# MingyuKim87/Safe_Denoiser

Hardware: AMD Instinct MI355X
Metric: images/sec (512x512, 50 steps, SD-v1.4 + repellency) (higher is better)
Workload: dtype bf16; 1 GPU; README-default end to end (safree = svf = lra = true, safree_neg_prompt_config.json:26-28): token ids -> CLIP -> SAFREE projection -> DDPM 50 steps x UNet on 3 guidance branches with per-prompt text switching + safe_denoiser.yaml repellency (kernel_fast, M=515, sigma 3.15, scale .33, margin 1.6, window 780<=t<=1000) -> VAE decode -> uint8 512x512 images; SD-v1.4 UNet / CLIP / VAE with random weigh; guidance_branches=3, text_encoder_precision=bf16x3, prompts_per_batch=64, latent_repeat=3, renoise_draws_rank0=3520, parallelism=prompt-shard x1

## Files before the change

### include/sdn.h

```cpp
#ifndef SDN_H_
#define SDN_H_

#include <stddef.h>
#include <stdint.h>

#ifdef __cplusplus
extern "C" {
#endif

#define SDN_OK            0
#define SDN_E_INVALID    -1
#define SDN_E_LAUNCH     -2
#define SDN_E_WORKSPACE  -3
#define SDN_E_ARCH       -4

int sdn_abi_version(void);
const char* sdn_device_arch_host(void);


#define SDN_REPEL_RBF     0
#define SDN_REPEL_SPARSE  1
#define SDN_QNORM_NONE    0
#define SDN_QNORM_CHANNEL 1
#define SDN_OUT_REPELLED  0
// ... 129 lines not shown
                        void* stream);

int sdn_layernorm_mod_bf16(const void* x, int64_t rows, int32_t c, float eps, const float* scale, const float* shift,
                           int32_t ld_mod, int32_t rows_per_batch, void* out, void* stream);
int sdn_layernorm_mod_f16(const void* x, int64_t rows, int32_t c, float eps, const float* scale, const float* shift,
                          int32_t ld_mod, int32_t rows_per_batch, void* out, void* stream);

int sdn_patchify_bf16(const float* latents, int32_t batch, int32_t c, int32_t h, int32_t w, int32_t p, void* out, void* stream);
int sdn_patchify_f16(const float* latents, int32_t batch, int32_t c, int32_t h, int32_t w, int32_t p, void* out, void* stream);
int sdn_unpatchify_f32(const float* tokens, int32_t batch, int32_t c, int32_t h, int32_t w, int32_t p, float* out, void* stream);

int sdn_conv_in_bf16(const float* latents_nchw, const void* w, const float* bias, int32_t batch, int32_t cin,
                     int32_t h, int32_t wd, int32_t cout, void* out_nhwc, void* stream);
int sdn_conv_in_f16(const float* latents_nchw, const void* w, const float* bias, int32_t batch, int32_t cin,
                    int32_t h, int32_t wd, int32_t cout, void* out_nhwc, void* stream);

int sdn_timestep_embed_bf16(float timestep, int32_t batch, int32_t dim, void* out, void* stream);
int sdn_timestep_embed_f16(float timestep, int32_t batch, int32_t dim, void* out, void* stream);

int sdn_gemm_f32(const sdn_gemm_desc* d_host, const void* a, const void* a2, const void* w,
                 const float* bias, const float* rowbias, const float* rowgate, const void* residual, void* out,
                 void* stream);
int sdn_groupnorm_f32(const void* x, const void* x2, int32_t batch, int32_t hw, int32_t c1, int32_t c2,
                      int32_t groups, float eps, int32_t silu, const float* gamma, const float* beta,
                      void* out, float* stats_ws, void* stream);
int sdn_layernorm_f32(const void* x, int64_t rows, int32_t c, float eps, const float* gamma,
                      const float* beta, void* out, void* stream);
int sdn_attention_f32(const void* q, const void* k, const void* v, void* out, int32_t batch, int32_t heads,
                      int32_t nq, int32_t nk, int32_t head_dim, int32_t ldq, int32_t ldk, int32_t ldv,
                      int32_t ldo, float scale, void* stream);
int sdn_conv_in_f32(const float* latents_nchw, const void* w, const float* bias, int32_t batch, int32_t cin,
                    int32_t h, int32_t wd, int32_t cout, void* out_nhwc, void* stream);
int sdn_timestep_embed_f32(float timestep, int32_t batch, int32_t dim, void* out, void* stream);

int sdn_gemm_x3(const sdn_gemm_desc* d_host, const void* a, const void* a2, const void* w,
                const float* bias, const float* rowbias, const float* rowgate, const void* residual, void* out,
                void* stream);
int sdn_attention_x3(const void* q, const void* k, const void* v, void* out, int32_t batch, int32_t heads,
                     int32_t nq, int32_t nk, int32_t head_dim, int32_t ldq, int32_t ldk, int32_t ldv,
                     int32_t ldo, float scale, void* stream);

int sdn_layernorm_mod_f32(const void* x, int64_t rows, int32_t c, float eps, const float* scale, const float* shift,
                          int32_t ld_mod, int32_t rows_per_batch, void* out, void* stream);
int sdn_patchify_f32(const float* latents, int32_t batch, int32_t c, int32_t h, int32_t w, int32_t p, void* out, void* stream);
int sdn_joint_attention_f32(int32_t mode, const void* q, const void* k, const void* v, void* out,
                            const sdn_attn_segment2* seg2_host, int32_t batch, int32_t heads, int32_t n_total,
                            int32_t head_dim, int32_t ldq, int32_t ldk, int32_t ldv, int32_t ldo, float scale,
                            void* stream);

int sdn_split3(const float* x, const float* x2, int64_t rows, int32_t c1, int32_t c2, void* out_triple, void* stream);
int sdn_expand3_weights(const float* w, int64_t rows, int32_t cols, int32_t group, void* out_bf16, void* stream);
int sdn_groupnorm_f32_triple(const void* x, const void* x2, int32_t batch, int32_t hw, int32_t c1, int32_t c2, int32_t groups,
                             float eps, int32_t silu, const float* gamma, const float* beta, void* out_triple, float* stats_ws,
                             void* stream);
int sdn_layernorm_f32_triple(const void* x, int64_t rows, int32_t c, float eps, const float* gamma, const float* beta,
                             void* out_triple, void* stream);
int sdn_attention_x3_triple(const void* q, const void* k, const void* v, void* out_triple, int32_t batch, int32_t heads, int32_t nq,
                            int32_t nk, int32_t head_dim, int32_t ldq, int32_t ldk, int32_t ldv, int32_t ldo, float scale,
                            void* stream);
int sdn_attention_x3_pairs(const void* q, const void* k, const void* v, int32_t lo_offset_q, int32_t lo_offset_kv, void* out,
                           int32_t batch, int32_t heads, int32_t nq, int32_t nk, int32_t head_dim, int32_t ldq, int32_t ldk,
                           int32_t ldv, int32_t ldo, float scale, int32_t triple_out, void* stream);

int sdn_randn_philox_plan(int64_t numel, int32_t* grid_out, int64_t* offset_increment_out);
int sdn_randn_philox(const uint64_t* seeds, const uint64_t* offsets, const int32_t* rows, int32_t n_gen, int64_t numel,
                     float* out, void* stream);
int sdn_randn_philox_state(const uint64_t* seeds, uint64_t* offsets, const int32_t* flags, int32_t n_gen, int64_t numel,
                           float* out, void* stream);

typedef struct sdn_unet_config {
  int32_t in_channels, out_channels, sample_size;
  int32_t n_levels;
  int32_t block_out_channels[4];
  int32_t level_has_attn[4];
  int32_t layers_per_block;
  int32_t n_heads;
  int32_t cross_dim, text_len;
  int32_t norm_groups;
  int32_t dtype;
  int32_t latent_repeat;
} sdn_unet_config;

typedef struct sdn_unet sdn_unet;

#define SDN_P_VEC_F32     0
#define SDN_P_MAT         1
#define SDN_P_CONV3X3     2
#define SDN_P_GEGLU_MAT   3
#define SDN_P_GEGLU_VEC   4
#define SDN_P_POS_CROP    5
#define SDN_P_GLU_VALUE   7
#define SDN_P_GLU_GATE    8
#define SDN_P_DERIVED     6

typedef struct sdn_param_info {
  char     name[128];
  int32_t  kind;
  int32_t  rows, cols;
  int32_t  rows_padded;
  int64_t  offset;
} sdn_param_info;

int    sdn_unet_create(const sdn_unet_config* cfg_host, sdn_unet** out_host);
void   sdn_unet_destroy(sdn_unet* u);
int    sdn_unet_param_count(const sdn_unet* u);
int    sdn_unet_param_info(const sdn_unet* u, int32_t index, sdn_param_info* info_host);
size_t sdn_unet_weight_bytes(const sdn_unet* u);
size_t sdn_unet_workspace_bytes(sdn_unet* u, int32_t batch);
double sdn_unet_flops(sdn_unet* u, int32_t batch, double* attention_core_flops_host);

int sdn_unet_forward(sdn_unet* u, const void* weights, const float* latents, float timestep, const void* text,
                     float* out, int32_t batch, void* workspace, size_t workspace_bytes, void* stream);

typedef struct sdn_mmdit_config {
  int32_t in_channels, out_channels;
  int32_t sample_size, patch_size;
  int32_t num_layers;
  int32_t num_heads, head_dim;
  int32_t joint_dim, pooled_dim;
  int32_t text_len;
  int32_t time_dim;
  int32_t dtype;
} sdn_mmdit_config;
int sdn_mmdit_create(const sdn_mmdit_config* cfg_host, sdn_unet** out_host);
int sdn_mmdit_forward(sdn_unet* m, const void* weights, const float* latents, float timestep, const void* text,
                      const void* pooled, float* out, int32_t batch, void* workspace, size_t workspace_bytes,
                      void* stream);

typedef struct sdn_mmdit_ext {
  int32_t qk_norm;
  float qk_norm_eps;
  uint64_t dual_attention_mask;
} sdn_mmdit_ext;
int sdn_mmdit_create_ex(const sdn_mmdit_config* cfg_host, const sdn_mmdit_ext* ext_host, sdn_unet** out_host);
int sdn_qk_rmsnorm(int32_t dtype, void* qkv, int64_t rows, int32_t heads, int32_t ld, const float* wq, const float* wk, float eps,
                   void* stream);

int sdn_ln_fold(int32_t dtype, const void* w, const float* gamma, const float* beta, const float* bias, int32_t rows,
                int32_t cols, void* w_folded, float* c, float* d, void* stream);
int sdn_gemm_ln_bf16(const sdn_gemm_desc* desc, const void* a, const void* w_folded, const float* c, const float* d, float eps,
                     const float* row_stats, void* out, void* stream);
int sdn_gemm_ln_f16(const sdn_gemm_desc* desc, const void* a, const void* w_folded, const float* c, const float* d, float eps,
                    const float* row_stats, void* out, void* stream);
int sdn_row_stats_bf16(const void* x, int64_t rows, int32_t c, float eps, float* out, void* stream);
int sdn_row_stats_f16(const void* x, int64_t rows, int32_t c, float eps, float* out, void* stream);

int sdn_ffn_geglu_fused(int32_t dtype, int64_t M, int32_t C, const void* x, const float* row_stats, const void* w1_folded,
                        const float* c1, const float* d1, const void* w_cat, const float* b_cat, const void* residual, void* out,
                        float* col_stats, void* stream);

int sdn_gemm_k320(int32_t dtype, const sdn_gemm_desc* desc, const void* a, const void* w, const float* bias, const float* ln_c,
                  const float* ln_d, float ln_eps, const void* residual, void* out, void* stream);
int32_t sdn_gemm_k320_map(int32_t grid, int32_t col_groups, int32_t wg, int32_t* stream_out, int32_t* group_out);

int sdn_gemm_stats_bf16(const sdn_gemm_desc* desc, const void* a, const void* a2, const void* w, const float* bias,
                        const float* rowbias, const void* residual, void* out, float* col_stats, void* stream);
int sdn_gemm_stats_f16(const sdn_gemm_desc* desc, const void* a, const void* a2, const void* w, const float* bias,
                       const float* rowbias, const void* residual, void* out, float* col_stats, void* stream);
int sdn_groupnorm_cols_bf16(const void* x, const void* x2, int32_t batch, int32_t hw, int32_t c1, int32_t c2, int32_t groups,
                            float eps, int32_t silu, const float* gamma, const float* beta, void* out, float* stats_ws,
                            const float* cols1, const float* cols2, void* stream);
int sdn_groupnorm_cols_f16(const void* x, const void* x2, int32_t batch, int32_t hw, int32_t c1, int32_t c2, int32_t groups,
                           float eps, int32_t silu, const float* gamma, const float* beta, void* out, float* stats_ws,
                           const float* cols1, const float* cols2, void* stream);

int sdn_gemm_splitk_bf16(const sdn_gemm_desc* d, const void* a, const void* a2, const void* w, const float* bias,
                         const float* rowbias, const float* rowgate, const void* residual, void* out, void* partials,
                         size_t partial_bytes, void* stream);
int sdn_gemm_splitk_f16(const sdn_gemm_desc* d, const void* a, const void* a2, const void* w, const float* bias,
                        const float* rowbias, const float* rowgate, const void* residual, void* out, void* partials,
                        size_t partial_bytes, void* stream);

int sdn_conv_up4_weights(int32_t dtype, const void* w9, int32_t N, int32_t Cin, void* out, void* stream);

int sdn_repeat(const void* in, size_t bytes, int32_t rep, void* out, void* stream);

int sdn_unet_prepare(sdn_unet* u, void* weights, void* stream);

typedef struct sdn_vae_config {
  int32_t latent_channels, out_channels;
  int32_t sample_size;
  int32_t n_levels;
  int32_t block_out_channels[4];
  int32_t layers_per_block;
  int32_t norm_groups;
  int32_t dtype;
} sdn_vae_config;
int sdn_vae_decoder_create(const sdn_vae_config* cfg_host, sdn_unet** out_host);
int sdn_vae_decode(sdn_unet* vae, const void* weights, const float* latents, float latent_scale, float* image,
                   int32_t batch, void* workspace, size_t workspace_bytes, void* stream);
int sdn_vae_encoder_create(const sdn_vae_config* cfg_host, sdn_unet** out_host);
int sdn_vae_encode(sdn_unet* vae_encoder, const void* weights, const float* image, float* moments, int32_t batch,
                   void* workspace, size_t workspace_bytes, void* stream);
int sdn_gaussian_sample(const float* moments, const float* noise, int32_t batch, int32_t latent_channels, int32_t hw,
                        float scale, float* out, void* stream);
int sdn_image_postprocess(const float* image_nchw, int32_t batch, int32_t channels, int32_t height, int32_t width,
                          float* out_nhwc01, uint8_t* out_nhwc_u8, void* stream);
int sdn_latent_mix(const float* z, const float* w, const float* bias, int32_t batch, int32_t channels, int32_t hw,
                   float in_scale, float* out, void* stream);
int sdn_softmax_rows(int32_t dtype, const float* scores, int64_t ld_scores, int64_t rows, int32_t n, float scale,
                     void* out, int64_t ld_out, void* stream);
int sdn_transpose16(const void* in, int32_t rows, int32_t cols, int64_t ld_in, void* out, int64_t ld_out, void* stream);
int sdn_transpose32(const void* in, int32_t rows, int32_t cols, int64_t ld_in, void* out, int64_t ld_out, void* stream);

typedef struct sdn_clip_config {
  int32_t vocab_size;
  int32_t hidden_size, intermediate_size;
  int32_t num_layers, num_heads;
  int32_t max_position_embeddings;
  int32_t dtype;
} sdn_clip_config;
int sdn_clip_create(const sdn_clip_config* cfg_host, sdn_unet** out_host);
int sdn_clip_forward(sdn_unet* clip, const void* weights, const int32_t* input_ids, const int32_t* attention_mask,
                     void* last_hidden_state, int32_t batch, void* workspace, size_t workspace_bytes, void* stream);
int sdn_clip_embed(int32_t dtype, const int32_t* input_ids, const void* token_embedding, const void* position_embedding,
                   int64_t rows, int32_t seq_len, int32_t hidden, int32_t vocab, void* out, void* stream);
int sdn_masked_attention(int32_t dtype, const void* q, const void* k, const void* v, void* out, const int32_t* key_mask,
                         int32_t causal, int32_t batch, int32_t heads, int32_t n, int32_t head_dim, int32_t ldq,
                         int32_t ldk, int32_t ldv, int32_t ldo, float scale, void* stream);
int sdn_clip_embed_f32(const int32_t* input_ids, const void* token_embedding, const void* position_embedding, int64_t rows,
                       int32_t seq_len, int32_t hidden, int32_t vocab, void* out, void* stream);
int sdn_masked_attention_f32(const void* q, const void* k, const void* v, void* out, const int32_t* key_mask, int32_t causal,
                             int32_t batch, int32_t heads, int32_t n, int32_t head_dim, int32_t ldq, int32_t ldk, int32_t ldv,
                             int32_t ldo, float scale, void* stream);

typedef struct sdn_clip_proj_config {
  int32_t vocab_size;
  int32_t hidden_size, intermediate_size;
  int32_t num_layers, num_heads;
  int32_t max_position_embeddings;
  int32_t dtype;
  int32_t projection_dim;
  int32_t act;
  int32_t eos_token_id;
  int32_t hidden_tap;
} sdn_clip_proj_config;
int sdn_clip_proj_create(const sdn_clip_proj_config* cfg_host, sdn_unet** out_host);
int sdn_clip_proj_forward(sdn_unet* clip, const void* weights, const int32_t* input_ids, void* hidden, int64_t hidden_batch_stride,
                          int64_t hidden_row_stride, void* text_embeds, int64_t embeds_row_stride, int32_t batch, void* workspace,
                          size_t workspace_bytes, void* stream);
int sdn_clip_eos_rows(int32_t dtype, const int32_t* input_ids, const void* x, const float* gamma, const float* beta, int32_t batch,
                      int32_t seq_len, int32_t hidden, int32_t vocab, int32_t eos_token_id, float eps, void* out,
                      int32_t* positions, void* stream);
int sdn_copy_rows_strided(const void* src, int32_t batch, int32_t rows_per_batch, int32_t cols, int32_t elem_bytes, void* dst,
                          int64_t dst_batch_stride, int64_t dst_row_stride, void* stream);

typedef struct sdn_clip_vision_config {
  int32_t image_size, patch_size;
  int32_t hidden_size, intermediate_size;
  int32_t num_layers, num_heads;
  int32_t projection_dim;
  int32_t act;
  int32_t dtype;
} sdn_clip_vision_config;
int sdn_clip_vision_create(const sdn_clip_vision_config* cfg_host, sdn_unet** out_host);
int sdn_clip_vision_forward(sdn_unet* vision, const void* weights, const float* pixel_values, void* last_hidden_state,
                            void* image_embeds, int32_t batch, void* workspace, size_t workspace_bytes, void* stream);
int sdn_clip_patch_rows(int32_t dtype, const float* pixels, int32_t batch, int32_t image_size, int32_t patch_size, int32_t kpad,
                        void* out, void* stream);
int sdn_clip_vision_embed(int32_t dtype, const void* patch_proj, const float* class_embedding, const void* position_embedding,
                          const float* gamma, const float* beta, int32_t batch, int32_t tokens, int32_t hidden, float eps, void* out,
                          void* stream);
int sdn_clip_class_rows(int32_t dtype, const void* x, const float* gamma, const float* beta, int32_t batch, int32_t seq_len,
                        int32_t hidden, float eps, void* out, void* stream);
int sdn_image_resize_u8(const uint8_t* in, int32_t batch, int32_t in_size, int32_t out_size, const int32_t* coeffs,
                        const int32_t* bounds, int32_t ksize, uint8_t* tmp, uint8_t* out, void* stream);
int sdn_clip_normalize_u8(const uint8_t* in, int32_t batch, int32_t size, float mean_r, float mean_g, float mean_b, float std_r,
                          float std_g, float std_b, float* out, void* stream);
int sdn_embed_row_scores(const void* x, int32_t dtype_x, int64_t ldx, const void* y, int32_t dtype_y, int64_t ldy,
                         int32_t y_rows, int32_t rows, int32_t dim, int32_t normalize_y, float scale, float bias,
                         float* out, void* stream);
int sdn_embed_cross_mean(const void* x, int32_t dtype_x, int64_t ldx, int32_t rx, const void* y, int32_t dtype_y, int64_t ldy,
                         int32_t ry, int32_t dim, float* scratch, float* out, void* stream);
int sdn_image_resize_rect_u8(const uint8_t* in, int32_t batch, int32_t in_h, int32_t in_w, int32_t out_h, int32_t out_w,
                             const int32_t* coeffs_x, const int32_t* bounds_x, int32_t ksize_x, const int32_t* coeffs_y,
                             const int32_t* bounds_y, int32_t ksize_y, uint8_t* tmp, uint8_t* out_u8, float* out_f32, float mean_r,
                             float mean_g, float mean_b, float std_r, float std_g, float std_b, void* stream);

typedef struct sdn_t5_config {
  int32_t vocab_size;
  int32_t d_model, d_kv, d_ff;
  int32_t num_layers, num_heads;
  int32_t num_buckets, max_distance;
  float   eps;
  int32_t dtype;
} sdn_t5_config;
int sdn_t5_create(const sdn_t5_config* cfg_host, sdn_unet** out_host);
size_t sdn_t5_workspace_bytes(sdn_unet* t5, int32_t batch, int32_t n);
double sdn_t5_flops(sdn_unet* t5, int32_t batch, int32_t n, double* attention_core_flops_host);
int sdn_t5_forward(sdn_unet* t5, const void* weights, const int32_t* input_ids, const int32_t* attention_mask, int32_t n,
                   void* out, int32_t batch, void* workspace, size_t workspace_bytes, void* stream);
int sdn_rmsnorm(int32_t dtype, const void* x, int32_t x_is_f32, int64_t rows, int32_t c, float eps, const float* weight, void* out,
                void* stream);
int sdn_embed_tokens(int32_t dtype, const int32_t* input_ids, const void* token_embedding, int64_t rows, int32_t hidden,
                     int32_t vocab, float* out, void* stream);
int sdn_t5_bucket(int32_t relative_position, int32_t num_buckets, int32_t max_distance);
int sdn_t5_relative_bias(int32_t dtype, const void* table, int32_t num_buckets, int32_t max_distance, int32_t heads, int32_t n,
                         float* out, void* stream);
int sdn_bias_attention(int32_t dtype, const void* q, const void* k, const void* v, void* out, const float* bias,
                       const int32_t* key_mask, int32_t batch, int32_t heads, int32_t n, int32_t head_dim, int32_t ldq,
                       int32_t ldk, int32_t ldv, int32_t ldo, float scale, void* stream);

void sdn_unet_set_text_version(sdn_unet* u, uint64_t version);

void sdn_unet_set_graph_mode(sdn_unet* u, int32_t on);
void sdn_unet_set_split_k(sdn_unet* u, int32_t on);
// ... 42 lines not shown
```

### safe_denoiser_amd/_lib.py

```python
from __future__ import annotations

import ctypes as C
import os

import torch

_HERE = os.path.dirname(os.path.abspath(__file__))
_LIB = None


class SdnUnavailable(RuntimeError):
    """libsdn.so is missing/unloadable, or there is no gfx950 device for a compute call."""


class SdnError(RuntimeError):
    """A libsdn entry point returned a negative status."""


_ERR = {-1: "SDN_E_INVALID (bad shape / null or misaligned pointer)", -2: "SDN_E_LAUNCH", -3: "SDN_E_WORKSPACE",
        -4: "SDN_E_ARCH"}


def lib_path() -> str:
    return os.environ.get("SDN_LIB", os.path.join(_HERE, "libsdn.so"))


class RepelParams(C.Structure):
    _fields_ = [("n_query", C.c_int32), ("n_ref", C.c_int32), ("channels", C.c_int32), ("hw", C.c_int32),
                ("weight_fn", C.c_int32), ("qnorm", C.c_int32), ("sigma", C.c_float), ("radius", C.c_float),
                ("scale", C.c_float), ("epsilon", C.c_float), ("gate", C.c_float)]


class GemmDesc(C.Structure):
    _fields_ = [(n, C.c_int32) for n in ("M", "N", "K", "a_mode", "K1", "Hs", "Ws", "Cin", "Ho", "Wo", "stride",
                                         "upsample", "act", "out_kind", "rows_per_batch", "ld_rowbias", "ld_rowgate",
                                         "residual_bcast", "n_valid", "ldc", "asym_pad", "split_k", "res_pre", "x3_out",
                                         "f32_stream")]


class UnetConfig(C.Structure):
    _fields_ = [("in_channels", C.c_int32), ("out_channels", C.c_int32), ("sample_size", C.c_int32),
                ("n_levels", C.c_int32), ("block_out_channels", C.c_int32 * 4), ("level_has_attn", C.c_int32 * 4),
                ("layers_per_block", C.c_int32), ("n_heads", C.c_int32), ("cross_dim", C.c_int32),
                ("text_len", C.c_int32), ("norm_groups", C.c_int32), ("dtype", C.c_int32), ("latent_repeat", C.c_int32)]


class ProfileRow(C.Structure):
    _fields_ = [("kernel", C.c_char * 24), ("launches", C.c_int32), ("ms", C.c_double), ("flops", C.c_double),
                ("bytes", C.c_double)]


class MmditConfig(C.Structure):
    _fields_ = [(n, C.c_int32) for n in ("in_channels", "out_channels", "sample_size", "patch_size", "num_layers",
                                         "num_heads", "head_dim", "joint_dim", "pooled_dim", "text_len", "time_dim",
                                         "dtype")]


class MmditExt(C.Structure):
    _fields_ = [("qk_norm", C.c_int32), ("qk_norm_eps", C.c_float), ("dual_attention_mask", C.c_uint64)]


class VaeConfig(C.Structure):
    _fields_ = [("latent_channels", C.c_int32), ("out_channels", C.c_int32), ("sample_size", C.c_int32),
                ("n_levels", C.c_int32), ("block_out_channels", C.c_int32 * 4), ("layers_per_block", C.c_int32),
                ("norm_groups", C.c_int32), ("dtype", C.c_int32)]


class ClipConfig(C.Structure):
    _fields_ = [(n, C.c_int32) for n in ("vocab_size", "hidden_size", "intermediate_size", "num_layers", "num_heads",
                                         "max_position_embeddings", "dtype")]


class ClipProjConfig(C.Structure):
    _fields_ = [(n, C.c_int32) for n in ("vocab_size", "hidden_size", "intermediate_size", "num_layers", "num_heads",
                                         "max_position_embeddings", "dtype", "projection_dim", "act", "eos_token_id", "hidden_tap")]


class ClipVisionConfig(C.Structure):
    _fields_ = [(n, C.c_int32) for n in ("image_size", "patch_size", "hidden_size", "intermediate_size", "num_layers", "num_heads",
                                         "projection_dim", "act", "dtype")]


class InceptionConfig(C.Structure):
    _fields_ = [(n, C.c_int32) for n in ("image_size", "normalize_input", "dtype")]


class InceptionConv(C.Structure):
    _fields_ = [("name", C.c_char * 64)] + [(n, C.c_int32) for n in ("cin", "cout", "kh", "kw", "stride", "pad_h", "pad_w", "kpad",
                                                                     "n_padded")]


class T5Config(C.Structure):
    _fields_ = [(n, C.c_int32) for n in ("vocab_size", "d_model", "d_kv", "d_ff", "num_layers", "num_heads", "num_buckets",
                                         "max_distance")] + [("eps", C.c_float), ("dtype", C.c_int32)]


class AttnSegment2(C.Structure):
    _fields_ = [("q2", C.c_void_p), ("k2", C.c_void_p), ("v2", C.c_void_p), ("out2", C.c_void_p), ("n1", C.c_int32),
                ("ldq2", C.c_int32), ("ldk2", C.c_int32), ("ldv2", C.c_int32), ("ldo2", C.c_int32)]


class ParamInfo(C.Structure):
    _fields_ = [("name", C.c_char * 128), ("kind", C.c_int32), ("rows", C.c_int32), ("cols", C.c_int32),
                ("rows_padded", C.c_int32), ("offset", C.c_int64)]


_vp, _i32, _i64, _f32, _sz = C.c_void_p, C.c_int32, C.c_int64, C.c_float, C.c_size_t

SIGNATURES = {
    "sdn_abi_version": (C.c_int, []),
    "sdn_device_arch_host": (C.c_char_p, []),
    "sdn_repel_workspace_bytes": (_sz, [_i32, _i32, _i32, _i32]),
    "sdn_repel_apply": (C.c_int, [C.POINTER(RepelParams), _vp, _vp, _vp, _vp, _vp, _vp, _sz, _vp]),
    "sdn_repel_calibrate": (C.c_int, [C.POINTER(RepelParams), _vp, _vp, _vp, _vp, _sz, _vp]),
    "sdn_cfg_combine": (C.c_int, [_vp, _i32, _i32, _i64, _f32, _vp, _vp]),
    "sdn_sld_guidance": (C.c_int, [_vp, _i32, _i64, _f32, _f32, _f32, _f32, _f32, _i32, _vp, _vp, _vp]),
    "sdn_cfg_combine_rows": (C.c_int, [_vp, _i32, _i32, _i64, _vp, _vp, _vp]),
    "sdn_sld_guidance_rows": (C.c_int, [_vp, _i32, _i64, _vp, _f32, _f32, _f32, _f32, _i32, _vp, _vp, _vp]),
    "sdn_pred_x0": (C.c_int, [_vp, _vp, _i64, _f32, _f32, _f32, _vp, _vp]),
    "sdn_sched_step": (C.c_int, [_vp, _vp, _vp, _i64, _f32, _f32, _f32, _f32, _f32, _f32, _f32, _vp, _vp]),
    "sdn_add_noise": (C.c_int, [_vp, _vp, _i64, _f32, _f32, _vp, _vp]),
    "sdn_renoise_select": (C.c_int, [_vp, _vp, _vp, _vp, _i32, _i64, _f32, _f32, _vp]),
    "sdn_flow_euler_step": (C.c_int, [_vp, _vp, _i64, _f32, _f32, _vp, _vp]),
    "sdn_flow_endpoints": (C.c_int, [_vp, _vp, _i64, _f32, _vp, _vp, _vp]),
    "sdn_flow_renoise": (C.c_int, [_vp, _vp, _vp, _i64, _f32, _vp, _vp]),
    "sdn_gemm_bf16": (C.c_int, [C.POINTER(GemmDesc), _vp, _vp, _vp, _vp, _vp, _vp, _vp, _vp, _vp]),
    "sdn_gemm_f16": (C.c_int, [C.POINTER(GemmDesc), _vp, _vp, _vp, _vp, _vp, _vp, _vp, _vp, _vp]),
    "sdn_ln_fold": (C.c_int, [_i32, _vp, _vp, _vp, _vp, _i32, _i32, _vp, _vp, _vp, _vp]),
    "sdn_gemm_ln_bf16": (C.c_int, [C.POINTER(GemmDesc), _vp, _vp, _vp, _vp, _f32, _vp, _vp, _vp]),
    "sdn_gemm_ln_f16": (C.c_int, [C.POINTER(GemmDesc), _vp, _vp, _vp, _vp, _f32, _vp, _vp, _vp]),
    "sdn_row_stats_bf16": (C.c_int, [_vp, _i64, _i32, _f32, _vp, _vp]),
    "sdn_row_stats_f16": (C.c_int, [_vp, _i64, _i32, _f32, _vp, _vp]),
    "sdn_ffn_geglu_fused": (C.c_int, [_i32, _i64, _i32, _vp, _vp, _vp, _vp, _vp, _vp, _vp, _vp, _vp, _vp, _vp]),
    "sdn_gemm_k320": (C.c_int, [_i32, C.POINTER(GemmDesc), _vp, _vp, _vp, _vp, _vp, _f32, _vp, _vp, _vp]),
    "sdn_gemm_k320_map": (_i32, [_i32, _i32, _i32, C.POINTER(_i32), C.POINTER(_i32)]),
    "sdn_gemm_stats_bf16": (C.c_int, [C.POINTER(GemmDesc), _vp, _vp, _vp, _vp, _vp, _vp, _vp, _vp, _vp]),
    "sdn_gemm_stats_f16": (C.c_int, [C.POINTER(GemmDesc), _vp, _vp, _vp, _vp, _vp, _vp, _vp, _vp, _vp]),
    "sdn_groupnorm_cols_bf16": (C.c_int, [_vp, _vp, _i32, _i32, _i32, _i32, _i32, _f32, _i32, _vp, _vp, _vp, _vp, _vp, _vp, _vp]),
    "sdn_groupnorm_cols_f16": (C.c_int, [_vp, _vp, _i32, _i32, _i32, _i32, _i32, _f32, _i32, _vp, _vp, _vp, _vp, _vp, _vp, _vp]),
    "sdn_gemm_splitk_bf16": (C.c_int, [C.POINTER(GemmDesc), _vp, _vp, _vp, _vp, _vp, _vp, _vp, _vp, _vp, _sz, _vp]),
    "sdn_gemm_splitk_f16": (C.c_int, [C.POINTER(GemmDesc), _vp, _vp, _vp, _vp, _vp, _vp, _vp, _vp, _vp, _sz, _vp]),
    "sdn_groupnorm_bf16": (C.c_int, [_vp, _vp, _i32, _i32, _i32, _i32, _i32, _f32, _i32, _vp, _vp, _vp, _vp, _vp]),
    "sdn_groupnorm_f16": (C.c_int, [_vp, _vp, _i32, _i32, _i32, _i32, _i32, _f32, _i32, _vp, _vp, _vp, _vp, _vp]),
    "sdn_layernorm_f16": (C.c_int, [_vp, _i64, _i32, _f32, _vp, _vp, _vp, _vp]),
    "sdn_conv_in_f16": (C.c_int, [_vp, _vp, _vp, _i32, _i32, _i32, _i32, _i32, _vp, _vp]),
    "sdn_timestep_embed_f16": (C.c_int, [_f32, _i32, _i32, _vp, _vp]),
    "sdn_layernorm_bf16": (C.c_int, [_vp, _i64, _i32, _f32, _vp, _vp, _vp, _vp]),
    "sdn_attention_bf16": (C.c_int, [_vp, _vp, _vp, _vp, _i32, _i32, _i32, _i32, _i32, _i32, _i32, _i32, _i32, _f32,
                                     _vp]),
    "sdn_attention_f16": (C.c_int, [_vp, _vp, _vp, _vp, _i32, _i32, _i32, _i32, _i32, _i32, _i32, _i32, _i32, _f32,
                                    _vp]),
    "sdn_conv_in_bf16": (C.c_int, [_vp, _vp, _vp, _i32, _i32, _i32, _i32, _i32, _vp, _vp]),
    "sdn_timestep_embed_bf16": (C.c_int, [_f32, _i32, _i32, _vp, _vp]),
    "sdn_gemm_f32": (C.c_int, [C.POINTER(GemmDesc), _vp, _vp, _vp, _vp, _vp, _vp, _vp, _vp, _vp]),
    "sdn_groupnorm_f32": (C.c_int, [_vp, _vp, _i32, _i32, _i32, _i32, _i32, _f32, _i32, _vp, _vp, _vp, _vp, _vp]),
    "sdn_layernorm_f32": (C.c_int, [_vp, _i64, _i32, _f32, _vp, _vp, _vp, _vp]),
    "sdn_attention_f32": (C.c_int, [_vp, _vp, _vp, _vp, _i32, _i32, _i32, _i32, _i32, _i32, _i32, _i32, _i32, _f32, _vp]),
    "sdn_randn_philox_plan": (C.c_int, [C.c_int64, C.POINTER(C.c_int32), C.POINTER(C.c_int64)]),
    "sdn_randn_philox": (C.c_int, [_vp, _vp, _vp, _i32, C.c_int64, _vp, _vp]),
    "sdn_randn_philox_state": (C.c_int, [_vp, _vp, _vp, _i32, C.c_int64, _vp, _vp]),
    "sdn_gemm_x3": (C.c_int, [C.POINTER(GemmDesc), _vp, _vp, _vp, _vp, _vp, _vp, _vp, _vp, _vp]),
    "sdn_attention_x3": (C.c_int, [_vp, _vp, _vp, _vp, _i32, _i32, _i32, _i32, _i32, _i32, _i32, _i32, _i32, _f32, _vp]),
    "sdn_conv_in_f32": (C.c_int, [_vp, _vp, _vp, _i32, _i32, _i32, _i32, _i32, _vp, _vp]),
    "sdn_timestep_embed_f32": (C.c_int, [_f32, _i32, _i32, _vp, _vp]),
    "sdn_unet_create": (C.c_int, [C.POINTER(UnetConfig), C.POINTER(_vp)]),
    "sdn_unet_destroy": (None, [_vp]),
    "sdn_unet_param_count": (C.c_int, [_vp]),
    "sdn_unet_param_info": (C.c_int, [_vp, _i32, C.POINTER(ParamInfo)]),
    "sdn_unet_weight_bytes": (_sz, [_vp]),
    "sdn_unet_workspace_bytes": (_sz, [_vp, _i32]),
    "sdn_unet_flops": (C.c_double, [_vp, _i32, C.POINTER(C.c_double)]),
    "sdn_unet_forward": (C.c_int, [_vp, _vp, _vp, _f32, _vp, _vp, _i32, _vp, _sz, _vp]),
    "sdn_mmdit_create": (C.c_int, [C.POINTER(MmditConfig), C.POINTER(_vp)]),
    "sdn_mmdit_forward": (C.c_int, [_vp, _vp, _vp, _f32, _vp, _vp, _vp, _i32, _vp, _sz, _vp]),
    "sdn_mmdit_create_ex": (C.c_int, [C.POINTER(MmditConfig), C.POINTER(MmditExt), C.POINTER(_vp)]),
    "sdn_qk_rmsnorm": (C.c_int, [_i32, _vp, _i64, _i32, _i32, _vp, _vp, _f32, _vp]),
    "sdn_joint_attention": (C.c_int, [_i32, _vp, _vp, _vp, _vp, C.POINTER(AttnSegment2), _i32, _i32, _i32, _i32, _i32,
                                      _i32, _i32, _i32, _f32, _vp]),
    "sdn_layernorm_mod_bf16": (C.c_int, [_vp, _i64, _i32, _f32, _vp, _vp, _i32, _i32, _vp, _vp]),
    "sdn_layernorm_mod_f16": (C.c_int, [_vp, _i64, _i32, _f32, _vp, _vp, _i32, _i32, _vp, _vp]),
    "sdn_patchify_bf16": (C.c_int, [_vp, _i32, _i32, _i32, _i32, _i32, _vp, _vp]),
    "sdn_patchify_f16": (C.c_int, [_vp, _i32, _i32, _i32, _i32, _i32, _vp, _vp]),
    "sdn_unpatchify_f32": (C.c_int, [_vp, _i32, _i32, _i32, _i32, _i32, _vp, _vp]),
    "sdn_layernorm_mod_f32": (C.c_int, [_vp, _i64, _i32, _f32, _vp, _vp, _i32, _i32, _vp, _vp]),
    "sdn_patchify_f32": (C.c_int, [_vp, _i32, _i32, _i32, _i32, _i32, _vp, _vp]),
    "sdn_joint_attention_f32": (C.c_int, [_i32, _vp, _vp, _vp, _vp, C.POINTER(AttnSegment2), _i32, _i32, _i32, _i32, _i32,
                                          _i32, _i32, _i32, _f32, _vp]),
    "sdn_repeat": (C.c_int, [_vp, _sz, _i32, _vp, _vp]),
    "sdn_vae_decoder_create": (C.c_int, [C.POINTER(VaeConfig), C.POINTER(_vp)]),
    "sdn_vae_decode": (C.c_int, [_vp, _vp, _vp, _f32, _vp, _i32, _vp, _sz, _vp]),
    "sdn_vae_encoder_create": (C.c_int, [C.POINTER(VaeConfig), C.POINTER(_vp)]),
    "sdn_vae_encode": (C.c_int, [_vp, _vp, _vp, _vp, _i32, _vp, _sz, _vp]),
    "sdn_gaussian_sample": (C.c_int, [_vp, _vp, _i32, _i32, _i32, _f32, _vp, _vp]),
    "sdn_image_postprocess": (C.c_int, [_vp, _i32, _i32, _i32, _i32, _vp, _vp, _vp]),
    "sdn_latent_mix": (C.c_int, [_vp, _vp, _vp, _i32, _i32, _i32, _f32, _vp, _vp]),
    "sdn_softmax_rows": (C.c_int, [_i32, _vp, _i64, _i64, _i32, _f32, _vp, _i64, _vp]),
    "sdn_transpose16": (C.c_int, [_vp, _i32, _i32, _i64, _vp, _i64, _vp]),
    "sdn_transpose32": (C.c_int, [_vp, _i32, _i32, _i64, _vp, _i64, _vp]),
    "sdn_clip_create": (C.c_int, [C.POINTER(ClipConfig), C.POINTER(_vp)]),
    "sdn_clip_forward": (C.c_int, [_vp, _vp, _vp, _vp, _vp, _i32, _vp, _sz, _vp]),
    "sdn_clip_embed": (C.c_int, [_i32, _vp, _vp, _vp, _i64, _i32, _i32, _i32, _vp, _vp]),
    "sdn_masked_attention": (C.c_int, [_i32, _vp, _vp, _vp, _vp, _vp, _i32, _i32, _i32, _i32, _i32, _i32, _i32, _i32, _i32,
                                       _f32, _vp]),
    "sdn_clip_proj_create": (C.c_int, [C.POINTER(ClipProjConfig), C.POINTER(_vp)]),
    "sdn_clip_proj_forward": (C.c_int, [_vp, _vp, _vp, _vp, _i64, _i64, _vp, _i64, _i32, _vp, _sz, _vp]),
    "sdn_clip_eos_rows": (C.c_int, [_i32, _vp, _vp, _vp, _vp, _i32, _i32, _i32, _i32, _i32, _f32, _vp, _vp, _vp]),
    "sdn_copy_rows_strided": (C.c_int, [_vp, _i32, _i32, _i32, _i32, _vp, _i64, _i64, _vp]),
    "sdn_clip_vision_create": (C.c_int, [C.POINTER(ClipVisionConfig), C.POINTER(_vp)]),
    "sdn_clip_vision_forward": (C.c_int, [_vp, _vp, _vp, _vp, _vp, _i32, _vp, _sz, _vp]),
    "sdn_clip_patch_rows": (C.c_int, [_i32, _vp, _i32, _i32, _i32, _i32, _vp, _vp]),
    "sdn_clip_vision_embed": (C.c_int, [_i32, _vp, _vp, _vp, _vp, _vp, _i32, _i32, _i32, _f32, _vp, _vp]),
    "sdn_clip_class_rows": (C.c_int, [_i32, _vp, _vp, _vp, _i32, _i32, _i32, _f32, _vp, _vp]),
    "sdn_image_resize_u8": (C.c_int, [_vp, _i32, _i32, _i32, _vp, _vp, _i32, _vp, _vp, _vp]),
    "sdn_clip_normalize_u8": (C.c_int, [_vp, _i32, _i32, _f32, _f32, _f32, _f32, _f32, _f32, _vp, _vp]),
    "sdn_image_resize_rect_u8": (C.c_int, [_vp, _i32, _i32, _i32, _i32, _i32, _vp, _vp, _i32, _vp, _vp, _i32, _vp, _vp, _vp, _f32, _f32,
                                           _f32, _f32, _f32, _f32, _vp]),
    "sdn_inception_create": (C.c_int, [C.POINTER(InceptionConfig), C.POINTER(_vp)]),
    "sdn_inception_conv_count": (C.c_int, [_vp]),
    "sdn_inception_conv_info": (C.c_int, [_vp, _i32, C.POINTER(InceptionConv)]),
    "sdn_inception_forward": (C.c_int, [_vp, _vp, _vp, _vp, _i32, _i32, _i32, _i32, _vp, _sz, _vp]),
    "sdn_patch_rows_f32": (C.c_int, [_vp, _i32, _i32, _i32, _i32, _i32, _i32, _i32, _i32, _i32, _i32, _i32, _vp, _vp]),
    "sdn_pool3_f32": (C.c_int, [_i32, _vp, _i32, _i32, _i32, _i32, _i32, _i32, _vp, _i32, _i32, _vp]),
    "sdn_resize_bilinear_f32": (C.c_int, [_vp, _i32, _i32, _i32, _i32, _i32, _f32, _f32, _vp, _vp]),
    "sdn_spatial_mean_f32": (C.c_int, [_vp, _i32, _i32, _i32, _vp, _vp]),
    "sdn_embed_row_scores": (C.c_int, [_vp, _i32, _i64, _vp, _i32, _i64, _i32, _i32, _i32, _i32, _f32, _f32, _vp, _vp]),
    "sdn_embed_cross_mean": (C.c_int, [_vp, _i32, _i64, _i32, _vp, _i32, _i64, _i32, _i32, _vp, _vp, _vp]),
    "sdn_t5_create": (C.c_int, [C.POINTER(T5Config), C.POINTER(_vp)]),
    "sdn_t5_workspace_bytes": (_sz, [_vp, _i32, _i32]),
    "sdn_t5_flops": (C.c_double, [_vp, _i32, _i32, C.POINTER(C.c_double)]),
    "sdn_t5_forward": (C.c_int, [_vp, _vp, _vp, _vp, _i32, _vp, _i32, _vp, _sz, _vp]),
    "sdn_rmsnorm": (C.c_int, [_i32, _vp, _i32, _i64, _i32, _f32, _vp, _vp, _vp]),
    "sdn_embed_tokens": (C.c_int, [_i32, _vp, _vp, _i64, _i32, _i32, _vp, _vp]),
    "sdn_t5_bucket": (C.c_int, [_i32, _i32, _i32]),
    "sdn_t5_relative_bias": (C.c_int, [_i32, _vp, _i32, _i32, _i32, _i32, _vp, _vp]),
    "sdn_bias_attention": (C.c_int, [_i32, _vp, _vp, _vp, _vp, _vp, _vp, _i32, _i32, _i32, _i32, _i32, _i32, _i32, _i32, _f32,
                                     _vp]),
    "sdn_split3": (C.c_int, [_vp, _vp, _i64, _i32, _i32, _vp, _vp]),
    "sdn_expand3_weights": (C.c_int, [_vp, _i64, _i32, _i32, _vp, _vp]),
    "sdn_groupnorm_f32_triple": (C.c_int, [_vp, _vp, _i32, _i32, _i32, _i32, _i32, _f32, _i32, _vp, _vp, _vp, _vp, _vp]),
    "sdn_layernorm_f32_triple": (C.c_int, [_vp, _i64, _i32, _f32, _vp, _vp, _vp, _vp]),
    "sdn_attention_x3_triple": (C.c_int, [_vp, _vp, _vp, _vp, _i32, _i32, _i32, _i32, _i32, _i32, _i32, _i32, _i32, _f32, _vp]),
    "sdn_attention_x3_pairs": (C.c_int, [_vp, _vp, _vp, _i32, _i32, _vp, _i32, _i32, _i32, _i32, _i32, _i32, _i32, _i32, _i32, _f32, _i32, _vp]),
    "sdn_clip_embed_f32": (C.c_int, [_vp, _vp, _vp, _i64, _i32, _i32, _i32, _vp, _vp]),
    "sdn_masked_attention_f32": (C.c_int, [_vp, _vp, _vp, _vp, _vp, _i32, _i32, _i32, _i32, _i32, _i32, _i32, _i32, _i32, _f32, _vp]),
    "sdn_unet_prepare": (C.c_int, [_vp, _vp, _vp]),
    "sdn_unet_set_graph_mode": (None, [_vp, _i32]),
    "sdn_unet_set_text_version": (None, [_vp, C.c_uint64]),
    "sdn_unet_set_split_k": (None, [_vp, _i32]),
    "sdn_unet_set_conv_up4": (None, [_vp, _i32]),
    "sdn_conv_up4_weights": (C.c_int, [_i32, _vp, _i32, _i32, _vp, _vp]),
    "sdn_unet_profile_next": (None, [_vp]),
    "sdn_unet_profile_read": (C.c_int, [_vp, C.POINTER(ProfileRow), _i32]),
}


def lib():
    global _LIB
    if _LIB is None:
        path = lib_path()
        if not os.path.exists(path):
            raise SdnUnavailable(f"{path} not found: build it with `python -c 'import __graft_entry__ as g; g.build()'` "
                                 f"(or `make -C safe_denoiser_amd/csrc`).  There is no CPU fallback.")
        try:
            handle = C.CDLL(path)
        except OSError as e:
            raise SdnUnavailable(f"cannot load {path}: {e}") from e
        for name, (res, args) in SIGNATURES.items():
            fn = getattr(handle, name)
            fn.restype, fn.argtypes = res, args
        _LIB = handle
    return _LIB


def check(rc: int, what: str):
    if rc != 0:
        raise SdnError(f"{what} failed: {_ERR.get(rc, rc)}")


def require_gpu():
    if not torch.cuda.is_available():
        raise SdnUnavailable("no GPU visible: the safe-denoiser hot path only runs on an MI355X (gfx950); "
                             "there is no CPU fallback")


def dptr(t: torch.Tensor | None, dtype=None) -> int | None:
    if t is None:
        return None
# ... 12 lines not shown
```

### safe_denoiser_amd/csrc/sdn_gemm_k320.hip

```cpp
#include "sdn_common.h"
#include "sdn_ops.h"
#include "sdn_gemm_common.h"
#include "sdn_gemm_k320.h"

static int g_k320_max_wgs = 0;
static int g_k320_last[8] = {0};

namespace sdn_gemm_detail {

struct K320Args {
  const unsigned short* a; const unsigned short* w; const float* bias; const float* ln_c; const float* ln_d;
  const unsigned short* res; unsigned short* out;
  int M, ldc, ncg;
  float ln_eps;
};

template <typename T, int LNF, bool RES>
__global__ void __launch_bounds__(512)
k_gemm_k320(const K320Args g) {
#if defined(__HIP_DEVICE_COMPILE__)
  constexpr int ROWS = RES ? 32 : 64;
  constexpr int G = ROWS / 32;
  constexpr int RB = ROWS / 8;
  constexpr int IMG = ROWS * 128;
  constexpr int A_PIECES = 5 * RB / 4;
  constexpr int SLOT = 40960, RING = 3 * SLOT;
  constexpr int STG = RING;
  constexpr int PRM = STG + 32 * 640;
  constexpr int SMEM = PRM + 3 * 1280;
  static_assert(5 * IMG * (RES ? 2 : 1) == SLOT, "a panel fills its slot");
  static_assert(A_PIECES + (RES ? 5 : 0) == 10, "vmcnt(10) below counts ten pieces per DMA wave and panel");
  __shared__ __attribute__((aligned(1024))) unsigned char smem[SMEM];

  const int tid = threadIdx.x, lane = tid & 63;
  const int wid = __builtin_amdgcn_readfirstlane(tid >> 6);
  const int wm = wid >> 2, wn = wid & 3;
  const int fr = lane & 15, fq = lane >> 4;
  int stream, cg;
  const int S = sdn_k320_map((int)gridDim.x, g.ncg, (int)blockIdx.x, &stream, &cg);
  if (stream < 0) return;
  const int n0 = cg * 320;

  typename T::v8 wf[5][10];
  {
    const unsigned short* wrow = g.w + (long)(n0 + wn * 80 + fr) * 320 + fq * 8;
#pragma unroll
    for (int t = 0; t < 5; ++t)
#pragma unroll
      for (int s = 0; s < 10; ++s) wf[t][s] = *reinterpret_cast<const typename T::v8*>(wrow + t * 16 * 320 + s * 32);
  }
  if (tid < 320) {
    float* prm = reinterpret_cast<float*>(smem + PRM);
    prm[tid] = g.bias ? g.bias[n0 + tid] : 0.f;
    if constexpr (LNF) { prm[320 + tid] = g.ln_c[n0 + tid]; prm[640 + tid] = g.ln_d[n0 + tid]; }
  }
#pragma unroll
  for (int t = 0; t < 5; ++t)
#pragma unroll
    for (int s = 0; s < 10; ++s) asm volatile("" : "+v"(wf[t][s]));
  asm volatile("s_waitcnt vmcnt(0)" ::: "memory");
  __syncthreads();

  const __amdgpu_buffer_rsrc_t rs_a = make_rsrc(g.a, (unsigned)((long)g.M * 640));
  [[maybe_unused]] const __amdgpu_buffer_rsrc_t rs_r = make_rsrc(RES ? g.res : g.a, RES ? (unsigned)((long)g.M * g.ldc * 2) : 0u);
  auto issue = [&](int p, int slot, int ln) {
    const int lrow = (ln >> 3) & 7;
    const unsigned a_lane = (unsigned)(lrow * 640 + (((ln & 7) ^ lrow) << 4));
    [[maybe_unused]] const unsigned r_lane = (unsigned)(lrow * g.ldc * 2 + (((ln & 7) ^ lrow) << 4));
    const unsigned m0 = (unsigned)p * ROWS;
    unsigned char* dst = smem + slot * SLOT;
#pragma unroll
    for (int q = 0; q < A_PIECES; ++q) {
      const int piece = wid * A_PIECES + q;
      const int kt = piece / RB, rb = piece - kt * RB;
      const unsigned off = (m0 + rb * 8) * 640u + kt * 128 + a_lane;
      __builtin_amdgcn_raw_ptr_buffer_load_lds(rs_a, (lds_ptr_t)(dst + piece * 1024), 16, off, 0, 0, 0);
    }
    if constexpr (RES) {
#pragma unroll
      for (int q = 0; q < 5; ++q) {
        const unsigned off = (m0 + wid * 8) * (unsigned)(g.ldc * 2) + (unsigned)(n0 * 2 + q * 128) + r_lane;
        __builtin_amdgcn_raw_ptr_buffer_load_lds(rs_r, (lds_ptr_t)(dst + 5 * IMG + (wid * 5 + q) * 1024), 16, off, 0, 0, 0);
      }
    }
  };

  const int NP = (g.M + ROWS - 1) / ROWS;
  const int n_my = stream < NP ? (NP - stream + S - 1) / S : 0;
  if (wid < 4) { issue(stream, 0, tid); issue(stream + S, 1, tid); }

  const float* prm = reinterpret_cast<const float*>(smem + PRM);
  int slot = 0;
  for (int i = 0; i < n_my; ++i) {
    int tl = tid;
    asm volatile("" : "+v"(tl));
    const int fr = tl & 15, fq = (tl >> 4) & 3;
    const int orow = wm * 16 + fr;
    const int o_rowpart = (orow >> 3) * 5120 + (orow & 7) * 128;
    auto out_off = [&](int t) {
      const int cb = wn * 160 + t * 32 + fq * 8;
      return o_rowpart + (cb >> 7) * 1024 + ((((cb >> 4) & 7) ^ (orow & 7)) << 4) + (cb & 8);
    };
    const int st_r = (tl >> 3) & 31;
    const int st_lds = (st_r >> 3) * 5120 + (st_r & 7) * 128 + (((tl & 7) ^ (st_r & 7)) << 4);
    const int p = stream + i * S;
    const int m0 = p * ROWS;
    if (wid < 4) asm volatile("s_waitcnt vmcnt(10)" ::: "memory");
    asm volatile("s_waitcnt lgkmcnt(0)" ::: "memory");
    __builtin_amdgcn_s_barrier();
    asm volatile("" ::: "memory");
    if (wid < 4) issue(p + 2 * S, slot == 0 ? 2 : slot - 1, tl);
    const unsigned char* sa = smem + slot * SLOT;
#pragma unroll
    for (int gi = 0; gi < G; ++gi) {
      const int row_l = wm * (ROWS / 2) + gi * 16 + fr;
      f32x4 acc[5];
#pragma unroll
      for (int t = 0; t < 5; ++t) acc[t] = *reinterpret_cast<const f32x4*>(prm + wn * 80 + t * 16 + fq * 4);
      if constexpr (RES) {
        const unsigned r_addr = (unsigned)(unsigned long)(lds_ptr_t)const_cast<unsigned char*>(sa + 5 * IMG);
        unsigned long long rr[5];
#pragma unroll
        for (int t = 0; t < 5; ++t) asm volatile("ds_read_b64 %0, %1" : "=v"(rr[t]) : "v"(r_addr + (unsigned)out_off(t)) : "memory");
        asm volatile("s_waitcnt lgkmcnt(0)" : "+v"(rr[0]), "+v"(rr[1]), "+v"(rr[2]), "+v"(rr[3]), "+v"(rr[4])::"memory");
#pragma unroll
        for (int t = 0; t < 5; ++t) {
          const unsigned lo = (unsigned)rr[t], hi = (unsigned)(rr[t] >> 32);
          acc[t][0] += T::to_f(lo & 0xffff); acc[t][1] += T::to_f(lo >> 16);
          acc[t][2] += T::to_f(hi & 0xffff); acc[t][3] += T::to_f(hi >> 16);
        }
      }
      [[maybe_unused]] float s1 = 0.f, s2 = 0.f;
      typename T::v8 fa[2];
      fa[0] = *reinterpret_cast<const typename T::v8*>(sa + lds_off(row_l, fq));
#pragma unroll
      for (int s = 0; s < 10; ++s) {
        if (s + 1 < 10)
          fa[(s + 1) & 1] = *reinterpret_cast<const typename T::v8*>(sa + ((s + 1) >> 1) * IMG + lds_off(row_l, ((s + 1) & 1) * 4 + fq));
        __builtin_amdgcn_sched_barrier(0);
        if constexpr (LNF) { s1 = T::dot_ones(fa[s & 1], s1); s2 = T::dot_self(fa[s & 1], s2); }
#pragma unroll
        for (int t = 0; t < 5; ++t) acc[t] = T::mfma16(wf[t][s], fa[s & 1], acc[t]);
        __builtin_amdgcn_sched_barrier(0);
      }
      [[maybe_unused]] float mu = 0.f, rs = 0.f;
      if constexpr (LNF) {
        const float invk = 1.0f / 320.0f;
        float a1 = s1, a2 = s2;
        a1 += __shfl_xor(a1, 16, 64); a2 += __shfl_xor(a2, 16, 64);
        a1 += __shfl_xor(a1, 32, 64); a2 += __shfl_xor(a2, 32, 64);
        mu = a1 * invk;
        const float var = fmaxf(a2 * invk - mu * mu, 0.f);
        rs = __builtin_amdgcn_rsqf(var + g.ln_eps);
      }
      if (!RES && gi > 0) {
        asm volatile("s_waitcnt lgkmcnt(0)" ::: "memory");
        __builtin_amdgcn_s_barrier();
        asm volatile("" ::: "memory");
      }
      const unsigned char* oimg = RES ? sa + 5 * IMG : smem + STG;
      const unsigned o_addr = (unsigned)(unsigned long)(lds_ptr_t)const_cast<unsigned char*>(oimg);
#pragma unroll
      for (int t = 0; t < 5; ++t) {
        f32x4 v = acc[t];
        if constexpr (LNF) {
          const f32x4 cv = *reinterpret_cast<const f32x4*>(prm + 320 + wn * 80 + t * 16 + fq * 4);
          const f32x4 dv = *reinterpret_cast<const f32x4*>(prm + 640 + wn * 80 + t * 16 + fq * 4);
          v = (acc[t] - mu * cv) * rs + dv;
        }
        uint2 pk; pk.x = T::pack2(v[0], v[1]); pk.y = T::pack2(v[2], v[3]);
        asm volatile("ds_write_b64 %0, %1" ::"v"(o_addr + (unsigned)out_off(t)), "v"((unsigned long long)pk.y << 32 | pk.x) : "memory");
        if constexpr (LNF) __builtin_amdgcn_sched_barrier(0);
      }
      asm volatile("s_waitcnt lgkmcnt(0)" ::: "memory");
      __builtin_amdgcn_s_barrier();
      asm volatile("" ::: "memory");
      if (wid >= 4) {
        const int m = m0 + (RES ? st_r : (st_r >> 4) * 32 + gi * 16 + (st_r & 15));
        if (m < g.M) {
          unsigned short* op = g.out + (long)m * g.ldc + n0 + (tl & 7) * 8;
#pragma unroll
          for (int k = 0; k < 5; ++k) *reinterpret_cast<u32x4*>(op + k * 64) = *reinterpret_cast<const u32x4*>(oimg + st_lds + k * 1024);
        }
      }
    }
    slot = slot == 2 ? 0 : slot + 1;
  }
  asm volatile("s_waitcnt vmcnt(0)" ::: "memory");
#endif
}

template <typename T>
int launch_k320(const K320Args& g, int grid, bool ln, bool res, hipStream_t st) {
  if (ln) hipLaunchKernelGGL((k_gemm_k320<T, 1, false>), dim3(grid), dim3(512), 0, st, g);
  else if (res) hipLaunchKernelGGL((k_gemm_k320<T, 0, true>), dim3(grid), dim3(512), 0, st, g);
  else hipLaunchKernelGGL((k_gemm_k320<T, 0, false>), dim3(grid), dim3(512), 0, st, g);
  return sdn_launch_status();
}

static inline bool al16(const void* p) { return (reinterpret_cast<uintptr_t>(p) & 15) == 0; }

}
using namespace sdn_gemm_detail;

extern "C" int32_t sdn_gemm_k320_map(int32_t grid, int32_t col_groups, int32_t wg, int32_t* stream_out, int32_t* group_out) {
  if (grid <= 0 || col_groups <= 0 || wg < 0 || wg >= grid) return SDN_E_INVALID;
  int s = -1, c = 0;
  const int S = sdn_k320_map(grid, col_groups, wg, &s, &c);
  if (stream_out) *stream_out = s;
  if (group_out) *group_out = c;
  return S;
}

extern "C" void sdn_debug_set_k320_max_wgs(int n) { g_k320_max_wgs = n > 0 ? n : 0; }
extern "C" void sdn_debug_k320_last_launch(int* out, int n) {
  for (int i = 0; out && i < n; ++i) out[i] = i < 8 ? g_k320_last[i] : 0;
}
extern "C" void sdn_debug_k320_reset_launch(void) { for (int& v : g_k320_last) v = 0; }

extern "C" int sdn_gemm_k320(int32_t dtype, const sdn_gemm_desc* d, const void* a, const void* w, const float* bias, const float* ln_c,
                             const float* ln_d, float ln_eps, const void* residual, void* out, void* stream) {
  if (!d || !a || !w || !out || dtype < 0 || dtype > 1) return SDN_E_INVALID;
  if (d->K != 320 || d->N <= 0 || d->N % 320 != 0 || d->M < 0) return SDN_E_INVALID;
  if (d->a_mode != SDN_A_PLAIN || (d->K1 != 0 && d->K1 != d->K) || d->act != SDN_ACT_NONE || d->out_kind != SDN_OUT_BF16 ||
      (d->n_valid != 0 && d->n_valid != d->N) || d->residual_bcast || d->split_k > 1 || d->x3_out || d->f32_stream || d->upsample)
    return SDN_E_INVALID;
  const bool ln = ln_c || ln_d;
  if (ln && (!ln_c || !ln_d || bias || residual)) return SDN_E_INVALID;
  const int ldc = d->ldc > 0 ? d->ldc : d->N;
  if (ldc < d->N || (ldc & 7)) return SDN_E_INVALID;
  if (!al16(a) || !al16(w) || !al16(out) || (residual && !al16(residual)) || (bias && !al16(bias)) || (ln && (!al16(ln_c) || !al16(ln_d))))
    return SDN_E_INVALID;
  if ((long)d->M * 640 >= (1L << 31) || (long)d->M * ldc * 2 >= (1L << 31) || ((long)d->M + 40000) * ldc * 2 >= (1L << 32)) return SDN_E_INVALID;
  if (d->M == 0) return SDN_OK;
  static int cus = 0;
  if (cus == 0) {
    int dev = 0;
    hipDeviceProp_t prop;
    if (hipGetDevice(&dev) != hipSuccess || hipGetDeviceProperties(&prop, dev) != hipSuccess) return SDN_E_LAUNCH;
    cus = prop.multiProcessorCount;
  }
  const int ncg = d->N / 320;
  int grid = cus > ncg ? cus : ncg;
  if (g_k320_max_wgs > 0 && g_k320_max_wgs < cus) {
    const int want = g_k320_max_wgs / ncg > 0 ? g_k320_max_wgs / ncg : 1;
    int s0, c0;
    for (grid = ncg; grid < cus && sdn_k320_map(grid, ncg, 0, &s0, &c0) < want; ++grid) {}
  }
  {
    int s0, c0;
    if (sdn_k320_map(grid, ncg, 0, &s0, &c0) < 1) return SDN_E_INVALID;
  }
  K320Args g{};
  g.a = (const unsigned short*)a; g.w = (const unsigned short*)w; g.bias = bias; g.ln_c = ln_c; g.ln_d = ln_d;
  g.res = (const unsigned short*)residual; g.out = (unsigned short*)out;
  g.M = d->M; g.ldc = ldc; g.ncg = ncg; g.ln_eps = ln_eps;
  {
    int s0, c0;
    const int S = sdn_k320_map(grid, ncg, 0, &s0, &c0);
    const int rows = residual ? 32 : 64;
    const int v[8] = {6, dtype, ln ? 1 : 0, residual ? 1 : 0, grid, ncg, S, (d->M + rows - 1) / rows};
    for (int i = 0; i < 8; ++i) g_k320_last[i] = v[i];
  }
  hipStream_t st = (hipStream_t)stream;
  return dtype == 0 ? launch_k320<SdnBF16>(g, grid, ln, residual != nullptr, st) : launch_k320<SdnF16>(g, grid, ln, residual != nullptr, st);
}
```

### safe_denoiser_amd/csrc/sdn_norm.hip

```cpp
#include "sdn_common.h"
#include "sdn_ops.h"

namespace sdn_norm_detail {

typedef __attribute__((ext_vector_type(4))) unsigned int u32x4;
constexpr int THREADS = 256;
constexpr int GN_MAX_TILES = 128;

template <typename T>
__device__ __forceinline__ void unpack8(const u32x4 v, float* f) {
  f[0] = T::to_f(v.x & 0xffff); f[1] = T::to_f(v.x >> 16); f[2] = T::to_f(v.y & 0xffff); f[3] = T::to_f(v.y >> 16);
  f[4] = T::to_f(v.z & 0xffff); f[5] = T::to_f(v.z >> 16); f[6] = T::to_f(v.w & 0xffff); f[7] = T::to_f(v.w >> 16);
}
template <typename T>
__device__ __forceinline__ u32x4 pack8(const float* f) {
  return (u32x4){T::pack2(f[0], f[1]), T::pack2(f[2], f[3]), T::pack2(f[4], f[5]), T::pack2(f[6], f[7])};
}
__device__ __forceinline__ float silu_f(float v) { return v / (1.f + __expf(-v)); }

template <typename T>
__global__ void __launch_bounds__(THREADS)
k_gn_stats(const unsigned short* __restrict__ x, const unsigned short* __restrict__ x2, int hw, int c1, int c2,
           int groups, int rows_per_tile, int ct, int nch, float* __restrict__ partials) {
  extern __shared__ float lds[];
  const int C = c1 + c2, cpg = C / groups;
  const int b = blockIdx.x, tile = blockIdx.y, ntiles = gridDim.y;
  const int rt = THREADS / ct;
  const int cl = threadIdx.x % ct, rl = threadIdx.x / ct;
  const int r_lo = tile * rows_per_tile, r_hi = min(hw, r_lo + rows_per_tile);
  if (rl < rt) {
    for (int q = 0; q < nch; ++q) {
      const int ch0 = (cl + q * ct) * 8;
      const unsigned short* src; int ld, cc;
      if (ch0 < c1) { src = x; ld = c1; cc = ch0; } else { src = x2; ld = c2; cc = ch0 - c1; }
      float s[8], ss[8];
#pragma unroll
      for (int e = 0; e < 8; ++e) { s[e] = 0.f; ss[e] = 0.f; }
      for (int r = r_lo + rl; r < r_hi; r += 4 * rt) {
        u32x4 v[4];
#pragma unroll
        for (int j = 0; j < 4; ++j) {
          const int rr = min(r + j * rt, r_hi - 1);
          v[j] = *reinterpret_cast<const u32x4*>(src + ((long)b * hw + rr) * ld + cc);
        }
#pragma unroll
        for (int j = 0; j < 4; ++j) {
          if (r + j * rt < r_hi) {
            float f[8];
            unpack8<T>(v[j], f);
#pragma unroll
            for (int e = 0; e < 8; ++e) { s[e] += f[e]; ss[e] = fmaf(f[e], f[e], ss[e]); }
          }
        }
      }
#pragma unroll
      for (int e = 0; e < 8; ++e) {
        lds[((long)rl * C + ch0 + e) * 2 + 0] = s[e];
        lds[((long)rl * C + ch0 + e) * 2 + 1] = ss[e];
      }
    }
  }
  __syncthreads();
  if (threadIdx.x < groups) {
    const int gidx = threadIdx.x;
    float s = 0.f, ss = 0.f;
    for (int r = 0; r < rt; ++r)
      for (int c = gidx * cpg; c < (gidx + 1) * cpg; ++c) {
        s += lds[((long)r * C + c) * 2 + 0];
        ss += lds[((long)r * C + c) * 2 + 1];
      }
    float* o = partials + (((long)b * ntiles + tile) * groups + gidx) * 2;
    o[0] = s; o[1] = ss;
  }
}

__global__ void __launch_bounds__(512)
k_gn_finalize(const float* __restrict__ partials, int ntiles, int groups, float n, float eps,
              float* __restrict__ stats) {
  __shared__ float sh[64][8][2];
  const int b = blockIdx.x, gi = threadIdx.x >> 3, part = threadIdx.x & 7;
  if (gi < groups) {
    float s = 0.f, ss = 0.f;
    for (int t = part; t < ntiles; t += 8) {
      const float* p = partials + (((long)b * ntiles + t) * groups + gi) * 2;
      s += p[0]; ss += p[1];
    }
    sh[gi][part][0] = s; sh[gi][part][1] = ss;
  }
  __syncthreads();
  if (gi < groups && part == 0) {
    float s = 0.f, ss = 0.f;
#pragma unroll
    for (int k = 0; k < 8; ++k) { s += sh[gi][k][0]; ss += sh[gi][k][1]; }
    const float mean = s / n;
    const float var = fmaxf(ss / n - mean * mean, 0.f);
    stats[((long)b * groups + gi) * 2 + 0] = mean;
    stats[((long)b * groups + gi) * 2 + 1] = rsqrtf(var + eps);
  }
}

__global__ void __launch_bounds__(256)
k_gn_finalize_cols(const float* __restrict__ cols1, const float* __restrict__ cols2, int blocks_per_sample, int c1, int c2,
                   int groups, float n, float eps, float* __restrict__ stats) {
  __shared__ float red[8];
  const int C = c1 + c2, cpg = C / groups, b = blockIdx.x, gi = blockIdx.y;
  const int total = blocks_per_sample * cpg;
  float s = 0.f, q = 0.f;
  for (int e = threadIdx.x; e < total; e += 256) {
    const int t = e / cpg, c = gi * cpg + (e - t * cpg);
    const bool second = c >= c1;
    const float* src = second ? cols2 : cols1;
    const int cw = second ? c2 : c1, cc = second ? c - c1 : c;
    const float2 v = *reinterpret_cast<const float2*>(src + 2 * (((long)b * blocks_per_sample + t) * cw + cc));
    s += v.x; q += v.y;
  }
  s = block_sum<4>(s, red);
  q = block_sum<4>(q, red + 4);
  if (threadIdx.x == 0) {
    const float mean = s / n;
    const float var = fmaxf(q / n - mean * mean, 0.f);
    stats[((long)b * groups + gi) * 2 + 0] = mean;
    stats[((long)b * groups + gi) * 2 + 1] = rsqrtf(var + eps);
  }
}

template <typename T>
__global__ void __launch_bounds__(THREADS)
k_gn_apply(const unsigned short* __restrict__ x, const unsigned short* __restrict__ x2, int hw, int c1, int c2,
           int groups, int rows_per_block, int silu, const float* __restrict__ gamma,
           const float* __restrict__ beta, const float* __restrict__ stats, unsigned short* __restrict__ out) {
  extern __shared__ float aff[];
  const int C = c1 + c2, cpg = C / groups, cchunks = C / 8;
  const int b = blockIdx.x;
  float* ca = aff; float* cb = aff + C;
  for (int c = threadIdx.x; c < C; c += THREADS) {
    const int gi = c / cpg;
    const float mean = stats[((long)b * groups + gi) * 2 + 0], rstd = stats[((long)b * groups + gi) * 2 + 1];
    const float a = rstd * gamma[c];
    ca[c] = a; cb[c] = beta[c] - mean * a;
  }
  __syncthreads();
  const int r_lo = blockIdx.y * rows_per_block, r_hi = min(hw, r_lo + rows_per_block);
  const long total = (long)(r_hi - r_lo) * cchunks;
  for (long e = threadIdx.x; e < total; e += THREADS) {
    const int r = r_lo + (int)(e / cchunks), ch0 = (int)(e % cchunks) * 8;
    const unsigned short* src; int ld, cc;
    if (ch0 < c1) { src = x; ld = c1; cc = ch0; } else { src = x2; ld = c2; cc = ch0 - c1; }
    const u32x4 v = *reinterpret_cast<const u32x4*>(src + ((long)b * hw + r) * ld + cc);
    float f[8];
    unpack8<T>(v, f);
    const float4 a0 = *reinterpret_cast<const float4*>(ca + ch0), a1 = *reinterpret_cast<const float4*>(ca + ch0 + 4);
    const float4 b0 = *reinterpret_cast<const float4*>(cb + ch0), b1 = *reinterpret_cast<const float4*>(cb + ch0 + 4);
    const float am[8] = {a0.x, a0.y, a0.z, a0.w, a1.x, a1.y, a1.z, a1.w};
    const float bm[8] = {b0.x, b0.y, b0.z, b0.w, b1.x, b1.y, b1.z, b1.w};
#pragma unroll
    for (int k = 0; k < 8; ++k) {
      const float y = fmaf(f[k], am[k], bm[k]);
      f[k] = silu ? silu_f(y) : y;
    }
    *reinterpret_cast<u32x4*>(out + ((long)b * hw + r) * C + ch0) = pack8<T>(f);
  }
}

template <typename T, int NQ, int R>
__global__ void __launch_bounds__(THREADS)
k_layernorm(const unsigned short* __restrict__ x, long rows, int C, float eps, const float* __restrict__ gamma,
            const float* __restrict__ beta, unsigned short* __restrict__ out, int mod, int rows_per_batch, int ld_mod) {
  const int lane = threadIdx.x & 63;
  const long row0 = ((long)blockIdx.x * 4 + (threadIdx.x >> 6)) * R;
  if (row0 >= rows) return;
  const int cchunks = C / 8;
  float f[R][NQ][8];
  float s[R];
#pragma unroll
  for (int r = 0; r < R; ++r) {
    s[r] = 0.f;
    const long row = row0 + r < rows ? row0 + r : rows - 1;
#pragma unroll
    for (int q = 0; q < NQ; ++q) {
      const int cc = lane + q * 64;
      if (cc < cchunks) {
        unpack8<T>(*reinterpret_cast<const u32x4*>(x + row * C + cc * 8), f[r][q]);
#pragma unroll
        for (int k = 0; k < 8; ++k) s[r] += f[r][q][k];
      }
    }
  }
  float mean[R], rstd[R];
#pragma unroll
  for (int r = 0; r < R; ++r) mean[r] = wave_sum(s[r]) / (float)C;
#pragma unroll
  for (int r = 0; r < R; ++r) {
    float ss = 0.f;
#pragma unroll
    for (int q = 0; q < NQ; ++q) {
      const int cc = lane + q * 64;
      if (cc < cchunks) {
#pragma unroll
        for (int k = 0; k < 8; ++k) { const float d = f[r][q][k] - mean[r]; ss = fmaf(d, d, ss); }
      }
    }
    s[r] = ss;
  }
#pragma unroll
  for (int r = 0; r < R; ++r) rstd[r] = rsqrtf(wave_sum(s[r]) / (float)C + eps);
#pragma unroll
  for (int q = 0; q < NQ; ++q) {
    const int cc = lane + q * 64;
    if (cc < cchunks) {
      float gm[8], bt[8];
      auto load_affine = [&](const float* gp, const float* bp) {
        const float4 g0 = *reinterpret_cast<const float4*>(gp + cc * 8), g1 = *reinterpret_cast<const float4*>(gp + cc * 8 + 4);
        const float4 b0 = *reinterpret_cast<const float4*>(bp + cc * 8), b1 = *reinterpret_cast<const float4*>(bp + cc * 8 + 4);
        gm[0] = g0.x; gm[1] = g0.y; gm[2] = g0.z; gm[3] = g0.w; gm[4] = g1.x; gm[5] = g1.y; gm[6] = g1.z; gm[7] = g1.w;
        bt[0] = b0.x; bt[1] = b0.y; bt[2] = b0.z; bt[3] = b0.w; bt[4] = b1.x; bt[5] = b1.y; bt[6] = b1.z; bt[7] = b1.w;
      };
      if (!mod) load_affine(gamma, beta);
#pragma unroll
      for (int r = 0; r < R; ++r) {
        const long row = row0 + r;
        if (row < rows) {
          if (mod) {
            const long b = row / rows_per_batch;
            load_affine(gamma + b * ld_mod, beta + b * ld_mod);
          }
          float y[8];
#pragma unroll
          for (int k = 0; k < 8; ++k) y[k] = (f[r][q][k] - mean[r]) * rstd[r] * (mod ? 1.f + gm[k] : gm[k]) + bt[k];
          *reinterpret_cast<u32x4*>(out + row * C + cc * 8) = pack8<T>(y);
        }
      }
    }
  }
}

template <typename T, int NQ, int R>
__global__ void __launch_bounds__(THREADS)
k_row_stats(const unsigned short* __restrict__ x, long rows, int C, float eps, float* __restrict__ out) {
  const int lane = threadIdx.x & 63;
  const long row0 = ((long)blockIdx.x * 4 + (threadIdx.x >> 6)) * R;
  if (row0 >= rows) return;
  const int cchunks = C / 8;
  float f[R][NQ][8];
  float s[R];
#pragma unroll
  for (int r = 0; r < R; ++r) {
    s[r] = 0.f;
    const long row = row0 + r < rows ? row0 + r : rows - 1;
#pragma unroll
    for (int q = 0; q < NQ; ++q) {
      const int cc = lane + q * 64;
      if (cc < cchunks) {
        unpack8<T>(*reinterpret_cast<const u32x4*>(x + row * C + cc * 8), f[r][q]);
#pragma unroll
        for (int k = 0; k < 8; ++k) s[r] += f[r][q][k];
      }
    }
  }
  float mean[R];
#pragma unroll
  for (int r = 0; r < R; ++r) mean[r] = wave_sum(s[r]) / (float)C;
#pragma unroll
  for (int r = 0; r < R; ++r) {
    float ss = 0.f;
#pragma unroll
    for (int q = 0; q < NQ; ++q) {
      const int cc = lane + q * 64;
      if (cc < cchunks) {
#pragma unroll
        for (int k = 0; k < 8; ++k) { const float d = f[r][q][k] - mean[r]; ss = fmaf(d, d, ss); }
      }
    }
    s[r] = ss;
  }
#pragma unroll
  for (int r = 0; r < R; ++r) {
    const float rstd = rsqrtf(wave_sum(s[r]) / (float)C + eps);
    if (lane == 0 && row0 + r < rows) *reinterpret_cast<float2*>(out + 2 * (row0 + r)) = make_float2(mean[r], rstd);
  }
}

template <typename T>
__global__ void __launch_bounds__(THREADS)
k_conv_in(const float* __restrict__ lat, const unsigned short* __restrict__ w, const float* __restrict__ bias,
          int B, int cin, int H, int W, int cout, int ldo, unsigned short* __restrict__ out) {
  extern __shared__ float wl[];
  const int kk = 9 * cin;
  for (int i = threadIdx.x; i < cout * kk; i += THREADS) {
    const int co = i / kk, k = i - co * kk;
    wl[((k * 2 + ((co >> 2) & 1)) * (cout / 8) + (co >> 3)) * 4 + (co & 3)] = T::to_f(w[i]);
  }
  __syncthreads();
  constexpr int PX = 4;
  const int cchunks = cout / 8;
  const int WQ = (W + PX - 1) / PX;
  const int total = B * H * WQ * cchunks;
  const int HWQ = H * WQ;
  for (int e = blockIdx.x * THREADS + threadIdx.x; e < total; e += gridDim.x * THREADS) {
    const int pq = e / cchunks, cc = e - pq * cchunks;
    const int b = pq / HWQ, rem = pq - b * HWQ;
    const int yh = rem / WQ, x0 = (rem - yh * WQ) * PX;
    float acc[PX][8];
    {
      const float4 b0 = *reinterpret_cast<const float4*>(bias + cc * 8), b1 = *reinterpret_cast<const float4*>(bias + cc * 8 + 4);
#pragma unroll
      for (int p = 0; p < PX; ++p) {
        acc[p][0] = b0.x; acc[p][1] = b0.y; acc[p][2] = b0.z; acc[p][3] = b0.w;
        acc[p][4] = b1.x; acc[p][5] = b1.y; acc[p][6] = b1.z; acc[p][7] = b1.w;
      }
    }
    const float* lb = lat + (long)b * cin * H * W;
    for (int c = 0; c < cin; ++c) {
      float v[3][PX + 2];
#pragma unroll
      for (int ty = 0; ty < 3; ++ty)
#pragma unroll
        for (int tx = 0; tx < PX + 2; ++tx) {
          const int iy = yh + ty - 1, ix = x0 + tx - 1;
          const bool ok = iy >= 0 && iy < H && ix >= 0 && ix < W;
          const float t = lb[((long)c * H + min(max(iy, 0), H - 1)) * W + min(max(ix, 0), W - 1)];
          v[ty][tx] = ok ? t : 0.f;
        }
#pragma unroll
      for (int tap = 0; tap < 9; ++tap) {
        const float4 w0 = *reinterpret_cast<const float4*>(&wl[(((tap * cin + c) * 2 + 0) * cchunks + cc) * 4]);
        const float4 w1 = *reinterpret_cast<const float4*>(&wl[(((tap * cin + c) * 2 + 1) * cchunks + cc) * 4]);
#pragma unroll
        for (int p = 0; p < PX; ++p) {
          const float x = v[tap / 3][tap % 3 + p];
          acc[p][0] = fmaf(x, w0.x, acc[p][0]); acc[p][1] = fmaf(x, w0.y, acc[p][1]);
          acc[p][2] = fmaf(x, w0.z, acc[p][2]); acc[p][3] = fmaf(x, w0.w, acc[p][3]);
          acc[p][4] = fmaf(x, w1.x, acc[p][4]); acc[p][5] = fmaf(x, w1.y, acc[p][5]);
          acc[p][6] = fmaf(x, w1.z, acc[p][6]); acc[p][7] = fmaf(x, w1.w, acc[p][7]);
        }
      }
    }
    const long pix0 = ((long)b * H + yh) * W + x0;
#pragma unroll
    for (int p = 0; p < PX; ++p)
      if (x0 + p < W) *reinterpret_cast<u32x4*>(out + (pix0 + p) * ldo + cc * 8) = pack8<T>(acc[p]);
  }
}

template <typename T>
__global__ void k_temb(float t_val, const float* __restrict__ t_dev, int B, int dim, unsigned short* __restrict__ out) {
  const float t = t_dev ? *t_dev : t_val;
  const int half = dim / 2;
  for (int i = blockIdx.x * blockDim.x + threadIdx.x; i < B * dim; i += gridDim.x * blockDim.x) {
    const int k = i % dim;
    const int kk = k < half ? k : k - half;
    const float f = expf(-9.210340371976184f * (float)kk / (float)half);
    const float a = t * f;
    const float v = k < half ? cosf(a) : sinf(a);
    out[i] = (unsigned short)(T::pack2(v, 0.f) & 0xffff);
  }
}

inline bool al16(const void* p) { return (reinterpret_cast<uintptr_t>(p) & 15) == 0; }


template <typename T>
int groupnorm_impl(const void* x, const void* x2, int32_t batch, int32_t hw, int32_t c1, int32_t c2, int32_t groups,
                   float eps, int32_t silu, const float* gamma, const float* beta, void* out, float* stats_ws,
                   void* stream, const float* cols1 = nullptr, const float* cols2 = nullptr) {
  if (!x || !gamma || !beta || !out || !stats_ws || batch < 0 || hw <= 0 || c1 <= 0 || c2 < 0 || groups <= 0 ||
      groups > 64)
    return SDN_E_INVALID;
  if (c2 > 0 && !x2) return SDN_E_INVALID;
  const int C = c1 + c2;
  if ((c1 & 7) || (c2 & 7) || C % groups != 0 || C > 4096) return SDN_E_INVALID;
  if (!al16(x) || (x2 && !al16(x2)) || !al16(out) || !al16(gamma) || !al16(beta)) return SDN_E_INVALID;
  if (batch == 0) return SDN_OK;
  const int cch = C / 8;
  int nch = (cch + THREADS - 1) / THREADS;
  while (cch % nch != 0) ++nch;
  const int ct = cch / nch;
  if (ct > THREADS) return SDN_E_INVALID;
  const int rt = THREADS / ct;
  int ntiles = (hw + 31) / 32;
  if (ntiles > GN_MAX_TILES) ntiles = GN_MAX_TILES;
  const int rows_per_tile = (hw + ntiles - 1) / ntiles;
  ntiles = (hw + rows_per_tile - 1) / rows_per_tile;
  hipStream_t st = (hipStream_t)stream;
  const size_t lds = (size_t)rt * C * 2 * sizeof(float);
  if (lds > 64 * 1024) return SDN_E_INVALID;
  if (cols1) {
    if ((hw & 127) || (c2 > 0 && !cols2)) return SDN_E_INVALID;
    record_norm_launch({2, T::kDtype, 0, 0, 0, 0, 0, 0, 0, 0, 1, 0});
    hipLaunchKernelGGL(k_gn_finalize_cols, dim3(batch, groups), dim3(256), 0, st, cols1, cols2, hw / 128, c1, c2, groups,
                       (float)hw * (float)(C / groups), eps, stats_ws);
  } else {
    float* partials = stats_ws + (size_t)batch * groups * 2;
    record_norm_launch({1, T::kDtype, 0, 0, nch, ct, ntiles, rows_per_tile, 0, 0, 0, 0});
    hipLaunchKernelGGL((k_gn_stats<T>), dim3(batch, ntiles), dim3(THREADS), lds, st, (const unsigned short*)x,
                       (const unsigned short*)x2, hw, c1, c2, groups, rows_per_tile, ct, nch, partials);
    hipLaunchKernelGGL(k_gn_finalize, dim3(batch), dim3(512), 0, st, partials, ntiles, groups,
                       (float)hw * (float)(C / groups), eps, stats_ws);
  }
  int rows_per_block = (256 * 8 * 16) / C;
  if (rows_per_block < 1) rows_per_block = 1;
  const int nblk = (hw + rows_per_block - 1) / rows_per_block;
  hipLaunchKernelGGL((k_gn_apply<T>), dim3(batch, nblk), dim3(THREADS), (size_t)2 * C * sizeof(float), st, (const unsigned short*)x,
                     (const unsigned short*)x2, hw, c1, c2, groups, rows_per_block, silu, gamma, beta, stats_ws,
                     (unsigned short*)out);
  return sdn_launch_status();
}

inline bool ln_width_ok(int c) { return c > 0 && !(c & 7) && (c <= 2048 || (c <= 2560 && c % 128 == 0)); }

template <typename T>
int layernorm_wide(const void* x, int64_t rows, int32_t c, float eps, const float* gamma, const float* beta, void* out, void* stream,
                   int mod, int rows_per_batch, int ld_mod) {
  hipLaunchKernelGGL((k_layernorm<T, 5, 1>), dim3((unsigned)((rows + 3) / 4)), dim3(THREADS), 0, (hipStream_t)stream,
                     (const unsigned short*)x, (long)rows, c, eps, gamma, beta, (unsigned short*)out, mod, rows_per_batch, ld_mod);
  record_norm_launch({mod ? 4 : 3, T::kDtype, 5, 1, 0, 0, 0, 0, 0, 0, 0, 0});
  return sdn_launch_status();
}
template <typename T>
int row_stats_wide(const void* x, int64_t rows, int32_t c, float eps, float* out, void* stream) {
  hipLaunchKernelGGL((k_row_stats<T, 5, 1>), dim3((unsigned)((rows + 3) / 4)), dim3(THREADS), 0, (hipStream_t)stream,
                     (const unsigned short*)x, (long)rows, c, eps, out);
  record_norm_launch({5, T::kDtype, 5, 1, 0, 0, 0, 0, 0, 0, 0, 0});
  return sdn_launch_status();
}

template <typename T>
int layernorm_impl(const void* x, int64_t rows, int32_t c, float eps, const float* gamma, const float* beta, void* out,
                   void* stream, int mod = 0, int rows_per_batch = 0, int ld_mod = 0) {
  if (!x || !gamma || !beta || !out || rows < 0 || !ln_width_ok(c)) return SDN_E_INVALID;
  if (!al16(x) || !al16(out) || !al16(gamma) || !al16(beta)) return SDN_E_INVALID;
  if (mod && (rows_per_batch <= 0 || ld_mod < c || (ld_mod & 3))) return SDN_E_INVALID;
  if (rows == 0) return SDN_OK;
  if (c > 2048) return layernorm_wide<T>(x, rows, c, eps, gamma, beta, out, stream, mod, rows_per_batch, ld_mod);
#define SDN_LN_LAUNCH(NQ, R)                                                                                          \
  do { hipLaunchKernelGGL((k_layernorm<T, NQ, R>), dim3((unsigned)((rows + 4 * (R) - 1) / (4 * (R)))), dim3(THREADS), 0,      \
                     (hipStream_t)stream, (const unsigned short*)x, (long)rows, c, eps, gamma, beta, (unsigned short*)out, \
                     mod, rows_per_batch, ld_mod);                                                                     \
  record_norm_launch({mod ? 4 : 3, T::kDtype, NQ, R, 0, 0, 0, 0, 0, 0, 0, 0}); } while (0)
  if (c <= 512) SDN_LN_LAUNCH(1, 4);
  else if (c <= 1024) SDN_LN_LAUNCH(2, 2);
  else SDN_LN_LAUNCH(4, 1);
#undef SDN_LN_LAUNCH
  return sdn_launch_status();
}

template <typename T>
__global__ void __launch_bounds__(THREADS)
k_patchify(const float* __restrict__ lat, int B, int C, int H, int W, int p, unsigned short* __restrict__ out) {
  const int hp = H / p, wp = W / p, K = C * p * p;
  const long total = (long)B * hp * wp * K;
  for (long e = (long)blockIdx.x * THREADS + threadIdx.x; e < total; e += (long)gridDim.x * THREADS) {
    const int k = (int)(e % K);
    const long tok = e / K;
    const int px = k % p, py = (k / p) % p, c = k / (p * p);
    const int tx = (int)(tok % wp), ty = (int)((tok / wp) % hp), b = (int)(tok / ((long)wp * hp));
    const float v = lat[(((long)b * C + c) * H + ty * p + py) * W + tx * p + px];
    out[e] = (unsigned short)(T::pack2(v, 0.f) & 0xffff);
  }
}
__global__ void __launch_bounds__(THREADS)
k_unpatchify(const float* __restrict__ tok, int B, int C, int H, int W, int p, float* __restrict__ out) {
  const int hp = H / p, wp = W / p;
  const long total = (long)B * C * H * W;
  for (long e = (long)blockIdx.x * THREADS + threadIdx.x; e < total; e += (long)gridDim.x * THREADS) {
    const int x = (int)(e % W), y = (int)((e / W) % H), c = (int)((e / ((long)W * H)) % C), b = (int)(e / ((long)W * H * C));
    const long t = ((long)b * hp + y / p) * wp + x / p;
    out[e] = tok[t * (p * p * C) + ((y % p) * p + (x % p)) * C + c];
  }
}
template <typename T>
int patchify_impl(const float* lat, int32_t B, int32_t C, int32_t H, int32_t W, int32_t p, void* out, void* stream) {
  if (!lat || !out || B < 0 || C <= 0 || H <= 0 || W <= 0 || p <= 0 || H % p || W % p) return SDN_E_INVALID;
  if (B == 0) return SDN_OK;
  const long total = (long)B * C * H * W;
  long grid = (total + THREADS - 1) / THREADS;
  if (grid > 2048) grid = 2048;
  hipLaunchKernelGGL((k_patchify<T>), dim3((unsigned)grid), dim3(THREADS), 0, (hipStream_t)stream, lat, B, C, H, W, p,
                     (unsigned short*)out);
  return sdn_launch_status();
}

template <typename T>
int conv_in_impl(const float* lat, const void* w, const float* bias, int32_t batch, int32_t cin, int32_t h, int32_t wd,
                 int32_t cout, void* out, void* stream) {
  if (!lat || !w || !bias || !out || batch < 0 || cin <= 0 || cin > 16 || h <= 0 || wd <= 0 || cout <= 0 ||
      (cout & 7) || !al16(out))
    return SDN_E_INVALID;
  if (batch == 0) return SDN_OK;
  int chunk = (int)((64 * 1024) / ((size_t)9 * cin * sizeof(float))) & ~7;
  if (chunk < 8) return SDN_E_INVALID;
  if (chunk > cout) chunk = cout;
  if ((long)batch * h * wd * (chunk / 8) >= (1L << 31)) return SDN_E_INVALID;
  for (int co0 = 0; co0 < cout; co0 += chunk) {
    const int cc = cout - co0 < chunk ? cout - co0 : chunk;
    const size_t lds = (size_t)cc * 9 * cin * sizeof(float);
    const long total = (long)batch * h * ((wd + 3) / 4) * (cc / 8);
    long grid = (total + THREADS - 1) / THREADS;
    if (grid > 4096) grid = 4096;
    hipLaunchKernelGGL((k_conv_in<T>), dim3((unsigned)grid), dim3(THREADS), lds, (hipStream_t)stream, lat,
                       (const unsigned short*)w + (size_t)co0 * 9 * cin, bias + co0, batch, cin, h, wd, cc, cout,
                       (unsigned short*)out + co0);
  }
  return sdn_launch_status();
}

template <typename T>
int temb_impl(float timestep, int32_t batch, int32_t dim, void* out, void* stream, const float* t_dev = nullptr) {
  if (!out || batch < 0 || dim <= 0 || (dim & 1)) return SDN_E_INVALID;
  if (batch == 0) return SDN_OK;
  const int n = batch * dim;
  hipLaunchKernelGGL((k_temb<T>), dim3((n + 255) / 256), dim3(256), 0, (hipStream_t)stream, timestep, t_dev, batch, dim,
                     (unsigned short*)out);
  return sdn_launch_status();
}

template <typename T>
int row_stats_impl(const void* x, int64_t rows, int32_t c, float eps, float* out, void* stream) {
  if (!x || !out || rows < 0 || !ln_width_ok(c) || !al16(x) || (reinterpret_cast<uintptr_t>(out) & 7)) return SDN_E_INVALID;
  if (rows == 0) return SDN_OK;
  if (c > 2048) return row_stats_wide<T>(x, rows, c, eps, out, stream);
#define SDN_RS_LAUNCH(NQ, R)                                                                                          \
  do { hipLaunchKernelGGL((k_row_stats<T, NQ, R>), dim3((unsigned)((rows + 4 * (R) - 1) / (4 * (R)))), dim3(THREADS), 0,      \
                     (hipStream_t)stream, (const unsigned short*)x, (long)rows, c, eps, out);                            \
  record_norm_launch({5, T::kDtype, NQ, R, 0, 0, 0, 0, 0, 0, 0, 0}); } while (0)
  if (c <= 512) SDN_RS_LAUNCH(1, 4);
  else if (c <= 1024) SDN_RS_LAUNCH(2, 2);
  else SDN_RS_LAUNCH(4, 1);
#undef SDN_RS_LAUNCH
  return sdn_launch_status();
}

}

int sdn_temb_from_device(int dtype, const float* t_dev, int batch, int dim, void* out, void* stream) {
  if (!t_dev) return SDN_E_INVALID;
  return dtype == 1 ? sdn_norm_detail::temb_impl<SdnF16>(0.f, batch, dim, out, stream, t_dev)
                    : sdn_norm_detail::temb_impl<SdnBF16>(0.f, batch, dim, out, stream, t_dev);
}
namespace { __global__ void k_set_scalar(float* dst, float v) { *dst = v; } }
int sdn_set_scalar(float* dst, float v, void* stream) {
  if (!dst) return SDN_E_INVALID;
  hipLaunchKernelGGL(k_set_scalar, dim3(1), dim3(1), 0, (hipStream_t)stream, dst, v);
  return sdn_launch_status();
}
using namespace sdn_norm_detail;

static int g_last_norm_launch[SDN_NL_COUNT] = {0};
void record_norm_launch(const sdn_norm_launch& l) {
  const int v[SDN_NL_COUNT] = {l.kernel, l.dtype, l.nq, l.r, l.nch, l.ct, l.ntiles, l.rows_per_tile, l.rpc, l.nchunk, l.stats_src, l.triple};
  for (int i = 0; i < SDN_NL_COUNT; ++i) g_last_norm_launch[i] = v[i];
}
extern "C" void sdn_debug_norm_last_launch(int* out, int n) {
  for (int i = 0; out && i < n; ++i) out[i] = i < SDN_NL_COUNT ? g_last_norm_launch[i] : 0;
}

#define SDN_NORM_ENTRY(SUF, T)                                                                                          \
  extern "C" int sdn_groupnorm_##SUF(const void* x, const void* x2, int32_t batch, int32_t hw, int32_t c1, int32_t c2, \
                                     int32_t groups, float eps, int32_t silu, const float* gamma, const float* beta,   \
                                     void* out, float* stats_ws, void* stream) {                                        \
    return groupnorm_impl<T>(x, x2, batch, hw, c1, c2, groups, eps, silu, gamma, beta, out, stats_ws, stream);         \
  }                                                                                                                     \
  extern "C" int sdn_groupnorm_cols_##SUF(const void* x, const void* x2, int32_t batch, int32_t hw, int32_t c1,         \
                                          int32_t c2, int32_t groups, float eps, int32_t silu, const float* gamma,      \
                                          const float* beta, void* out, float* stats_ws, const float* cols1,            \
                                          const float* cols2, void* stream) {                                           \
    if (!cols1) return SDN_E_INVALID;                                                                                   \
    return groupnorm_impl<T>(x, x2, batch, hw, c1, c2, groups, eps, silu, gamma, beta, out, stats_ws, stream, cols1,    \
                             cols2);                                                                                    \
  }                                                                                                                     \
  extern "C" int sdn_layernorm_##SUF(const void* x, int64_t rows, int32_t c, float eps, const float* gamma,            \
                                     const float* beta, void* out, void* stream) {                                      \
    return layernorm_impl<T>(x, rows, c, eps, gamma, beta, out, stream);                                                \
  }                                                                                                                     \
  extern "C" int sdn_layernorm_mod_##SUF(const void* x, int64_t rows, int32_t c, float eps, const float* scale,        \
                                         const float* shift, int32_t ld_mod, int32_t rows_per_batch, void* out,        \
                                         void* stream) {                                                                \
    return layernorm_impl<T>(x, rows, c, eps, scale, shift, out, stream, 1, rows_per_batch, ld_mod);                    \
  }                                                                                                                     \
  extern "C" int sdn_patchify_##SUF(const float* lat, int32_t B, int32_t C, int32_t H, int32_t W, int32_t p, void* out, \
                                    void* stream) {                                                                     \
    return patchify_impl<T>(lat, B, C, H, W, p, out, stream);                                                           \
  }                                                                                                                     \
  extern "C" int sdn_conv_in_##SUF(const float* lat, const void* w, const float* bias, int32_t batch, int32_t cin,     \
                                   int32_t h, int32_t wd, int32_t cout, void* out, void* stream) {                      \
    return conv_in_impl<T>(lat, w, bias, batch, cin, h, wd, cout, out, stream);                                         \
  }                                                                                                                     \
  extern "C" int sdn_timestep_embed_##SUF(float timestep, int32_t batch, int32_t dim, void* out, void* stream) {       \
    return temb_impl<T>(timestep, batch, dim, out, stream);                                                             \
  }
SDN_NORM_ENTRY(bf16, SdnBF16)
SDN_NORM_ENTRY(f16, SdnF16)

extern "C" int sdn_row_stats_bf16(const void* x, int64_t rows, int32_t c, float eps, float* out, void* stream) {
  return sdn_norm_detail::row_stats_impl<SdnBF16>(x, rows, c, eps, out, stream);
}
extern "C" int sdn_row_stats_f16(const void* x, int64_t rows, int32_t c, float eps, float* out, void* stream) {
  return sdn_norm_detail::row_stats_impl<SdnF16>(x, rows, c, eps, out, stream);
}

extern "C" int sdn_unpatchify_f32(const float* tok, int32_t B, int32_t C, int32_t H, int32_t W, int32_t p, float* out,
                                  void* stream) {
  if (!tok || !out || B < 0 || C <= 0 || H <= 0 || W <= 0 || p <= 0 || H % p || W % p) return SDN_E_INVALID;
  if (B == 0) return SDN_OK;
  const long total = (long)B * C * H * W;
  long grid = (total + THREADS - 1) / THREADS;
  if (grid > 2048) grid = 2048;
  hipLaunchKernelGGL(k_unpatchify, dim3((unsigned)grid), dim3(THREADS), 0, (hipStream_t)stream, tok, B, C, H, W, p, out);
  return sdn_launch_status();
}
```

### safe_denoiser_amd/csrc/sdn_plan.h

```cpp
#pragma once
#include <stdio.h>
#include <string.h>

#include <map>
#include <set>
#include <string>
#include <tuple>
#include <vector>

#include "sdn_common.h"
#include "sdn_ops.h"

namespace sdn_plan {

enum ModelKind { UNET, MMDIT, VAE_DECODER, VAE_ENCODER, CLIP, CLIP_PROJ, T5, CLIP_VISION, INCEPTION };

enum Space { SP_NONE = 0, SP_W = 1, SP_WS = 2, SP_IN = 3, SP_TEXT = 4, SP_OUT = 5, SP_POOLED = 6, SP_KV = 7, SP_OUT2 = 8 };
struct Ref { int space = SP_NONE; int64_t off = 0; };

struct Call {
  const void* weights; void* workspace; size_t workspace_bytes; int32_t batch; void* stream;
  const void *in = nullptr, *text = nullptr, *pooled = nullptr;
  void *out = nullptr, *out2 = nullptr;
  float scalar = 0.f; int n = 0;
  const int32_t* mask = nullptr;
  int64_t out_bs = 0, out_rs = 0, out2_rs = 0;
  int64_t kv_base = 0;
  int in_h = 0, in_w = 0;
  Call(const void* w, void* ws, size_t ws_bytes, int32_t b, void* s) : weights(w), workspace(ws), workspace_bytes(ws_bytes), batch(b), stream(s) {}
  const char* operator()(const Ref& r) const {
    switch (r.space) {
      case SP_W: return (const char*)weights + r.off;
      case SP_WS: return (const char*)workspace + r.off;
      case SP_KV: return (const char*)workspace + kv_base + r.off;
      case SP_IN: return (const char*)in + r.off;
      case SP_TEXT: return (const char*)text + r.off;
      case SP_OUT: return (const char*)out + r.off;
      case SP_OUT2: return (const char*)out2 + r.off;
      case SP_POOLED: return (const char*)pooled + r.off;
      default: return nullptr;
    }
  }
};

enum OpKind { OP_TEMB, OP_CONV_IN, OP_GEMM, OP_GN, OP_LN, OP_ATTN, OP_PATCHIFY, OP_UNPATCHIFY, OP_LATENT_MIX, OP_SOFTMAX,
              OP_TRANSPOSE, OP_REPEAT = 12 , OP_CLIP_EMBED, OP_MATTN,
              OP_ROWSTATS, OP_FFN, OP_SPLIT3,
              OP_RMSNORM, OP_EMBED, OP_T5_BIAS, OP_BATTN, OP_EOS_ROWS, OP_COPY_ROWS, OP_PATCH_ROWS, OP_VISION_EMBED, OP_CLASS_ROWS,
              OP_CONV_ROWS, OP_POOL3, OP_RESIZE, OP_SPATIAL_MEAN,
              OP_QK_RMSNORM  };

struct Op {
  int kind;
  sdn_gemm_desc gd;
  Ref a, a2, w, bias, rowbias, rowgate, residual, out, aux;
  Ref q2, k2, v2, out2;
  Ref col, cols1, cols2;
  Ref ln_c, ln_d, ln_stats;
  int ln = 0;
  int text_kv = 0;
  int x3t = 0;
  int pair_in = 0;
  int tri_out = 0;
  int dyn_ldc = 0;
  int k320 = 0;
  int n1 = 0, mod = 0, ld_mod = 0, patch = 0;
  int batch = 0, hw = 0, c1 = 0, c2 = 0, groups = 0, silu = 0;
  float eps = 0.f;
  int64_t rows = 0;
  int heads = 0, nq = 0, nk = 0, hd = 0, ldq = 0, ldk = 0, ldv = 0, ldo = 0;
  float scale = 0.f;
  Ref k, v;
  int kh = 0, kw = 0, sh = 0, sw = 0, ph = 0, pw = 0;
  char label[24] = {0};
  double flops = 0.0;
  double bytes = 0.0;
};

struct Arena {
  std::map<int64_t, int64_t> free_;
  int64_t top = 0, peak = 0;
  static int64_t up(int64_t v) { return (v + 255) & ~(int64_t)255; }
  int64_t alloc(int64_t bytes) {
    bytes = up(bytes);
    for (auto it = free_.begin(); it != free_.end(); ++it) {
      if (it->second >= bytes) {
        const int64_t off = it->first, rest = it->second - bytes;
        free_.erase(it);
        if (rest > 0) free_[off + bytes] = rest;
        return off;
      }
    }
    if (!free_.empty()) {
      auto last = std::prev(free_.end());
      if (last->first + last->second == top) {
        const int64_t off = last->first;
        free_.erase(last);
        top = off + bytes;
        if (top > peak) peak = top;
        return off;
      }
    }
    const int64_t off = top;
    top += bytes;
    if (top > peak) peak = top;
    return off;
  }
  void release(int64_t off, int64_t bytes) {
    bytes = up(bytes);
    auto it = free_.emplace(off, bytes).first;
    auto nx = std::next(it);
    if (nx != free_.end() && it->first + it->second == nx->first) { it->second += nx->second; free_.erase(nx); }
    if (it != free_.begin()) {
      auto pv = std::prev(it);
      if (pv->first + pv->second == it->first) { pv->second += it->second; free_.erase(it); }
    }
  }
};

struct Act {
  int64_t off = -1, bytes = 0; int C = 0, hw = 0, side = 0;
  int64_t content = 0;
  int64_t st_off = -1, st_bytes = 0;
};

struct Plan {
  int batch = 0;
  int64_t tscalar_off = -1;
  std::vector<Op> ops;
  int64_t ws_bytes = 0;
  int64_t kv_base = 0;
  double flops = 0.0, attn_flops = 0.0;
};

}

struct sdn_unet {
  sdn_plan::ModelKind kind = sdn_plan::UNET;
  sdn_unet_config cfg;
  sdn_mmdit_config mcfg;
  sdn_mmdit_ext mext = {0, 0.f, 0};
  sdn_vae_config vcfg;
  sdn_clip_config ccfg;
  sdn_clip_proj_config pcfg;
  sdn_t5_config tcfg;
  sdn_clip_vision_config vis;
  sdn_inception_config icfg;
  std::vector<sdn_inception_conv> convs;
  std::vector<sdn_param_info> params;
  std::map<std::string, int> param_index;
  int64_t weight_bytes = 0;
  std::map<int, sdn_plan::Plan> plans;
  int tproj_total = 0;
  int64_t subbatch_bytes = 0;
  bool profile_next = false;
  bool use_graph = false;
  bool gn_fuse = true;
  bool ln_fold = true;
  int ln_prepass_all = 0;
  bool ff_fuse = true;
  bool ffn_own_stats = true;
  bool ffn_fuse = true;
  struct FoldJob { int64_t w, gamma, beta, bias, wf, c, d; int rows, cols; int kind = 0; int group = 0; };
  std::vector<FoldJob> fold_jobs;
  uint64_t text_version = 0, kv_version = 0;
  int kv_batch = 0;
  const void *kv_w = nullptr, *kv_text = nullptr, *kv_ws = nullptr;
  bool x3_pairs = true;
  bool res_pre = true;
  bool gemm_k320 = true;
  bool x3_expand = true;
  bool split_k = false;
  bool conv_up4 = true;
  struct GraphKey {
    int batch; const void *w, *lat, *text, *pooled, *out, *ws;
    bool operator<(const GraphKey& o) const {
      return std::tie(batch, w, lat, text, pooled, out, ws) < std::tie(o.batch, o.w, o.lat, o.text, o.pooled, o.out, o.ws);
    }
  };
  std::map<GraphKey, hipGraphExec_t> graphs;
  hipStream_t cap_stream = nullptr;
  ~sdn_unet() {
    for (auto& kv : graphs) (void)hipGraphExecDestroy(kv.second);
    for (auto e : ev) (void)hipEventDestroy(e);
    if (cap_stream) (void)hipStreamDestroy(cap_stream);
  }
  std::vector<hipEvent_t> ev;
  int profiled_batch = 0;
  int profiled_n = 0;
  int dtype() const {
    switch (kind) {
      case sdn_plan::MMDIT: return mcfg.dtype;
      case sdn_plan::VAE_DECODER: case sdn_plan::VAE_ENCODER: return vcfg.dtype;
      case sdn_plan::CLIP: return ccfg.dtype;
      case sdn_plan::CLIP_PROJ: return pcfg.dtype;
      case sdn_plan::T5: return tcfg.dtype;
      case sdn_plan::CLIP_VISION: return vis.dtype;
      case sdn_plan::INCEPTION: return icfg.dtype;
      default: return cfg.dtype;
    }
  }
  bool is_vae() const { return kind == sdn_plan::VAE_DECODER || kind == sdn_plan::VAE_ENCODER; }
  bool is_clip() const { return kind == sdn_plan::CLIP || kind == sdn_plan::CLIP_PROJ; }
};

namespace sdn_plan {

constexpr bool kK320Plain = true, kK320Ln = true, kK320Rp = true;

struct GemmSpec {
  int64_t M; int N, K;
  Ref a, w, bias, out;
  Ref a2; int K1 = 0;
  Ref rowbias, rowgate; int rows_per_batch = 0, ld_row = 0;
  Ref residual; int residual_bcast = 0;
  int act = SDN_ACT_NONE, out_kind = SDN_OUT_BF16, n_valid = 0;
  Ref cols;
  bool res_pre = false;
  bool k320 = false;
  bool triple_out = false;
  bool pair_out = false;
  bool force_x3t = false;
  bool text_kv = false;
  bool dyn_ldc = false;
  bool f32_stream = false;
  GemmSpec(int64_t M_, int N_, int K_, Ref a_, Ref w_, Ref bias_, Ref out_) : M(M_), N(N_), K(K_), a(a_), w(w_), bias(bias_), out(out_) {}
  GemmSpec& with_a2(Ref v, int k1) { a2 = v; K1 = k1; return *this; }
  GemmSpec& with_rowbias(Ref v, int rpb, int ld) { rowbias = v; rows_per_batch = rpb; ld_row = ld; return *this; }
  GemmSpec& with_rowgate(Ref v, int rpb, int ld) { rowgate = v; rows_per_batch = rpb; ld_row = ld; return *this; }
  GemmSpec& with_residual(Ref v) { residual = v; return *this; }
  GemmSpec& with_residual_bcast(Ref v, int rpb) { residual = v; residual_bcast = 1; rows_per_batch = rpb; return *this; }
  GemmSpec& with_act(int v) { act = v; return *this; }
  GemmSpec& with_out_kind(int v) { out_kind = v; return *this; }
  GemmSpec& with_cols(Ref v) { cols = v; return *this; }
  GemmSpec& with_res_pre(bool v) { res_pre = v; return *this; }
  GemmSpec& with_k320(bool v) { k320 = v; return *this; }
  GemmSpec& with_triple_out(bool v) { triple_out = v; return *this; }
  GemmSpec& with_pair_out(bool v) { pair_out = v; return *this; }
  GemmSpec& with_force_x3t(bool v) { force_x3t = v; return *this; }
  GemmSpec& with_text_kv() { text_kv = true; return *this; }
  GemmSpec& with_dyn_ldc() { dyn_ldc = true; return *this; }
  GemmSpec& with_f32_stream(bool v) { f32_stream = v; return *this; }
};
struct ConvSpec {
  Act in; int cout, n_pad;
  Ref w, bias, out;
  int stride = 1, upsample = 0, asym_pad = 0;
  Ref rowbias; int ld_row = 0;
  Ref residual;
  int out_kind = SDN_OUT_BF16, n_valid = 0;
  Ref cols;
  bool res_pre = false;
  ConvSpec(const Act& in_, int cout_, Ref w_, Ref bias_, Ref out_) : in(in_), cout(cout_), n_pad(cout_), w(w_), bias(bias_), out(out_) {}
  ConvSpec& with_stride(int v, int asym = 0) { stride = v; asym_pad = asym; return *this; }
  ConvSpec& with_upsample() { upsample = 1; return *this; }
  ConvSpec& with_rowbias(Ref v, int ld) { rowbias = v; ld_row = ld; return *this; }
  ConvSpec& with_residual(Ref v) { residual = v; return *this; }
  ConvSpec& with_nchw_out(int n_pad_) { out_kind = SDN_OUT_F32_NCHW; n_valid = cout; n_pad = n_pad_; return *this; }
  ConvSpec& with_cols(Ref v) { cols = v; return *this; }
  ConvSpec& with_res_pre(bool v) { res_pre = v; return *this; }
};

struct Builder {
  sdn_unet* u;
  Plan* plan;
  Arena arena;
  int B;
  int seq = 0;
  int es = 2;
  bool x3t = false;
  bool x3t_hold = false;
  std::set<int64_t> tri;
  Ref tproj;
  int tproj_cursor = 0;
  Ref gn_stats;
  int64_t kv_top = 0;
  bool plan_bad = false;
  std::set<int64_t> pairs;
  struct Up4 { int64_t op; int64_t w9; int N, Cin; };
  std::vector<Up4> up4_pending;
  void finish_up4();
  struct Res { std::string pfx; int cout; };

  Ref param(const std::string& name, int kind, int rows, int cols, int rows_padded = 0);
  Ref stacked(const std::vector<std::pair<std::string, int>>& members, int cols);
  Ref stacked(const std::vector<std::string>& names, int rows_each, int cols);
  Ref derived(const std::string& name, int64_t bytes);
  Act act(int64_t rows, int C, int hw = 0, int side = 0, int esz = 0);
  Act act_gn(int64_t rows, int C, int hw, int side);
  static Ref stats_of(const Act& out) { return out.st_off >= 0 ? Ref{SP_WS, out.st_off} : Ref(); }
  void drop(Act& t);
  static Ref R(const Act& t) { return Ref{SP_WS, t.off}; }
  Ref x3_weight(Ref w, int rows, int cols, int group);
  Act split3(Ref a, Ref a2, int64_t rows, int c1, int c2, int hw = 0, int side = 0);
  bool x3t_on(const Ref& a) const { return x3t && !x3t_hold && a.space == SP_WS; }
  void emit(Op& o, bool attn = false);
  std::vector<Ref> derived_job(const std::vector<std::pair<std::string, int64_t>>& regions, sdn_unet::FoldJob job);
  void gemm(const GemmSpec& s);
  void push_gemm(Op& o, Ref cols);
  void conv3x3(const ConvSpec& s);
  void groupnorm(const Act& x, const Act* x2, float eps, int silu, Ref gamma, Ref beta, const Act& out);
  void layernorm(const Act& x, Ref gamma, Ref beta, const Act& out);
  void repeat(const Act& in, const Act& out, int rep);
  void attention(Ref q, Ref k, Ref v, Ref out, int nq, int nk, int C, int ldq, int ldk, int ldv, bool kv_pairs = false);

  std::vector<Ref> ln_fold_regions(const std::string& wname, Ref w, Ref gamma, Ref beta, Ref bias, int N, int K);
  void row_stats(Ref x, int64_t rows, int C, const Act& st);
  void gemm_ln(const GemmSpec& s, const std::string& wname, Ref gamma, Ref beta, bool prepass);
  Act resnet(const std::string& pfx, Act& x, Act* skip, int cout);
  Act transformer(const std::string& pfx, Act& x);
  void transformer_body(const std::string& pfx, Act& x, const Act& out, int64_t text_off, int rep = 1,
                        const Act* x_full = nullptr);
  std::vector<Res> enumerate_resnets() const;
  void build();

  void gemm_ex(const GemmSpec& s);
  void ln_mod(const Act& x, int64_t rows, int rows_per_batch, Ref scale, Ref shift, int ld, const Act& out);
  void qk_rmsnorm(const Act& qkv, int64_t rows, Ref wq, Ref wk);
  Ref fcol(int col) const { return Ref{SP_WS, tproj.off + (int64_t)col * 4}; }
  void build_mmdit();

  Act vae_resnet(const std::string& pfx, Act& x, int cout);
  Act vae_attention(const std::string& pfx, Act& x);
  void vae_f32_rows();
  void build_vae();
  void build_vae_encoder();

  void build_clip();
  Ref glu_pair(const std::string& value_name, const std::string& gate_name, int F, int K);
  void t5_gemm(const GemmSpec& s);
  void t5_rmsnorm(Ref x, bool x_f32, int64_t rows, int C, Ref w, Ref out);
  void build_t5();

  void build_clip_vision();

  void inception_conv(const std::string& name, const Act& in, int cout, int kh, int kw, int stride, int ph, int pw, const Act& out,
                      int c0);
  Act inception_conv_new(const std::string& name, const Act& in, int cout, int kh = 1, int kw = 1, int stride = 1, int ph = 0, int pw = 0);
  void inception_pool(int mode, const Act& in, int stride, int pad, const Act& out, int c0);
  void build_inception();
};

Plan* get_plan(sdn_unet* u, int batch, int n = 0);
int run_plan(sdn_unet* u, const Call& c);
void drop_graphs(sdn_unet* u);

}
```

### safe_denoiser_amd/csrc/sdn_plan_api.hip

```cpp
#include <algorithm>

#include "sdn_plan.h"

using namespace sdn_plan;

template <class F, class V> static void set_plan_toggle(sdn_unet* u, F sdn_unet::*field, V value) {
  u->*field = value;
  drop_graphs(u);
  u->plans.clear();
}

static void plain_chain_for_f32(sdn_unet* u, int dtype) { if (dtype >= 2) u->gn_fuse = u->ln_fold = u->ff_fuse = false; }

extern "C" {

int sdn_unet_create(const sdn_unet_config* cfg, sdn_unet** out) {
  if (!cfg || !out) return SDN_E_INVALID;
  if (cfg->n_levels < 1 || cfg->n_levels > 4 || cfg->layers_per_block < 1 || cfg->n_heads <= 0 ||
      cfg->in_channels <= 0 || cfg->in_channels > 16 || cfg->out_channels <= 0 || cfg->out_channels > 32 ||
      cfg->sample_size <= 0 || (cfg->sample_size % (1 << (cfg->n_levels - 1))) != 0 || cfg->cross_dim % 64 != 0 ||
      cfg->text_len <= 0 || cfg->norm_groups <= 0 || cfg->norm_groups > 64 || cfg->dtype < 0 || cfg->dtype > 3 ||
      cfg->latent_repeat < 0 || cfg->latent_repeat > 8)
    return SDN_E_INVALID;
  for (int i = 0; i < cfg->n_levels; ++i) {
// ... 185 lines not shown
    const int64_t cap = std::min<int64_t>(4, (((int64_t)1 << 31) - 1) / largest);
    return cap < 1 ? 0 : (int)cap;
  }
  int64_t cmax = 0;
  for (int i = 0; i < c.n_levels; ++i) if (c.block_out_channels[i] > cmax) cmax = c.block_out_channels[i];
  int64_t cap = (((int64_t)1 << 32) - 1) / (side * side * cmax * 2);
  if (cap > 8) cap = 8;
  return cap < 1 ? 0 : (int)cap;
}

size_t sdn_unet_workspace_bytes(sdn_unet* u, int32_t batch) {
  if (!u || batch <= 0) return 0;
  if (u->kind == T5) return sdn_t5_workspace_bytes(u, batch, 512);
  if (u->is_vae()) {
    const int cap = vae_chunk(u);
    if (cap == 0) return 0;
    if (batch > cap) batch = cap;
  }
  const int64_t b = get_plan(u, batch)->ws_bytes;
  return b < 0 ? 0 : (size_t)b;
}

double sdn_unet_flops(sdn_unet* u, int32_t batch, double* attn) {
  if (!u || batch <= 0) return 0.0;
  Plan* p = get_plan(u, batch);
  if (attn) *attn = p->attn_flops;
  return p->flops;
}

static int vae_run(sdn_unet* v, Call call, const float* in, int64_t in_n, float* out, int64_t out_n, int32_t batch) {
  if (batch < 0 || (batch > 0 && (!in || !out))) return SDN_E_INVALID;
  const int cap = vae_chunk(v);
  if (cap == 0) return SDN_E_INVALID;
  for (int lo = 0; lo < batch; lo += cap) {
    call.batch = batch - lo < cap ? batch - lo : cap;
    call.in = in + lo * in_n; call.out = out + lo * out_n;
    const int rc = run_plan(v, call);
    if (rc != SDN_OK) return rc;
  }
  return SDN_OK;
}

int sdn_vae_decode(sdn_unet* v, const void* weights, const float* latents, float latent_scale, float* image, int32_t batch,
                   void* workspace, size_t workspace_bytes, void* stream) {
  if (!v || v->kind != VAE_DECODER) return SDN_E_INVALID;
  const sdn_vae_config& c = v->vcfg;
  const int64_t side = (int64_t)c.sample_size << (c.n_levels - 1);
  Call call(weights, workspace, workspace_bytes, 0, stream);
  call.scalar = latent_scale;
  return vae_run(v, call, latents, (int64_t)c.latent_channels * c.sample_size * c.sample_size, image, (int64_t)c.out_channels * side * side, batch);
}

int sdn_vae_encode(sdn_unet* v, const void* weights, const float* image, float* moments, int32_t batch, void* workspace,
                   size_t workspace_bytes, void* stream) {
  if (!v || v->kind != VAE_ENCODER) return SDN_E_INVALID;
  const sdn_vae_config& c = v->vcfg;
  const int64_t side = (int64_t)c.sample_size << (c.n_levels - 1);
  return vae_run(v, Call(weights, workspace, workspace_bytes, 0, stream), image, (int64_t)c.out_channels * side * side, moments,
                 (int64_t)2 * c.latent_channels * c.sample_size * c.sample_size, batch);
}

int sdn_clip_forward(sdn_unet* m, const void* weights, const int32_t* input_ids, const int32_t* attention_mask,
                     void* last_hidden_state, int32_t batch, void* workspace, size_t workspace_bytes, void* stream) {
  if (!m || m->kind != CLIP || !input_ids || !last_hidden_state) return SDN_E_INVALID;
  Call call(weights, workspace, workspace_bytes, batch, stream);
  call.in = input_ids; call.mask = attention_mask; call.out = last_hidden_state;
  return run_plan(m, call);
}

int sdn_clip_proj_forward(sdn_unet* m, const void* weights, const int32_t* input_ids, void* hidden, int64_t hidden_batch_stride,
                          int64_t hidden_row_stride, void* text_embeds, int64_t embeds_row_stride, int32_t batch, void* workspace,
                          size_t workspace_bytes, void* stream) {
  if (!m || m->kind != CLIP_PROJ || !input_ids || !hidden || !text_embeds) return SDN_E_INVALID;
  const sdn_clip_proj_config& c = m->pcfg;
  if (hidden_row_stride < c.hidden_size || hidden_batch_stride < (int64_t)c.max_position_embeddings * hidden_row_stride ||
      embeds_row_stride < c.projection_dim || embeds_row_stride > 0x7fffffff || (hidden_row_stride & 7) || (hidden_batch_stride & 7) ||
      (embeds_row_stride & 7) || (reinterpret_cast<uintptr_t>(hidden) & 15) || (reinterpret_cast<uintptr_t>(text_embeds) & 15))
    return SDN_E_INVALID;
  Call call(weights, workspace, workspace_bytes, batch, stream);
  call.in = input_ids; call.out = hidden; call.out2 = text_embeds;
  call.out_bs = hidden_batch_stride; call.out_rs = hidden_row_stride; call.out2_rs = embeds_row_stride;
  return run_plan(m, call);
}

size_t sdn_t5_workspace_bytes(sdn_unet* m, int32_t batch, int32_t n) {
  if (!m || m->kind != T5 || batch <= 0 || batch > (1 << 20) || n < 2 || n > 512) return 0;
  const int64_t b = get_plan(m, batch, n)->ws_bytes;
  return b < 0 ? 0 : (size_t)b;
}

double sdn_t5_flops(sdn_unet* m, int32_t batch, int32_t n, double* attn) {
  if (!m || m->kind != T5 || batch <= 0 || batch > (1 << 20) || n < 2 || n > 512) return 0.0;
  Plan* p = get_plan(m, batch, n);
  if (attn) *attn = p->attn_flops;
  return p->flops;
}

int sdn_t5_forward(sdn_unet* m, const void* weights, const int32_t* input_ids, const int32_t* attention_mask, int32_t n,
                   void* out, int32_t batch, void* workspace, size_t workspace_bytes, void* stream) {
  if (!m || m->kind != T5 || n < 2 || n > 512 || batch > (1 << 20) || !input_ids || !out) return SDN_E_INVALID;
  Call call(weights, workspace, workspace_bytes, batch, stream);
  call.in = input_ids; call.mask = attention_mask; call.n = n; call.out = out;
  return run_plan(m, call);
}

int sdn_unet_forward(sdn_unet* u, const void* weights, const float* latents, float timestep, const void* text,
                     float* out, int32_t batch, void* workspace, size_t workspace_bytes, void* stream) {
  if (!u || u->kind != UNET || !latents || !text || !out) return SDN_E_INVALID;
  Call call(weights, workspace, workspace_bytes, batch, stream);
  call.in = latents; call.scalar = timestep; call.text = text; call.out = out;
  return run_plan(u, call);
}

int sdn_mmdit_forward(sdn_unet* u, const void* weights, const float* latents, float timestep, const void* text,
                      const void* pooled, float* out, int32_t batch, void* workspace, size_t workspace_bytes,
                      void* stream) {
  if (!u || u->kind != MMDIT || !latents || !text || !pooled || !out) return SDN_E_INVALID;
  Call call(weights, workspace, workspace_bytes, batch, stream);
  call.in = latents; call.scalar = timestep; call.text = text; call.pooled = pooled; call.out = out;
  return run_plan(u, call);
}

void sdn_unet_set_text_version(sdn_unet* u, uint64_t version) {
  if (!u) return;
  u->text_version = version;
  if (version == 0) u->kv_version = 0;
}

void sdn_unet_profile_next(sdn_unet* u) { if (u) u->profile_next = true; }

void sdn_unet_set_split_k(sdn_unet* u, int32_t on) {
  if (!u || u->kind == T5 || u->kind == CLIP_PROJ || u->kind == CLIP_VISION || u->split_k == (on != 0)) return;
  if (u->dtype() >= 2) return;
  set_plan_toggle(u, &sdn_unet::split_k, on != 0);
}

void sdn_unet_set_conv_up4(sdn_unet* u, int32_t on) {
  if (!u || u->kind != UNET || u->dtype() >= 2 || u->conv_up4 == (on != 0)) return;
  set_plan_toggle(u, &sdn_unet::conv_up4, on != 0);
}

void sdn_unet_set_graph_mode(sdn_unet* u, int32_t on) {
  if (!u) return;
  u->use_graph = on != 0;
  if (!on) drop_graphs(u);
}


void sdn_debug_set_x3_expand(sdn_unet* u, int on) { if (u && u->x3_expand != (on != 0)) set_plan_toggle(u, &sdn_unet::x3_expand, on != 0); }

void sdn_debug_set_res_pre(sdn_unet* u, int on) { if (u && u->res_pre != (on != 0)) set_plan_toggle(u, &sdn_unet::res_pre, on != 0); }

void sdn_debug_set_gemm_k320(sdn_unet* u, int on) { if (u && u->gemm_k320 != (on != 0)) set_plan_toggle(u, &sdn_unet::gemm_k320, on != 0); }

void sdn_debug_set_ln_fold(sdn_unet* u, int on) { if (u) set_plan_toggle(u, &sdn_unet::ln_fold, on != 0); }

void sdn_debug_set_ln_prepass_all(sdn_unet* u, int on) { if (u) set_plan_toggle(u, &sdn_unet::ln_prepass_all, on); }

void sdn_debug_set_ffn_fuse(sdn_unet* u, int on) { if (u) set_plan_toggle(u, &sdn_unet::ffn_fuse, on != 0); }

void sdn_debug_set_ff_fuse(sdn_unet* u, int on) { if (u) set_plan_toggle(u, &sdn_unet::ff_fuse, on != 0); }

void sdn_debug_set_ffn_own_stats(sdn_unet* u, int on) { if (u) set_plan_toggle(u, &sdn_unet::ffn_own_stats, on != 0); }

void sdn_debug_set_x3_pairs(sdn_unet* u, int on) { if (u) set_plan_toggle(u, &sdn_unet::x3_pairs, on != 0); }

void sdn_debug_set_gn_fuse(sdn_unet* u, int on) { if (u) set_plan_toggle(u, &sdn_unet::gn_fuse, on != 0); }

void sdn_debug_set_subbatch_bytes(sdn_unet* u, long long bytes) {
  if (u && u->kind != MMDIT) set_plan_toggle(u, &sdn_unet::subbatch_bytes, (int64_t)bytes);
}

}
```

### safe_denoiser_amd/csrc/sdn_plan_core.hip

```cpp
#include <math.h>

#include "sdn_plan.h"

namespace sdn_plan {

Ref Builder::param(const std::string& name, int kind, int rows, int cols, int rows_padded) {
  auto it = u->param_index.find(name);
  if (it != u->param_index.end()) return Ref{SP_W, u->params[it->second].offset};
  sdn_param_info pi;
  memset(&pi, 0, sizeof(pi));
  snprintf(pi.name, sizeof(pi.name), "%s", name.c_str());
  pi.kind = kind; pi.rows = rows; pi.cols = cols; pi.rows_padded = rows_padded > rows ? rows_padded : rows;
  const int64_t esz = (kind == SDN_P_VEC_F32 || kind == SDN_P_GEGLU_VEC) ? 4 : es;
  const int64_t bytes = (int64_t)pi.rows_padded * (cols > 0 ? cols : 1) * esz;
  pi.offset = u->weight_bytes;
  u->weight_bytes += (bytes + 255) & ~(int64_t)255;
  u->param_index[name] = (int)u->params.size();
  u->params.push_back(pi);
  return Ref{SP_W, pi.offset};
}
Ref Builder::stacked(const std::vector<std::pair<std::string, int>>& members, int cols) {
  Ref first;
  int64_t expect = -1;
  for (size_t i = 0; i < members.size(); ++i) {
    const int rows = members[i].second;
    Ref r = cols ? param(members[i].first, SDN_P_MAT, rows, cols) : param(members[i].first, SDN_P_VEC_F32, rows, 0);
    if (i == 0) first = r;
    else if (r.off != expect) { fprintf(stderr, "libsdn: stacked parameter %s is not contiguous\n", members[i].first.c_str()); abort(); }
    expect = r.off + (cols ? (int64_t)rows * cols * es : (int64_t)rows * 4);
  }
  return first;
}
Ref Builder::stacked(const std::vector<std::string>& names, int rows_each, int cols) {
  std::vector<std::pair<std::string, int>> members;
  for (const std::string& n : names) members.push_back({n, rows_each});
  return stacked(members, cols);
}
Ref Builder::derived(const std::string& name, int64_t bytes) {
  auto it = u->param_index.find(name);
  if (it != u->param_index.end()) return Ref{SP_W, u->params[it->second].offset};
  sdn_param_info pi; memset(&pi, 0, sizeof(pi));
  snprintf(pi.name, sizeof(pi.name), "%s", name.c_str());
  pi.kind = SDN_P_DERIVED; pi.rows = (int)bytes; pi.cols = 0; pi.rows_padded = (int)bytes;
  pi.offset = u->weight_bytes;
  u->weight_bytes += (bytes + 255) & ~(int64_t)255;
  u->param_index[name] = (int)u->params.size();
  u->params.push_back(pi);
  return Ref{SP_W, pi.offset};
}
std::vector<Ref> Builder::derived_job(const std::vector<std::pair<std::string, int64_t>>& regions, sdn_unet::FoldJob job) {
  const bool fresh = u->param_index.find(regions[0].first) == u->param_index.end();
  std::vector<Ref> r;
  for (const auto& g : regions) r.push_back(derived(g.first, g.second));
  if (fresh) {
    job.wf = r[0].off;
    if (r.size() > 1) job.c = r[1].off;
    if (r.size() > 2) job.d = r[2].off;
    u->fold_jobs.push_back(job);
  }
  return r;
}

Act Builder::act(int64_t rows, int C, int hw, int side, int esz) {
  const bool dflt = esz == 0;
  if (esz == 0) esz = es;
  Act t; t.content = rows * C * esz;
  t.bytes = (x3t && dflt) ? rows * C * 6 : t.content;
  t.off = arena.alloc(t.bytes); t.C = C; t.hw = hw; t.side = side; return t;
}
Act Builder::act_gn(int64_t rows, int C, int hw, int side) {
  Act t = act(rows, C, hw, side);
  if (u->gn_fuse && !u->split_k && hw > 0 && hw % 128 == 0) {
    t.st_bytes = ((rows + 127) / 128) * (int64_t)C * 8;
    t.st_off = arena.alloc(t.st_bytes);
  }
  return t;
}
void Builder::drop(Act& t) {
  if (t.off >= 0) { arena.release(t.off, t.bytes); tri.erase(t.off); pairs.erase(t.off); }
  if (t.st_off >= 0) arena.release(t.st_off, t.st_bytes);
  t.off = -1; t.st_off = -1;
}

Ref Builder::x3_weight(Ref w, int rows, int cols, int group) {
  return derived_job({{"x3@" + std::to_string((long long)w.off), (int64_t)rows * 3 * cols * 2}}, {w.off, -1, -1, -1, -1, -1, -1, rows, cols, 2, group})[0];
}
Act Builder::split3(Ref a, Ref a2, int64_t rows, int c1, int c2, int hw, int side) {
  Act t = act(rows, c1 + c2, hw, side);
  Op o; o.kind = OP_SPLIT3; o.a = a; o.a2 = a2; o.rows = rows; o.c1 = c1; o.c2 = c2; o.out = R(t);
  o.bytes = 10.0 * (double)rows * (c1 + c2);
  snprintf(o.label, sizeof(o.label), "k_split3");
  emit(o);
  tri.insert(t.off);
  return t;
}

void Builder::emit(Op& o, bool attn) {
  plan->ops.push_back(o);
  plan->flops += o.flops;
  if (attn || o.kind == OP_ATTN || o.kind == OP_MATTN || o.kind == OP_BATTN) plan->attn_flops += o.flops;
}
void Builder::gemm(const GemmSpec& s) {
  if (s.rowgate.space != SP_NONE || s.residual_bcast || s.f32_stream) plan_bad = true;
  const int64_t M = s.M; const int N = s.N, K = s.K, act_ = s.act;
  const Ref& residual = s.residual;
  Op o; o.kind = OP_GEMM; memset(&o.gd, 0, sizeof(o.gd));
  o.text_kv = s.text_kv; o.dyn_ldc = s.dyn_ldc;
  o.gd.M = (int)M; o.gd.N = N; o.gd.a_mode = SDN_A_PLAIN; o.gd.act = act_; o.gd.rows_per_batch = s.rows_per_batch; o.gd.ld_rowbias = s.ld_row;
  o.bias = s.bias; o.rowbias = s.rowbias; o.residual = residual; o.out = s.out;
  if ((x3t_on(s.a) || (s.force_x3t && x3t && !x3t_hold)) && (act_ == SDN_ACT_NONE || act_ == SDN_ACT_GEGLU) &&
      s.out_kind != SDN_OUT_F32_NCHW && s.n_valid == 0) {
    const bool two = s.a2.space != SP_NONE;
    Act tmp; Ref au = s.a;
    if (s.a.space != SP_WS || !tri.count(s.a.off)) { tmp = split3(s.a, s.a2, M, two ? s.K1 : K, two ? K - s.K1 : 0); au = R(tmp); }
    o.x3t = 1; o.gd.K = 3 * K; o.gd.out_kind = SDN_OUT_F32;
    const bool tri_o = s.triple_out && act_ == SDN_ACT_NONE;
    const bool pair_o = s.pair_out && act_ == SDN_ACT_NONE && !tri_o && residual.space == SP_NONE;
    o.gd.x3_out = act_ == SDN_ACT_GEGLU ? 2 : (tri_o ? 3 : (pair_o ? 4 : 1));
    if (pair_o && s.out.space == SP_WS) pairs.insert(s.out.off);
    o.a = au; o.w = x3_weight(s.w, N, K, K);
    o.flops = 2.0 * (double)M * (double)N * (double)K;
    o.bytes = 6.0 * ((double)M * K + (double)N * K) + 4.0 * (double)M * (act_ == SDN_ACT_GEGLU ? 0.75 * N : N) +
              (residual.space != SP_NONE ? 4.0 * (double)M * N : 0.0);
    snprintf(o.label, sizeof(o.label), "k_gemm<%d>x3", sdn_gemm_pick_tile((int)M, N, 3 * K, act_));
    push_gemm(o, s.cols);
    if ((act_ == SDN_ACT_GEGLU || tri_o) && s.out.space == SP_WS) tri.insert(s.out.off);
    if (tmp.off >= 0) drop(tmp);
    return;
  }
  if (s.triple_out || s.pair_out || s.force_x3t) plan_bad = true;
  const bool rp = s.res_pre && residual.space != SP_NONE && act_ == SDN_ACT_NONE && s.out_kind == SDN_OUT_BF16 && s.n_valid == 0 && es == 2;
  o.gd.res_pre = rp ? 1 : 0; o.gd.K = K; o.gd.K1 = s.K1; o.gd.out_kind = s.out_kind; o.gd.n_valid = s.n_valid;
  o.a = s.a; o.a2 = s.a2; o.w = s.w;
  o.flops = 2.0 * (double)M * (double)(s.n_valid > 0 ? s.n_valid : N) * (double)K;
  o.bytes = 2.0 * ((double)M * K + (double)N * K + (double)M * (act_ == SDN_ACT_GEGLU ? N / 2 : N)) +
            (residual.space != SP_NONE ? 2.0 * (double)M * N : 0.0);
  snprintf(o.label, sizeof(o.label), "k_gemm<%d>%s", sdn_gemm_pick_tile((int)M, N, K, act_, residual.space != SP_NONE && !rp), rp ? "/rp" : "");
  if (s.k320 && !x3t && K == 320 && N % 320 == 0 && act_ == SDN_ACT_NONE && s.out_kind == SDN_OUT_BF16 && s.n_valid == 0 && s.a2.space == SP_NONE &&
      s.rowbias.space == SP_NONE && (residual.space == SP_NONE || rp) && s.cols.space == SP_NONE && !u->split_k &&
      (rp ? kK320Rp : kK320Plain)) {
    o.k320 = 1;
    snprintf(o.label, sizeof(o.label), "k_gemm_k320%s", rp ? "/rp" : "");
  }
  push_gemm(o, s.cols);
}
void Builder::push_gemm(Op& o, Ref cols) {
  o.col = cols;
  const int nv = o.gd.n_valid > 0 ? o.gd.n_valid : o.gd.N;
  const int split = (!u->split_k || nv != o.gd.N || (o.gd.a_mode == SDN_A_CONV3X3 && o.gd.upsample == 2)) ? 1
                    : sdn_gemm_pick_split(o.gd.M, o.gd.N, o.gd.K, o.gd.act, o.gd.out_kind);
  if (split > 1) {
    const int64_t bytes = (int64_t)split * o.gd.M * o.gd.N * 4;
    const int64_t off = arena.alloc(bytes);
    o.gd.split_k = split; o.aux = Ref{SP_WS, off}; o.rows = bytes;
    arena.release(off, bytes);
    const size_t L = strlen(o.label);
    if (L + 3 < sizeof(o.label)) snprintf(o.label + L, sizeof(o.label) - L, "/s%d", split);
  }
  emit(o);
}
void Builder::conv3x3(const ConvSpec& s) {
  const Act& in = s.in;
  const int cout = s.cout, n_pad = s.n_pad, stride = s.stride, upsample = s.upsample, asym_pad = s.asym_pad;
  const Ref& residual = s.residual;
  const int Hi = upsample ? in.side * 2 : in.side;
  const int Ho = (Hi + (asym_pad ? 1 : 2) - 3) / stride + 1;
  Op o; o.kind = OP_GEMM; memset(&o.gd, 0, sizeof(o.gd));
  o.gd.M = B * Ho * Ho; o.gd.N = n_pad; o.gd.a_mode = SDN_A_CONV3X3;
  o.gd.Hs = in.side; o.gd.Ws = in.side; o.gd.Ho = Ho; o.gd.Wo = Ho; o.gd.stride = stride;
  o.gd.upsample = upsample; o.gd.asym_pad = asym_pad; o.gd.n_valid = s.n_valid; o.gd.rows_per_batch = Ho * Ho; o.gd.ld_rowbias = s.ld_row;
  o.bias = s.bias; o.rowbias = s.rowbias; o.residual = residual; o.out = s.out;
  if (x3t_on(R(in))) {
    Act tmp; Ref au = R(in);
    if (!tri.count(in.off)) { tmp = split3(R(in), Ref(), (int64_t)B * in.side * in.side, in.C, 0, in.hw, in.side); au = R(tmp); }
    o.x3t = 1;
    o.gd.K = 27 * in.C; o.gd.Cin = 3 * in.C;
    if (s.out_kind == SDN_OUT_F32_NCHW) { o.gd.out_kind = s.out_kind; o.gd.x3_out = 0; }
    else { o.gd.out_kind = SDN_OUT_F32; o.gd.x3_out = 1; }
    o.a = au; o.w = x3_weight(s.w, n_pad, 9 * in.C, in.C);
    o.flops = 2.0 * (double)o.gd.M * (double)cout * 9.0 * in.C;
    o.bytes = 6.0 * ((double)B * in.side * in.side * in.C + (double)n_pad * 9 * in.C) + 4.0 * (double)o.gd.M * cout +
              (residual.space != SP_NONE ? 4.0 * (double)o.gd.M * cout : 0.0);
    if (Ho == in.side && sdn_conv_slab_shape_ok(o.gd.M, n_pad, 3 * in.C, in.side, stride, upsample, asym_pad, SDN_OUT_BF16, s.n_valid) &&
        sdn_gemm_pick_tile(o.gd.M, n_pad, o.gd.K, SDN_ACT_NONE) == 10)
      snprintf(o.label, sizeof(o.label), "k_conv_slab<%d>/x3", in.side);
    else
      snprintf(o.label, sizeof(o.label), "k_gemm<%d>x3", sdn_gemm_pick_tile(o.gd.M, n_pad, o.gd.K, SDN_ACT_NONE));
    push_gemm(o, s.cols);
    if (tmp.off >= 0) drop(tmp);
    return;
  }
  o.gd.res_pre = (s.res_pre && residual.space != SP_NONE && s.out_kind == SDN_OUT_BF16 && s.n_valid == 0 && es == 2) ? 1 : 0;
  o.gd.K = 9 * in.C; o.gd.Cin = in.C; o.gd.out_kind = s.out_kind;
  o.a = R(in); o.w = s.w;
  o.flops = 2.0 * (double)o.gd.M * (double)cout * (double)o.gd.K;
  o.bytes = 2.0 * ((double)B * in.side * in.side * in.C + (double)n_pad * o.gd.K + (double)o.gd.M * cout) +
            (residual.space != SP_NONE ? 2.0 * (double)o.gd.M * cout : 0.0);
  const int up4 = (upsample == 1 && u->kind == UNET && es == 2 && stride == 1 && !asym_pad && s.out_kind == SDN_OUT_BF16 && s.n_valid == 0 &&
                   n_pad == cout && residual.space == SP_NONE && s.rowbias.space == SP_NONE && s.w.space == SP_W)
                      ? sdn_conv_up4_tile(in.side, in.side, in.C, n_pad) : 0;
  if (up4) {
    up4_pending.push_back({u->conv_up4 ? (int64_t)plan->ops.size() : -1, s.w.off, n_pad, in.C});
    if (u->conv_up4) {
      o.gd.K = 4 * in.C; o.gd.upsample = 2; o.gd.res_pre = 0;
      o.bytes = 2.0 * ((double)B * in.side * in.side * in.C + 4.0 * n_pad * o.gd.K + (double)o.gd.M * cout);
      snprintf(o.label, sizeof(o.label), "k_conv_up4<%d>", up4);
      push_gemm(o, s.cols);
      return;
    }
  }
  if (Ho == in.side && sdn_conv_slab_shape_ok(o.gd.M, n_pad, in.C, in.side, stride, upsample, asym_pad, s.out_kind, s.n_valid) &&
      sdn_gemm_pick_tile(o.gd.M, n_pad, o.gd.K, SDN_ACT_NONE) == 10)
    snprintf(o.label, sizeof(o.label), "k_conv_slab<%d>", in.side);
  else
    snprintf(o.label, sizeof(o.label), "k_gemm<%d>", sdn_gemm_pick_tile(o.gd.M, n_pad, o.gd.K, SDN_ACT_NONE));
  push_gemm(o, s.cols);
}
void Builder::finish_up4() {
  for (const Up4& p : up4_pending) {
    Ref d = derived_job({{"up4@" + std::to_string((long long)p.w9), (int64_t)16 * p.N * p.Cin * 2}}, {p.w9, -1, -1, -1, -1, -1, -1, p.N, p.Cin, 3})[0];
    if (p.op >= 0) plan->ops[(size_t)p.op].w = d;
  }
  up4_pending.clear();
}
void Builder::groupnorm(const Act& x, const Act* x2, float eps, int silu, Ref gamma, Ref beta, const Act& out) {
  Op o; o.kind = OP_GN; o.a = R(x); if (x2) o.a2 = R(*x2);
  o.batch = B; o.hw = x.hw; o.c1 = x.C; o.c2 = x2 ? x2->C : 0; o.groups = u->cfg.norm_groups; o.eps = eps;
  o.silu = silu; o.w = gamma; o.bias = beta; o.out = R(out); o.aux = gn_stats;
  if (x3t) { o.tri_out = 1; tri.insert(out.off); }
  if (x.st_off >= 0 && (!x2 || x2->st_off >= 0)) {
    o.cols1 = Ref{SP_WS, x.st_off};
    if (x2) o.cols2 = Ref{SP_WS, x2->st_off};
  }
  o.bytes = 2.0 * (o.cols1.space != SP_NONE ? 2.0 : 3.0) * (double)B * x.hw * (o.c1 + o.c2);
  snprintf(o.label, sizeof(o.label), o.cols1.space != SP_NONE ? "k_gn_apply" : "k_gn_stats+apply");
  emit(o);
}
void Builder::layernorm(const Act& x, Ref gamma, Ref beta, const Act& out) {
  Op o; o.kind = OP_LN; o.a = R(x); o.rows = (int64_t)B * x.hw; o.c1 = x.C; o.eps = 1e-5f; o.w = gamma; o.bias = beta;
  o.out = R(out);
  if (x3t) { o.tri_out = 1; tri.insert(out.off); }
  o.bytes = 2.0 * 2.0 * (double)o.rows * x.C;
  snprintf(o.label, sizeof(o.label), "k_layernorm");
  emit(o);
}
void Builder::repeat(const Act& in, const Act& out, int rep) {
  Op o; o.kind = OP_REPEAT; o.a = R(in); o.out = R(out); o.rows = in.content; o.c1 = rep;
  o.bytes = (double)in.content * (1 + rep);
  snprintf(o.label, sizeof(o.label), "k_repeat");
  emit(o);
}
void Builder::attention(Ref q, Ref k, Ref v, Ref out, int nq, int nk, int C, int ldq, int ldk, int ldv, bool kv_pairs) {
  Op o; o.kind = OP_ATTN; o.a = q; o.k = k; o.v = v; o.out = out; o.batch = B; o.heads = u->cfg.n_heads;
  o.nq = nq; o.nk = nk; o.hd = C / u->cfg.n_heads; o.ldq = ldq; o.ldk = ldk; o.ldv = ldv; o.ldo = C;
  o.scale = 1.0f / sqrtf((float)o.hd);
  if (x3t && out.space == SP_WS) { o.tri_out = 1; tri.insert(out.off); }
  if (q.space == SP_WS && pairs.count(q.off)) {
    o.pair_in = kv_pairs ? 2 : 1; pairs.erase(q.off);
  } else if (kv_pairs) {
    plan_bad = true;
  }
  o.flops = 4.0 * (double)B * o.heads * (double)nq * (double)nk * (double)o.hd;
  o.bytes = 2.0 * (double)B * C * (2.0 * nq + 2.0 * nk);
  snprintf(o.label, sizeof(o.label), "k_attn<%d>", o.hd);
  emit(o);
}

Plan* get_plan(sdn_unet* u, int batch, int n) {
  if (u->kind == T5 && n == 0) n = 512;
  const int key = u->kind == T5 ? batch * 1024 + n : batch;
  auto it = u->plans.find(key);
  if (it != u->plans.end()) return &it->second;
  if (u->kind == T5 && u->plans.size() >= 64) {
    u->plans.clear();
    u->profiled_batch = 0;
  }
  Plan& p = u->plans[key];
  p.batch = batch;
  Builder b{u, &p};
  b.B = batch;
  b.seq = n;
  b.es = u->dtype() >= 2 ? 4 : 2;
  b.x3t = u->kind == UNET && u->dtype() == 3 && u->x3_expand;
  switch (u->kind) {
    case UNET: b.build(); break;
    case MMDIT: b.build_mmdit(); break;
    case VAE_DECODER: b.build_vae(); break;
    case VAE_ENCODER: b.build_vae_encoder(); break;
    case CLIP: case CLIP_PROJ: b.build_clip(); break;
    case T5: b.build_t5(); break;
    case CLIP_VISION: b.build_clip_vision(); break;
    case INCEPTION: b.build_inception(); break;
  }
  if (b.plan_bad) p.ws_bytes = -1;
  return &p;
}

}
```

### safe_denoiser_amd/csrc/sdn_plan_run.hip

```cpp
#include "sdn_plan.h"

namespace sdn_plan {

static long g_x3_chunk_limit = (1L << 31) - 4096;
extern "C" void sdn_debug_set_x3_chunk_bytes(long long bytes) { g_x3_chunk_limit = bytes > 0 ? (long)bytes : (1L << 31) - 4096; }

static int launch_x3t_gemm(const Op& o, const char* a, const char* w, const float* bias, const float* rowbias, const char* residual,
                           void* out, void* stream) {
  const sdn_gemm_desc& d = o.gd;
  const bool conv = d.a_mode == SDN_A_CONV3X3;
  const long rows_out_unit = conv ? (long)d.Ho * d.Wo : 256;
  const long a_bytes_unit = conv ? (long)d.Hs * d.Ws * d.Cin * 2 : 256L * d.K * 2;
  const long units = conv ? d.M / rows_out_unit : (d.M + 255) / 256;
  long per = g_x3_chunk_limit / a_bytes_unit;
  if (per < 1) return SDN_E_INVALID;
  if (per > units) per = units;
  if (per < units) {
    const long n = (units + per - 1) / per;
    long even = (units + n - 1) / n;
    const int nrep = sdn_gemm_pick_tile((int)(even * rows_out_unit < d.M ? even * rows_out_unit : d.M), d.N, d.K, d.act, 0);
    const long tile_rows = nrep >= 8 ? 256 : 128, tile_cols = 32L * (nrep > 0 ? nrep : 2);
    const long tiles_per_unit = ((rows_out_unit + tile_rows - 1) / tile_rows) * ((d.N + tile_cols - 1) / tile_cols);
    long a_ = 256, b_ = tiles_per_unit % 256;
    while (b_) { const long t_ = a_ % b_; a_ = b_; b_ = t_; }
// ... 22 lines not shown
}

static int launch_op_f32(const sdn_unet* u, const Op& o, const Call& P, bool x3, const float* t_dev, void* stream) {
  int rc = SDN_OK;
  switch (o.kind) {
    case OP_TEMB:
      rc = sdn_temb_f32(P.scalar, t_dev, o.batch, o.c1, (void*)P(o.out), stream);
      break;
    case OP_CONV_IN:
      rc = sdn_conv_in_f32((const float*)P(o.a), P(o.w), (const float*)P(o.bias), o.batch, o.c1, o.hw, o.hw, o.c2, (void*)P(o.out), stream);
      break;
    case OP_GEMM:
      if (o.x3t) { rc = launch_x3t_gemm(o, P(o.a), P(o.w), (const float*)P(o.bias), (const float*)P(o.rowbias), P(o.residual), (void*)P(o.out), stream); break; }
      if (o.dyn_ldc) {
        sdn_gemm_desc gd = o.gd; gd.ldc = (int)P.out2_rs;
        rc = (x3 ? sdn_gemm_x3 : sdn_gemm_f32)(&gd, P(o.a), nullptr, P(o.w), nullptr, nullptr, nullptr, nullptr, (void*)P(o.out), stream);
        break;
      }
      rc = (o.ln || o.gd.split_k > 1) ? SDN_E_INVALID
           : (x3 ? sdn_gemm_x3 : sdn_gemm_f32)(&o.gd, P(o.a), P(o.a2), P(o.w), (const float*)P(o.bias), (const float*)P(o.rowbias),
                                               (const float*)P(o.rowgate), P(o.residual), (void*)P(o.out), stream);
      break;
    case OP_QK_RMSNORM:
      rc = sdn_qk_rmsnorm(2, (void*)P(o.a), o.rows, o.heads, o.ldq, (const float*)P(o.w), (const float*)P(o.bias), o.eps, stream);
      break;
    case OP_SPLIT3:
      rc = sdn_split3((const float*)P(o.a), (const float*)P(o.a2), o.rows, o.c1, o.c2, (void*)P(o.out), stream);
      break;
    case OP_GN:
      rc = (o.tri_out ? sdn_groupnorm_f32_triple : sdn_groupnorm_f32)(P(o.a), P(o.a2), o.batch, o.hw, o.c1, o.c2, o.groups, o.eps, o.silu,
                                                                     (const float*)P(o.w), (const float*)P(o.bias), (void*)P(o.out),
                                                                     (float*)P(o.aux), stream);
      break;
    case OP_LN:
      if (o.mod) {
        rc = o.tri_out ? SDN_E_INVALID
                       : sdn_layernorm_mod_f32(P(o.a), o.rows, o.c1, o.eps, (const float*)P(o.w), (const float*)P(o.bias), o.ld_mod,
                                               o.hw, (void*)P(o.out), stream);
        break;
      }
      rc = (o.tri_out ? sdn_layernorm_f32_triple : sdn_layernorm_f32)(P(o.a), o.rows, o.c1, o.eps, (const float*)P(o.w),
                                                                      (const float*)P(o.bias), (void*)P(o.out), stream);
      break;
    case OP_PATCHIFY:
      rc = sdn_patchify_f32((const float*)P(o.a), o.batch, o.c1, o.hw, o.hw, o.patch, (void*)P(o.out), stream);
      break;
    case OP_UNPATCHIFY:
      rc = sdn_unpatchify_f32((const float*)P(o.a), o.batch, o.c1, o.hw, o.hw, o.patch, (float*)P(o.out), stream);
      break;
    case OP_ATTN:
      if (o.pair_in == 1) {
        rc = sdn_attention_x3_pairs(P(o.a), P(o.a) + (size_t)o.ldo * 2, P(o.a) + (size_t)o.ldo * 4, o.ldq, o.ldq, (void*)P(o.out), o.batch, o.heads,
                                    o.nq, o.nk, o.hd, 2 * o.ldq, 2 * o.ldk, 2 * o.ldv, o.ldo, o.scale, o.tri_out, stream);
        break;
      }
      if (o.pair_in == 2) {
        rc = sdn_attention_x3_pairs(P(o.a), P(o.k), P(o.k) + (size_t)o.ldo * 2, o.ldq, o.ldk, (void*)P(o.out), o.batch, o.heads,
                                    o.nq, o.nk, o.hd, 2 * o.ldq, 2 * o.ldk, 2 * o.ldv, o.ldo, o.scale, o.tri_out, stream);
        break;
      }
      if (o.n1 > 0) {
        sdn_attn_segment2 s2{P(o.q2), P(o.k2), P(o.v2), (void*)P(o.out2), o.n1, o.ldq, o.ldk, o.ldv, o.ldo};
        rc = o.tri_out ? SDN_E_INVALID
                       : sdn_joint_attention_f32(x3 ? 1 : 0, P(o.a), P(o.k), P(o.v), (void*)P(o.out), &s2, o.batch, o.heads, o.nq, o.hd,
                                                 o.ldq, o.ldk, o.ldv, o.ldo, o.scale, stream);
        break;
      }
      rc = (o.tri_out ? sdn_attention_x3_triple : (x3 ? sdn_attention_x3 : sdn_attention_f32))(
          P(o.a), P(o.k), P(o.v), (void*)P(o.out), o.batch, o.heads, o.nq, o.nk, o.hd, o.ldq, o.ldk, o.ldv, o.ldo, o.scale, stream);
      break;
    case OP_REPEAT:
      rc = sdn_repeat(P(o.a), (size_t)o.rows, o.c1, (void*)P(o.out), stream);
      break;
    case OP_CLIP_EMBED:
      rc = sdn_clip_embed_f32((const int32_t*)P(o.a), P(o.w), P(o.bias), o.rows, o.hw, o.c1, o.c2, (void*)P(o.out), stream);
      break;
    case OP_EOS_ROWS:
      rc = sdn_clip_eos_rows(2, (const int32_t*)P(o.a), P(o.k), (const float*)P(o.w), (const float*)P(o.bias), o.batch, o.hw, o.c1, o.c2,
                             u->pcfg.eos_token_id, o.eps, (void*)P(o.out), nullptr, stream);
      break;
    case OP_COPY_ROWS:
      rc = sdn_copy_rows_strided(P(o.a), o.batch, o.hw, o.c1, 4, (void*)P(o.out), P.out_bs, P.out_rs, stream);
      break;
    case OP_CONV_ROWS:
      rc = sdn_patch_rows_f32((const float*)P(o.a), o.batch, o.hw, o.hw, o.c1, o.kh, o.kw, o.sh, o.sw, o.ph, o.pw, o.c2, (float*)P(o.out), stream);
      break;
    case OP_POOL3:
      rc = sdn_pool3_f32(o.mod, (const float*)P(o.a), o.batch, o.hw, o.hw, o.c1, o.sh, o.ph, (float*)P(o.out), o.ldo, o.c2, stream);
      break;
    case OP_RESIZE:
      rc = sdn_resize_bilinear_f32((const float*)P(o.a), o.batch, P.in_h, P.in_w, o.hw, o.hw, o.scale, o.eps, (float*)P(o.out), stream);
      break;
    case OP_SPATIAL_MEAN:
      rc = sdn_spatial_mean_f32((const float*)P(o.a), o.batch, o.hw, o.c1, (float*)P(o.out), stream);
      break;
    case OP_LATENT_MIX:
      rc = sdn_latent_mix((const float*)P(o.a), (const float*)P(o.w), (const float*)P(o.bias), o.batch, o.c1, o.hw,
                          o.mod ? o.scale : P.scalar , (float*)P(o.out), stream);
      break;
    case OP_SOFTMAX:
      rc = sdn_softmax_rows(2, (const float*)P(o.a), o.c1, o.rows, o.c1, o.scale, (void*)P(o.out), o.c1, stream);
      break;
    case OP_TRANSPOSE:
      rc = sdn_transpose32(P(o.a), (int)o.rows, o.c1, o.ldq, (void*)P(o.out), o.ldo, stream);
      break;
    case OP_MATTN:
      rc = sdn_masked_attention_f32(P(o.a), P(o.k), P(o.v), (void*)P(o.out), P.mask, 1, o.batch, o.heads,
                                    o.nq, o.hd, o.ldq, o.ldk, o.ldv, o.ldo, o.scale, stream);
      break;
    default:
      rc = SDN_E_INVALID;
  }
  return rc;
}

static int launch_op_16(const sdn_unet* u, const Op& o, const Call& P, bool f16, const float* t_dev, void* stream) {
  int rc = SDN_OK;
  switch (o.kind) {
    case OP_TEMB:
      if (t_dev) rc = sdn_temb_from_device(f16 ? 1 : 0, t_dev, o.batch, o.c1, (void*)P(o.out), stream);
      else rc = (f16 ? sdn_timestep_embed_f16 : sdn_timestep_embed_bf16)(P.scalar, o.batch, o.c1, (void*)P(o.out), stream);
      break;
    case OP_CONV_IN:
      rc = (f16 ? sdn_conv_in_f16 : sdn_conv_in_bf16)((const float*)P(o.a), P(o.w), (const float*)P(o.bias), o.batch, o.c1, o.hw, o.hw, o.c2,
                            (void*)P(o.out), stream);
      break;
    case OP_ROWSTATS:
      rc = (f16 ? sdn_row_stats_f16 : sdn_row_stats_bf16)(P(o.a), o.rows, o.c1, o.eps, (float*)P(o.out), stream);
      break;
    case OP_FFN:
      rc = sdn_ffn_geglu_fused(f16 ? 1 : 0, o.rows, o.c1, P(o.a), (const float*)P(o.ln_stats), P(o.w), (const float*)P(o.ln_c),
                               (const float*)P(o.ln_d), P(o.a2), (const float*)P(o.bias), P(o.residual), (void*)P(o.out),
                               o.col.space != SP_NONE ? (float*)P(o.col) : nullptr, stream);
      break;
    case OP_EOS_ROWS:
      rc = sdn_clip_eos_rows(f16 ? 1 : 0, (const int32_t*)P(o.a), P(o.k), (const float*)P(o.w), (const float*)P(o.bias), o.batch, o.hw,
                             o.c1, o.c2, u->pcfg.eos_token_id, o.eps, (void*)P(o.out), nullptr, stream);
      break;
    case OP_COPY_ROWS:
      rc = sdn_copy_rows_strided(P(o.a), o.batch, o.hw, o.c1, 2, (void*)P(o.out), P.out_bs, P.out_rs, stream);
      break;
    case OP_PATCH_ROWS:
      rc = sdn_clip_patch_rows(f16 ? 1 : 0, (const float*)P(o.a), o.batch, o.hw, o.patch, o.c1, (void*)P(o.out), stream);
      break;
    case OP_VISION_EMBED:
      rc = sdn_clip_vision_embed(f16 ? 1 : 0, P(o.a), (const float*)P(o.a2), P(o.aux), (const float*)P(o.w), (const float*)P(o.bias), o.batch,
                                 o.hw, o.c1, o.eps, (void*)P(o.out), stream);
      break;
    case OP_CLASS_ROWS:
      rc = sdn_clip_class_rows(f16 ? 1 : 0, P(o.a), (const float*)P(o.w), (const float*)P(o.bias), o.batch, o.hw, o.c1, o.eps,
                               (void*)P(o.out), stream);
      break;
    case OP_GEMM:
      if (o.k320) {
        rc = sdn_gemm_k320(f16 ? 1 : 0, &o.gd, P(o.a), P(o.w), o.ln ? nullptr : (const float*)P(o.bias), o.ln ? (const float*)P(o.ln_c) : nullptr,
                           o.ln ? (const float*)P(o.ln_d) : nullptr, o.eps, o.ln ? nullptr : P(o.residual), (void*)P(o.out), stream);
        break;
      }
      if (o.dyn_ldc) {
        sdn_gemm_desc gd = o.gd; gd.ldc = (int)P.out2_rs;
        rc = (f16 ? sdn_gemm_f16 : sdn_gemm_bf16)(&gd, P(o.a), nullptr, P(o.w), nullptr, nullptr, nullptr, nullptr, (void*)P(o.out), stream);
        break;
      }
      if (o.ln) {
        rc = (f16 ? sdn_gemm_ln_f16 : sdn_gemm_ln_bf16)(&o.gd, P(o.a), P(o.w), (const float*)P(o.ln_c), (const float*)P(o.ln_d), o.eps,
                                                        (const float*)P(o.ln_stats), (void*)P(o.out), stream);
        break;
      }
      if (o.col.space != SP_NONE && o.gd.split_k <= 1) {
        rc = (f16 ? sdn_gemm_stats_f16 : sdn_gemm_stats_bf16)(&o.gd, P(o.a), P(o.a2), P(o.w), (const float*)P(o.bias),
                                                              (const float*)P(o.rowbias), P(o.residual), (void*)P(o.out),
                                                              (float*)P(o.col), stream);
        break;
      }
      if (o.gd.split_k > 1) {
        rc = (f16 ? sdn_gemm_splitk_f16 : sdn_gemm_splitk_bf16)(&o.gd, P(o.a), P(o.a2), P(o.w), (const float*)P(o.bias),
                                                                (const float*)P(o.rowbias), (const float*)P(o.rowgate), P(o.residual),
                                                                (void*)P(o.out), (void*)P(o.aux), (size_t)o.rows, stream);
        break;
      }
      rc = (f16 ? sdn_gemm_f16 : sdn_gemm_bf16)(&o.gd, P(o.a), P(o.a2), P(o.w), (const float*)P(o.bias), (const float*)P(o.rowbias),
                         (const float*)P(o.rowgate), P(o.residual), (void*)P(o.out), stream);
      break;
    case OP_GN:
      if (o.cols1.space != SP_NONE) {
        rc = (f16 ? sdn_groupnorm_cols_f16 : sdn_groupnorm_cols_bf16)(P(o.a), P(o.a2), o.batch, o.hw, o.c1, o.c2, o.groups, o.eps,
                                                                      o.silu, (const float*)P(o.w), (const float*)P(o.bias),
                                                                      (void*)P(o.out), (float*)P(o.aux), (const float*)P(o.cols1),
                                                                      (const float*)P(o.cols2), stream);
        break;
      }
      rc = (f16 ? sdn_groupnorm_f16 : sdn_groupnorm_bf16)(P(o.a), P(o.a2), o.batch, o.hw, o.c1, o.c2, o.groups, o.eps, o.silu,
                              (const float*)P(o.w), (const float*)P(o.bias), (void*)P(o.out), (float*)P(o.aux), stream);
      break;
    case OP_CLIP_EMBED:
      rc = sdn_clip_embed(f16 ? 1 : 0, (const int32_t*)P(o.a), P(o.w), P(o.bias), o.rows, o.hw, o.c1, o.c2, (void*)P(o.out), stream);
      break;
    case OP_MATTN:
      rc = sdn_masked_attention(f16 ? 1 : 0, P(o.a), P(o.k), P(o.v), (void*)P(o.out), P.mask, 1, o.batch,
                                o.heads, o.nq, o.hd, o.ldq, o.ldk, o.ldv, o.ldo, o.scale, stream);
      break;
    case OP_RMSNORM:
      rc = sdn_rmsnorm(f16 ? 1 : 0, P(o.a), o.mod, o.rows, o.c1, o.eps, (const float*)P(o.w), (void*)P(o.out), stream);
      break;
    case OP_QK_RMSNORM:
      rc = sdn_qk_rmsnorm(f16 ? 1 : 0, (void*)P(o.a), o.rows, o.heads, o.ldq, (const float*)P(o.w), (const float*)P(o.bias), o.eps, stream);
      break;
    case OP_EMBED:
      rc = sdn_embed_tokens(f16 ? 1 : 0, (const int32_t*)P(o.a), P(o.w), o.rows, o.c1, o.c2, (float*)P(o.out), stream);
      break;
    case OP_T5_BIAS:
      rc = sdn_t5_relative_bias(f16 ? 1 : 0, P(o.w), u->tcfg.num_buckets, u->tcfg.max_distance, o.heads, o.nq, (float*)P(o.out), stream);
      break;
    case OP_BATTN:
      rc = sdn_bias_attention(f16 ? 1 : 0, P(o.a), P(o.k), P(o.v), (void*)P(o.out), (const float*)P(o.aux), P.mask,
                              o.batch, o.heads, o.nq, o.hd, o.ldq, o.ldk, o.ldv, o.ldo, o.scale, stream);
      break;
    case OP_REPEAT:
      rc = sdn_repeat(P(o.a), (size_t)o.rows, o.c1, (void*)P(o.out), stream);
      break;
    case OP_LATENT_MIX:
      rc = sdn_latent_mix((const float*)P(o.a), (const float*)P(o.w), (const float*)P(o.bias), o.batch, o.c1, o.hw,
                          o.mod ? o.scale : P.scalar ,
                          (float*)P(o.out), stream);
      break;
    case OP_SOFTMAX:
      rc = sdn_softmax_rows(f16 ? 1 : 0, (const float*)P(o.a), o.c1, o.rows, o.c1, o.scale, (void*)P(o.out), o.c1, stream);
      break;
    case OP_TRANSPOSE:
      rc = sdn_transpose16(P(o.a), (int)o.rows, o.c1, o.ldq, (void*)P(o.out), o.ldo, stream);
      break;
    case OP_PATCHIFY:
      rc = (f16 ? sdn_patchify_f16 : sdn_patchify_bf16)((const float*)P(o.a), o.batch, o.c1, o.hw, o.hw, o.patch,
                                                        (void*)P(o.out), stream);
      break;
    case OP_UNPATCHIFY:
      rc = sdn_unpatchify_f32((const float*)P(o.a), o.batch, o.c1, o.hw, o.hw, o.patch, (float*)P(o.out), stream);
      break;
    case OP_LN:
      if (o.mod) {
        rc = (f16 ? sdn_layernorm_mod_f16 : sdn_layernorm_mod_bf16)(P(o.a), o.rows, o.c1, o.eps, (const float*)P(o.w),
                                                                    (const float*)P(o.bias), o.ld_mod, o.hw,
                                                                    (void*)P(o.out), stream);
        break;
      }
      rc = (f16 ? sdn_layernorm_f16 : sdn_layernorm_bf16)(P(o.a), o.rows, o.c1, o.eps, (const float*)P(o.w), (const float*)P(o.bias),
                              (void*)P(o.out), stream);
      break;
    case OP_ATTN:
      if (o.n1 > 0) {
        sdn_attn_segment2 s2{P(o.q2), P(o.k2), P(o.v2), (void*)P(o.out2), o.n1, o.ldq, o.ldk, o.ldv, o.ldo};
        rc = sdn_joint_attention(f16 ? 1 : 0, P(o.a), P(o.k), P(o.v), (void*)P(o.out), &s2, o.batch, o.heads, o.nq, o.hd,
                                 o.ldq, o.ldk, o.ldv, o.ldo, o.scale, stream);
        break;
      }
      rc = (f16 ? sdn_attention_f16 : sdn_attention_bf16)(P(o.a), P(o.k), P(o.v), (void*)P(o.out), o.batch, o.heads, o.nq, o.nk, o.hd, o.ldq,
                              o.ldk, o.ldv, o.ldo, o.scale, stream);
      break;
    default:
      rc = SDN_E_INVALID;
  }
  return rc;
}

static int launch_ops(sdn_unet* u, const Plan* p, const Call& c, const float* t_dev, bool prof, void* stream, bool skip_text_kv = false) {
  const int sdt = u->dtype();
  const bool f32 = sdt >= 2;
  for (size_t opi = 0; opi < p->ops.size(); ++opi) {
    const Op& o = p->ops[opi];
    if ((skip_text_kv && o.text_kv) || (o.kind == OP_COPY_ROWS && !c.out)) continue;
    if (prof) (void)hipEventRecord(u->ev[2 * opi], (hipStream_t)stream);
    const int rc = f32 ? launch_op_f32(u, o, c, sdt == 3, t_dev, stream) : launch_op_16(u, o, c, sdt == 1, t_dev, stream);
    if (prof) (void)hipEventRecord(u->ev[2 * opi + 1], (hipStream_t)stream);
    if (rc != SDN_OK) return rc;
  }
  return SDN_OK;
}

int run_plan(sdn_unet* u, const Call& given) {
  if (!u || !given.weights || !given.workspace || given.batch <= 0) return SDN_E_INVALID;
  Plan* p = get_plan(u, given.batch, given.n);
  if (p->ws_bytes < 0) return SDN_E_INVALID;
  if (given.workspace_bytes < (size_t)p->ws_bytes) return SDN_E_WORKSPACE;
  Call c = given; c.kv_base = p->kv_base;
  const bool prof = u->profile_next;
  if (prof) {
    u->profile_next = false;
    while (u->ev.size() < 2 * p->ops.size()) { hipEvent_t e; if (hipEventCreate(&e) != hipSuccess) return SDN_E_LAUNCH; u->ev.push_back(e); }
    u->profiled_batch = c.batch; u->profiled_n = c.n;
  }
  hipStream_t hs = (hipStream_t)c.stream;
  if (u->use_graph && !prof && (u->kind == UNET || u->kind == MMDIT) && p->tscalar_off >= 0) {
    hipStreamCaptureStatus cs = hipStreamCaptureStatusNone;
    if (hipStreamIsCapturing(hs, &cs) == hipSuccess && cs == hipStreamCaptureStatusNone) {
      float* t_dev = (float*)((char*)c.workspace + p->tscalar_off);
      int rc = sdn_set_scalar(t_dev, c.scalar, c.stream);
      if (rc != SDN_OK) return rc;
      const sdn_unet::GraphKey key{c.batch, c.weights, c.in, c.text, c.pooled, c.out, c.workspace};
      auto it = u->graphs.find(key);
      if (it == u->graphs.end()) {
        if (u->graphs.size() >= 16) {
          (void)hipStreamSynchronize(hs);
          for (auto& kv : u->graphs) (void)hipGraphExecDestroy(kv.second);
          u->graphs.clear();
        }
        hipGraph_t graph = nullptr;
        if (!u->cap_stream && hipStreamCreateWithFlags(&u->cap_stream, hipStreamNonBlocking) != hipSuccess) return SDN_E_LAUNCH;
        if (hipStreamBeginCapture(u->cap_stream, hipStreamCaptureModeThreadLocal) != hipSuccess) return SDN_E_LAUNCH;
        rc = launch_ops(u, p, c, t_dev, false, (void*)u->cap_stream);
        const hipError_t ec = hipStreamEndCapture(u->cap_stream, &graph);
        if (rc != SDN_OK || ec != hipSuccess || !graph) { if (graph) (void)hipGraphDestroy(graph); return rc != SDN_OK ? rc : SDN_E_LAUNCH; }
        hipGraphExec_t exec = nullptr;
        const hipError_t ei = hipGraphInstantiate(&exec, graph, nullptr, nullptr, 0);
        (void)hipGraphDestroy(graph);
        if (ei != hipSuccess || !exec) return SDN_E_LAUNCH;
        it = u->graphs.emplace(key, exec).first;
      }
      u->kv_version = 0;
      return hipGraphLaunch(it->second, hs) == hipSuccess ? SDN_OK : SDN_E_LAUNCH;
    }
  }
  const bool declared = u->kind == UNET && u->text_version != 0 && u->subbatch_bytes == 0;
  const bool skip = declared && !prof && u->kv_version == u->text_version && u->kv_batch == c.batch && u->kv_w == c.weights &&
                    u->kv_text == c.text && u->kv_ws == c.workspace;
  const int rc_l = launch_ops(u, p, c, nullptr, prof, c.stream, skip);
  if (rc_l == SDN_OK && declared) { u->kv_version = u->text_version; u->kv_batch = c.batch; u->kv_w = c.weights; u->kv_text = c.text; u->kv_ws = c.workspace; }
  else if (!declared) u->kv_version = 0;
  return rc_l;
}

void drop_graphs(sdn_unet* u) {
  if (u->graphs.empty()) return;
  (void)hipDeviceSynchronize();
  for (auto& kv : u->graphs) (void)hipGraphExecDestroy(kv.second);
  u->graphs.clear();
}

// ... 84 lines not shown
```

### safe_denoiser_amd/csrc/sdn_plan_unet.hip

```cpp
#include <math.h>

#include "sdn_plan.h"

namespace sdn_plan {

std::vector<Ref> Builder::ln_fold_regions(const std::string& wname, Ref w, Ref gamma, Ref beta, Ref bias, int N, int K) {
  return derived_job({{wname + "#ln", (int64_t)N * K * 2}, {wname + "#ln_c", (int64_t)N * 4}, {wname + "#ln_d", (int64_t)N * 4}},
                     {w.off, gamma.off, beta.off, bias.space == SP_NONE ? -1 : bias.off, -1, -1, -1, N, K});
}
void Builder::row_stats(Ref x, int64_t rows, int C, const Act& st) {
  Op o; o.kind = OP_ROWSTATS; o.a = x; o.rows = rows; o.c1 = C; o.eps = 1e-5f; o.out = R(st);
  o.bytes = 2.0 * rows * C; snprintf(o.label, sizeof(o.label), "k_row_stats");
  emit(o);
}
void Builder::gemm_ln(const GemmSpec& s, const std::string& wname, Ref gamma, Ref beta, bool prepass) {
  if (s.cols.space != SP_NONE || s.a2.space != SP_NONE || s.residual.space != SP_NONE || s.rowbias.space != SP_NONE || s.rowgate.space != SP_NONE ||
      s.out_kind != SDN_OUT_BF16 || s.n_valid || s.res_pre || s.triple_out || s.pair_out || s.force_x3t || s.text_kv || s.dyn_ldc || s.f32_stream)
    plan_bad = true;
  const int64_t rows = s.M; const int N = s.N, K = s.K;
  const std::vector<Ref> f = ln_fold_regions(wname, s.w, gamma, beta, s.bias, N, K);
  Act st;
  if (prepass) { st = act(rows, 2, 0, 0, 4); row_stats(s.a, rows, K, st); }
  Op o; o.kind = OP_GEMM; memset(&o.gd, 0, sizeof(o.gd));
  o.gd.M = (int)rows; o.gd.N = N; o.gd.K = K; o.gd.a_mode = SDN_A_PLAIN; o.gd.act = s.act; o.gd.out_kind = SDN_OUT_BF16;
  o.a = s.a; o.w = f[0]; o.out = s.out; o.ln = 1; o.ln_c = f[1]; o.ln_d = f[2]; o.eps = 1e-5f;
  if (prepass) o.ln_stats = R(st);
  o.flops = 2.0 * (double)rows * N * K;
  o.bytes = 2.0 * ((double)rows * K + (double)N * K + (double)rows * (s.act == SDN_ACT_GEGLU ? N / 2 : N));
  { int t = sdn_gemm_pick_tile((int)rows, N, K, s.act);
    if (t == 8 && N % 320 == 0) t = 10;
    snprintf(o.label, sizeof(o.label), "k_gemm<%d>/ln%d", t, prepass ? 2 : 1); }
  if (s.k320 && !prepass && K == 320 && N % 320 == 0 && s.act == SDN_ACT_NONE && kK320Ln) {
    o.k320 = 1;
    snprintf(o.label, sizeof(o.label), "k_gemm_k320/ln1");
  }
  emit(o);
  if (prepass) drop(st);
}

Act Builder::resnet(const std::string& pfx, Act& x, Act* skip, int cout) {
  const int cin = x.C + (skip ? skip->C : 0);
  Ref n1g = param(pfx + ".norm1.weight", SDN_P_VEC_F32, cin, 0), n1b = param(pfx + ".norm1.bias", SDN_P_VEC_F32, cin, 0);
  Ref c1w = param(pfx + ".conv1.weight", SDN_P_CONV3X3, cout, 9 * cin), c1b = param(pfx + ".conv1.bias", SDN_P_VEC_F32, cout, 0);
  const int tcol = tproj_cursor; tproj_cursor += cout;
  Ref n2g = param(pfx + ".norm2.weight", SDN_P_VEC_F32, cout, 0), n2b = param(pfx + ".norm2.bias", SDN_P_VEC_F32, cout, 0);
  Ref c2w = param(pfx + ".conv2.weight", SDN_P_CONV3X3, cout, 9 * cout), c2b = param(pfx + ".conv2.bias", SDN_P_VEC_F32, cout, 0);
  const int64_t rows = (int64_t)B * x.hw;
  Act g1 = act(rows, cin, x.hw, x.side);
  groupnorm(x, skip, 1e-5f, 1, n1g, n1b, g1);
  Act h = act_gn(rows, cout, x.hw, x.side);
  conv3x3(ConvSpec(g1, cout, c1w, c1b, R(h)).with_rowbias(Ref{SP_WS, tproj.off + (int64_t)tcol * 4}, u->tproj_total).with_cols(stats_of(h)));
  drop(g1);
  Act g2 = act(rows, cout, x.hw, x.side);
  groupnorm(h, nullptr, 1e-5f, 1, n2g, n2b, g2);
  drop(h);
  Act out = act_gn(rows, cout, x.hw, x.side);
  Act sc;
  if (cin != cout) {
    Ref scw = param(pfx + ".conv_shortcut.weight", SDN_P_MAT, cout, cin), scb = param(pfx + ".conv_shortcut.bias", SDN_P_VEC_F32, cout, 0);
    sc = act(rows, cout, x.hw, x.side);
    gemm(GemmSpec(rows, cout, cin, R(x), scw, scb, R(sc)).with_a2(skip ? R(*skip) : Ref(), skip ? x.C : 0));
  }
  conv3x3(ConvSpec(g2, cout, c2w, c2b, R(out)).with_residual(cin != cout ? R(sc) : R(x)).with_res_pre(u->res_pre).with_cols(stats_of(out)));
  drop(sc); drop(g2);
  return out;
}

Act Builder::transformer(const std::string& pfx, Act& x) {
  const int64_t bytes_full = (int64_t)B * x.hw * x.C * es;
  int nsub = 1;
  if (u->subbatch_bytes > 0)
    while (nsub < B && bytes_full / nsub > u->subbatch_bytes && B % (nsub * 2) == 0) nsub *= 2;
  Act out = nsub == 1 ? act_gn((int64_t)B * x.hw, x.C, x.hw, x.side) : act((int64_t)B * x.hw, x.C, x.hw, x.side);
  const int Bfull = B, Bs = B / nsub;
  for (int sb = 0; sb < nsub; ++sb) {
    B = Bs;
    Act xs = x, os = out;
    xs.off += (int64_t)sb * Bs * x.hw * x.C * es; os.off += (int64_t)sb * Bs * x.hw * x.C * es;
    transformer_body(pfx, xs, os, (int64_t)sb * Bs * u->cfg.text_len * u->cfg.cross_dim * es);
  }
  B = Bfull;
  return out;
}

void Builder::transformer_body(const std::string& pfx, Act& x, const Act& out, int64_t text_off, int rep,
                               const Act* x_full) {
  const int C = x.C, hw = x.hw, T = u->cfg.text_len, X = u->cfg.cross_dim;
  const int Bfull = B;
  B = Bfull / rep;
  int64_t rows = (int64_t)B * hw;
  const std::string tb = pfx + ".transformer_blocks.0";
  Ref ng = param(pfx + ".norm.weight", SDN_P_VEC_F32, C, 0), nb = param(pfx + ".norm.bias", SDN_P_VEC_F32, C, 0);
  Ref piw = param(pfx + ".proj_in.weight", SDN_P_MAT, C, C), pib = param(pfx + ".proj_in.bias", SDN_P_VEC_F32, C, 0);
  Ref l1g = param(tb + ".norm1.weight", SDN_P_VEC_F32, C, 0), l1b = param(tb + ".norm1.bias", SDN_P_VEC_F32, C, 0);
  Ref qkv = stacked({tb + ".attn1.to_q.weight", tb + ".attn1.to_k.weight", tb + ".attn1.to_v.weight"}, C, C);
  Ref o1w = param(tb + ".attn1.to_out.0.weight", SDN_P_MAT, C, C), o1b = param(tb + ".attn1.to_out.0.bias", SDN_P_VEC_F32, C, 0);
  Ref l2g = param(tb + ".norm2.weight", SDN_P_VEC_F32, C, 0), l2b = param(tb + ".norm2.bias", SDN_P_VEC_F32, C, 0);
  Ref q2w = param(tb + ".attn2.to_q.weight", SDN_P_MAT, C, C);
  Ref kv2 = stacked({tb + ".attn2.to_k.weight", tb + ".attn2.to_v.weight"}, C, X);
  Ref o2w = param(tb + ".attn2.to_out.0.weight", SDN_P_MAT, C, C), o2b = param(tb + ".attn2.to_out.0.bias", SDN_P_VEC_F32, C, 0);
  Ref l3g = param(tb + ".norm3.weight", SDN_P_VEC_F32, C, 0), l3b = param(tb + ".norm3.bias", SDN_P_VEC_F32, C, 0);
  Ref f1w = param(tb + ".ff.net.0.proj.weight", SDN_P_GEGLU_MAT, 8 * C, C), f1b = param(tb + ".ff.net.0.proj.bias", SDN_P_GEGLU_VEC, 8 * C, 0);
  Ref f2w = param(tb + ".ff.net.2.weight", SDN_P_MAT, C, 4 * C), f2b = param(tb + ".ff.net.2.bias", SDN_P_VEC_F32, C, 0);
  Ref pow_ = param(pfx + ".proj_out.weight", SDN_P_MAT, C, C), pob = param(pfx + ".proj_out.bias", SDN_P_VEC_F32, C, 0);

  Act gn = act(rows, C, hw, x.side);
  groupnorm(x, nullptr, 1e-6f, 0, ng, nb, gn);
  Act h = act(rows, C, hw, x.side);
  const bool k320 = u->gemm_k320 && C == 320 && es == 2 && !x3t && u->subbatch_bytes == 0;
  gemm(GemmSpec(rows, C, C, R(gn), piw, pib, R(h)).with_k320(k320));
  drop(gn);
  const bool fold12 = u->ln_fold && C <= 640, fold3 = u->ln_fold && C == 320;
  const int hd = C / u->cfg.n_heads;
  const bool x3p = x3t && u->x3_pairs && (hd == 40 || hd == 80 || hd == 160);
  const bool x3p_self = x3p && (int64_t)hw * 6 * C * 2 < (1LL << 31), x3p_cross = x3p && u->subbatch_bytes == 0;
  Act ln;
  auto ln_gemm = [&](bool fold, const Act& in, const char* wname, Ref g, Ref b, bool prepass, GemmSpec s) {
    if (fold) { s.a = R(in); gemm_ln(s, tb + wname, g, b, prepass); }
    else { layernorm(in, g, b, ln); s.a = R(ln); gemm(s); }
  };
  if (!fold12 || !fold3) ln = act(rows, C, hw, x.side);
  Act qkvb = act(rows, 3 * C, hw, x.side);
  ln_gemm(fold12, h, ".attn1.to_q.weight", l1g, l1b, 3 * C > 960 || u->ln_prepass_all,
          GemmSpec(rows, 3 * C, C, Ref(), qkv, Ref(), R(qkvb)).with_k320(k320).with_pair_out(!fold12 && x3p_self));
  Act at = act(rows, C, hw, x.side);
  attention(R(qkvb), Ref{SP_WS, qkvb.off + (int64_t)C * es}, Ref{SP_WS, qkvb.off + (int64_t)2 * C * es}, R(at), hw, hw, C,
            3 * C, 3 * C, 3 * C);
  drop(qkvb);
  Act h2 = act(rows, C, hw, x.side);
  gemm(GemmSpec(rows, C, C, R(at), o1w, o1b, R(h2)).with_residual(R(h)).with_res_pre(u->res_pre).with_k320(k320));
  drop(h);
  Act qb = act(rows, C, hw, x.side);
  ln_gemm(fold12, h2, ".attn2.to_q.weight", l2g, l2b, u->ln_prepass_all != 0,
          GemmSpec(rows, C, C, Ref(), q2w, Ref(), R(qb)).with_k320(k320).with_pair_out(!fold12 && x3p_cross));
  if (rep > 1) {
    if (ln.off >= 0) drop(ln);
    drop(at);
    B = Bfull; rows = (int64_t)B * hw;
    Act h2f = act(rows, C, hw, x.side), qbf = act(rows, C, hw, x.side);
    repeat(h2, h2f, rep); repeat(qb, qbf, rep);
    const bool q_is_pairs = pairs.count(qb.off) > 0;
    drop(h2); drop(qb);
    h2 = h2f; qb = qbf;
    if (q_is_pairs) pairs.insert(qb.off);
    if (!fold3) ln = act(rows, C, hw, x.side);
    at = act(rows, C, hw, x.side);
  }
  if (u->subbatch_bytes > 0) {
    Act kvb = act((int64_t)B * T, 2 * C);
    gemm(GemmSpec((int64_t)B * T, 2 * C, X, Ref{SP_TEXT, text_off}, kv2, Ref(), R(kvb)));
    attention(R(qb), R(kvb), Ref{SP_WS, kvb.off + (int64_t)C * es}, R(at), hw, T, C, C, 2 * C, 2 * C);
    drop(qb); drop(kvb);
  } else {
    const Ref kvr{SP_KV, kv_top};
    kv_top += Arena::up((int64_t)B * T * 2 * C * es);
    gemm(GemmSpec((int64_t)B * T, 2 * C, X, Ref{SP_TEXT, text_off}, kv2, Ref(), kvr).with_text_kv().with_force_x3t(x3p_cross).with_pair_out(x3p_cross));
    attention(R(qb), kvr, Ref{SP_KV, kvr.off + (int64_t)C * es}, R(at), hw, T, C, C, 2 * C, 2 * C, x3p_cross);
    drop(qb);
  }
  Act h3 = act(rows, C, hw, x.side);
  gemm(GemmSpec(rows, C, C, R(at), o2w, o2b, R(h3)).with_residual(R(h2)).with_res_pre(u->res_pre).with_k320(k320));
  drop(h2); drop(at);
  const Ref xres = R(rep > 1 ? *x_full : x);
  auto ff_pair = [&] {
    return derived_job({{pfx + ".proj_out.weight#ff", (int64_t)C * 5 * C * 2}, {pfx + ".proj_out.bias#ff", (int64_t)C * 4}},
                       {f2w.off, pow_.off, f2b.off, pob.off, -1, -1, -1, C, 4 * C, 1});
  };
  if (fold3 && u->ff_fuse && u->ffn_fuse && C == 320) {
    if (ln.off >= 0) drop(ln);
    const std::vector<Ref> f1 = ln_fold_regions(tb + ".ff.net.0.proj.weight", f1w, l3g, l3b, f1b, 8 * C, C), f2 = ff_pair();
    Act st;
    if (!u->ffn_own_stats) { st = act(rows, 2, 0, 0, 4); row_stats(R(h3), rows, C, st); }
    Op o; o.kind = OP_FFN; o.a = R(h3); if (st.off >= 0) o.ln_stats = R(st); o.w = f1[0]; o.ln_c = f1[1]; o.ln_d = f1[2]; o.a2 = f2[0]; o.bias = f2[1];
    o.residual = xres; o.out = R(out); o.rows = rows; o.c1 = C;
    o.col = stats_of(out);
    o.flops = 2.0 * (double)rows * ((double)8 * C * C + (double)C * 5 * C);
    o.bytes = 2.0 * ((double)rows * C * 3 + (double)8 * C * C + (double)5 * C * C);
    snprintf(o.label, sizeof(o.label), "k_ffn320");
    emit(o);
    if (st.off >= 0) drop(st);
    drop(h3);
    return;
  }
  Act ff = act(rows, 4 * C, hw, x.side);
  ln_gemm(fold3, h3, ".ff.net.0.proj.weight", l3g, l3b, !u->ffn_own_stats, GemmSpec(rows, 8 * C, C, Ref(), f1w, f1b, R(ff)).with_act(SDN_ACT_GEGLU));
  if (ln.off >= 0) drop(ln);
  if (u->ff_fuse) {
    const std::vector<Ref> f2 = ff_pair();
    gemm(GemmSpec(rows, C, 5 * C, R(ff), f2[0], f2[1], R(out)).with_a2(R(h3), 4 * C).with_residual(xres).with_res_pre(u->res_pre && C != 320)
             .with_cols(stats_of(out)));
    drop(ff); drop(h3);
    return;
  }
  Act h4 = act(rows, C, hw, x.side);
  gemm(GemmSpec(rows, C, 4 * C, R(ff), f2w, f2b, R(h4)).with_residual(R(h3)).with_triple_out(x3t));
  drop(ff); drop(h3);
  gemm(GemmSpec(rows, C, C, R(h4), pow_, pob, R(out)).with_residual(xres).with_cols(stats_of(out)));
  drop(h4);
}

std::vector<Builder::Res> Builder::enumerate_resnets() const {
  const sdn_unet_config& c = u->cfg;
  std::vector<Res> v;
  char buf[96];
  for (int i = 0; i < c.n_levels; ++i)
    for (int j = 0; j < c.layers_per_block; ++j) {
      snprintf(buf, sizeof(buf), "down_blocks.%d.resnets.%d", i, j);
      v.push_back({buf, c.block_out_channels[i]});
    }
  const int top = c.block_out_channels[c.n_levels - 1];
  v.push_back({"mid_block.resnets.0", top});
  v.push_back({"mid_block.resnets.1", top});
  for (int i = 0; i < c.n_levels; ++i)
    for (int j = 0; j <= c.layers_per_block; ++j) {
      snprintf(buf, sizeof(buf), "up_blocks.%d.resnets.%d", i, j);
      v.push_back({buf, c.block_out_channels[c.n_levels - 1 - i]});
    }
  return v;
}

void Builder::build() {
  const sdn_unet_config& c = u->cfg;
  const int S = c.sample_size, ch0 = c.block_out_channels[0], tdim = 4 * ch0;
  char buf[96];

  Ref l1w = param("time_embedding.linear_1.weight", SDN_P_MAT, tdim, ch0), l1b = param("time_embedding.linear_1.bias", SDN_P_VEC_F32, tdim, 0);
  Ref l2w = param("time_embedding.linear_2.weight", SDN_P_MAT, tdim, tdim), l2b = param("time_embedding.linear_2.bias", SDN_P_VEC_F32, tdim, 0);
  const std::vector<Res> rs = enumerate_resnets();
  int total = 0;
  std::vector<std::pair<std::string, int>> tw, tb;
  for (const Res& r : rs) { tw.push_back({r.pfx + ".time_emb_proj.weight", r.cout}); tb.push_back({r.pfx + ".time_emb_proj.bias", r.cout}); total += r.cout; }
  Ref tpw = stacked(tw, tdim), tpb = stacked(tb, 0);
  u->tproj_total = total;
  gn_stats = Ref{SP_WS, arena.alloc((int64_t)B * 129 * 64 * 2 * 4)};
  plan->tscalar_off = arena.alloc(256);
  Act tsin = act(B, ch0);
  { Op o; o.kind = OP_TEMB; o.batch = B; o.c1 = ch0; o.out = R(tsin); snprintf(o.label, sizeof(o.label), "k_temb"); emit(o); }
  x3t_hold = true;
  Act t1 = act(B, tdim);
  gemm(GemmSpec(B, tdim, ch0, R(tsin), l1w, l1b, R(t1)).with_act(SDN_ACT_SILU));
  drop(tsin);
  Act semb = act(B, tdim);
  gemm(GemmSpec(B, tdim, tdim, R(t1), l2w, l2b, R(semb)).with_act(SDN_ACT_SILU));
  drop(t1);
  Act tp = act(B, total, 0, 0, 4);
  tproj = R(tp);
  gemm(GemmSpec(B, total, tdim, R(semb), tpw, tpb, R(tp)).with_out_kind(SDN_OUT_F32));
  drop(semb);
  x3t_hold = false;

  Ref ciw = param("conv_in.weight", SDN_P_CONV3X3, ch0, 9 * c.in_channels), cib = param("conv_in.bias", SDN_P_VEC_F32, ch0, 0);
  const int rep = (c.latent_repeat > 1 && c.level_has_attn[0] && u->subbatch_bytes == 0) ? c.latent_repeat : 1;
  if (B % rep != 0) { plan->ws_bytes = -1; return; }
  const int Bfull = B, Bp = B / rep;
  Act hp = act((int64_t)Bp * S * S, ch0, S * S, S);
  { Op o; o.kind = OP_CONV_IN; o.batch = Bp; o.c1 = c.in_channels; o.c2 = ch0; o.hw = S; o.a = Ref{SP_IN, 0}; o.w = ciw; o.bias = cib; o.out = R(hp);
    o.flops = 2.0 * Bp * S * S * (double)ch0 * 9 * c.in_channels; o.bytes = (double)Bp * S * S * (4.0 * c.in_channels + 2.0 * ch0);
    snprintf(o.label, sizeof(o.label), "k_conv_in"); emit(o); }
  Act h = hp;
  if (rep > 1) { h = act((int64_t)B * S * S, ch0, S * S, S); repeat(hp, h, rep); }

  std::vector<Act> skips;
  skips.push_back(h);
  Act cur = h;
// ... 87 lines not shown
```

Baseline: 8.424 images/sec.

## Fuse GroupNorm apply into the K=320 proj_in GEMM via per-batch affine table

Adds a GroupNorm variant that only computes statistics and emits a per-batch, per-channel scale/shift table. A new GNA form of the K=320 GEMM loads that table into LDS and applies it to the A panel before the MFMA loop. This skips writing and re-reading the normalized activation before proj_in. The path sits behind a new k320_gn plan flag that defaults to off. The change also moves the LayerNorm-fold row statistics in the k320 kernel into a separate pre-pass that stores mean and rstd in LDS; that part is on by default and adds an extra barrier per panel.

```diff
diff --git a/include/sdn.h b/include/sdn.h
--- a/include/sdn.h
+++ b/include/sdn.h
@@ -305,6 +305,10 @@
 int sdn_gemm_k320(int32_t dtype, const sdn_gemm_desc* desc, const void* a, const void* w, const float* bias, const float* ln_c,
                   const float* ln_d, float ln_eps, const void* residual, void* out, void* stream);
 int32_t sdn_gemm_k320_map(int32_t grid, int32_t col_groups, int32_t wg, int32_t* stream_out, int32_t* group_out);
+int sdn_gemm_k320_gn(int32_t dtype, const sdn_gemm_desc* desc, const void* x, int32_t hw, const float* gn_table, const void* w,
+                     const float* bias, const float* ln_c, const float* ln_d, const void* residual, void* out, void* stream);
+int sdn_groupnorm_table(int32_t dtype, const void* x, int32_t batch, int32_t hw, int32_t c, int32_t groups, float eps,
+                        const float* gamma, const float* beta, float* stats_ws, const float* cols, float* tab, void* stream);
 
 int sdn_gemm_stats_bf16(const sdn_gemm_desc* desc, const void* a, const void* a2, const void* w, const float* bias,
                         const float* rowbias, const void* residual, void* out, float* col_stats, void* stream);
diff --git a/safe_denoiser_amd/_lib.py b/safe_denoiser_amd/_lib.py
--- a/safe_denoiser_amd/_lib.py
+++ b/safe_denoiser_amd/_lib.py
@@ -133,6 +133,8 @@
     "sdn_row_stats_f16": (C.c_int, [_vp, _i64, _i32, _f32, _vp, _vp]),
     "sdn_ffn_geglu_fused": (C.c_int, [_i32, _i64, _i32, _vp, _vp, _vp, _vp, _vp, _vp, _vp, _vp, _vp, _vp, _vp]),
     "sdn_gemm_k320": (C.c_int, [_i32, C.POINTER(GemmDesc), _vp, _vp, _vp, _vp, _vp, _f32, _vp, _vp, _vp]),
+    "sdn_gemm_k320_gn": (C.c_int, [_i32, C.POINTER(GemmDesc), _vp, _i32, _vp, _vp, _vp, _vp, _vp, _vp, _vp, _vp]),
+    "sdn_groupnorm_table": (C.c_int, [_i32, _vp, _i32, _i32, _i32, _i32, _f32, _vp, _vp, _vp, _vp, _vp, _vp]),
     "sdn_gemm_k320_map": (_i32, [_i32, _i32, _i32, C.POINTER(_i32), C.POINTER(_i32)]),
     "sdn_gemm_stats_bf16": (C.c_int, [C.POINTER(GemmDesc), _vp, _vp, _vp, _vp, _vp, _vp, _vp, _vp, _vp]),
     "sdn_gemm_stats_f16": (C.c_int, [C.POINTER(GemmDesc), _vp, _vp, _vp, _vp, _vp, _vp, _vp, _vp, _vp]),
diff --git a/safe_denoiser_amd/csrc/sdn_gemm_k320.hip b/safe_denoiser_amd/csrc/sdn_gemm_k320.hip
--- a/safe_denoiser_amd/csrc/sdn_gemm_k320.hip
+++ b/safe_denoiser_amd/csrc/sdn_gemm_k320.hip
@@ -13,9 +13,10 @@
   const unsigned short* res; unsigned short* out;
   int M, ldc, ncg;
   float ln_eps;
+  const float* gn_tab; int gn_hw, gn_batch;
 };
 
-template <typename T, int LNF, bool RES>
+template <typename T, int LNF, bool RES, bool GNA = false>
 __global__ void __launch_bounds__(512)
 k_gemm_k320(const K320Args g) {
 #if defined(__HIP_DEVICE_COMPILE__)
@@ -26,10 +27,14 @@
   constexpr int A_PIECES = 5 * RB / 4;
   constexpr int SLOT = 40960, RING = 3 * SLOT;
   constexpr int STG = RING;
-  constexpr int PRM = STG + 32 * 640;
-  constexpr int SMEM = PRM + 3 * 1280;
+  constexpr int TAB = STG + 32 * 640;
+  constexpr int PRM = TAB + (GNA ? 3 * 4096 : 0);
+  constexpr int LNT = PRM + 3 * 1280;
+  constexpr int SMEM = LNT + (LNF ? 512 : 0);
   static_assert(5 * IMG * (RES ? 2 : 1) == SLOT, "a panel fills its slot");
-  static_assert(A_PIECES + (RES ? 5 : 0) == 10, "vmcnt(10) below counts ten pieces per DMA wave and panel");
+  static_assert(A_PIECES + (RES ? 5 : 0) == 10, "vmcnt(10) below counts ten pieces per DMA wave and panel (GNA: + 1 table piece, vmcnt(11))");
+  static_assert(!GNA || (!RES && !LNF), "the GroupNorm pre-pass goes with the plain form only");
+  static_assert(SMEM <= 160 * 1024, "one workgroup's LDS");
   __shared__ __attribute__((aligned(1024))) unsigned char smem[SMEM];
 
   const int tid = threadIdx.x, lane = tid & 63;
@@ -63,6 +68,7 @@
 
   const __amdgpu_buffer_rsrc_t rs_a = make_rsrc(g.a, (unsigned)((long)g.M * 640));
   [[maybe_unused]] const __amdgpu_buffer_rsrc_t rs_r = make_rsrc(RES ? g.res : g.a, RES ? (unsigned)((long)g.M * g.ldc * 2) : 0u);
+  [[maybe_unused]] const __amdgpu_buffer_rsrc_t rs_t = make_rsrc(GNA ? (const void*)g.gn_tab : (const void*)g.a, GNA ? (unsigned)g.gn_batch * 2560u : 0u);
   auto issue = [&](int p, int slot, int ln) {
     const int lrow = (ln >> 3) & 7;
     const unsigned a_lane = (unsigned)(lrow * 640 + (((ln & 7) ^ lrow) << 4));
@@ -82,6 +88,10 @@
         const unsigned off = (m0 + wid * 8) * (unsigned)(g.ldc * 2) + (unsigned)(n0 * 2 + q * 128) + r_lane;
         __builtin_amdgcn_raw_ptr_buffer_load_lds(rs_r, (lds_ptr_t)(dst + 5 * IMG + (wid * 5 + q) * 1024), 16, off, 0, 0, 0);
       }
+    }
+    if constexpr (GNA) {
+      const unsigned off = (m0 / (unsigned)g.gn_hw) * 2560u + (unsigned)(wid * 1024 + (ln & 63) * 16);
+      __builtin_amdgcn_raw_ptr_buffer_load_lds(rs_t, (lds_ptr_t)(smem + TAB + slot * 4096 + wid * 1024), 16, off, 0, 0, 0);
     }
   };
 
@@ -105,12 +115,71 @@
     const int st_lds = (st_r >> 3) * 5120 + (st_r & 7) * 128 + (((tl & 7) ^ (st_r & 7)) << 4);
     const int p = stream + i * S;
     const int m0 = p * ROWS;
-    if (wid < 4) asm volatile("s_waitcnt vmcnt(10)" ::: "memory");
+    if (wid < 4) {
+      if constexpr (GNA) asm volatile("s_waitcnt vmcnt(11)" ::: "memory");
+      else asm volatile("s_waitcnt vmcnt(10)" ::: "memory");
+    }
     asm volatile("s_waitcnt lgkmcnt(0)" ::: "memory");
     __builtin_amdgcn_s_barrier();
     asm volatile("" ::: "memory");
     if (wid < 4) issue(p + 2 * S, slot == 0 ? 2 : slot - 1, tl);
     const unsigned char* sa = smem + slot * SLOT;
+    if constexpr (GNA) {
+      const int prow = (tl >> 3) & 63, pch = (tl & 7) ^ (prow & 7);
+      const unsigned x_addr = (unsigned)(unsigned long)(lds_ptr_t)const_cast<unsigned char*>(sa) + (unsigned)(prow * 128 + ((tl & 7) << 4));
+      const unsigned t_addr = (unsigned)(unsigned long)(lds_ptr_t)(smem + TAB) + (unsigned)(slot * 4096 + pch * 32);
+      u32x4 xv[5];
+      asm volatile("ds_read_b128 %0, %1" : "=v"(xv[0]) : "v"(x_addr) : "memory");
+#pragma unroll
+      for (int j = 0; j < 5; ++j) {
+        f32x4 ca0, ca1, cb0, cb1;
+        asm volatile("ds_read_b128 %0, %1" : "=v"(ca0) : "v"(t_addr + (unsigned)(j * 256)) : "memory");
+        asm volatile("ds_read_b128 %0, %1" : "=v"(ca1) : "v"(t_addr + (unsigned)(j * 256 + 16)) : "memory");
+        asm volatile("ds_read_b128 %0, %1" : "=v"(cb0) : "v"(t_addr + (unsigned)(1280 + j * 256)) : "memory");
+        asm volatile("ds_read_b128 %0, %1" : "=v"(cb1) : "v"(t_addr + (unsigned)(1280 + j * 256 + 16)) : "memory");
+        if (j + 1 < 5) {
+          asm volatile("ds_read_b128 %0, %1" : "=v"(xv[j + 1]) : "v"(x_addr + (unsigned)((j + 1) * IMG)) : "memory");
+          asm volatile("s_waitcnt lgkmcnt(1)" : "+v"(xv[j]), "+v"(ca0), "+v"(ca1), "+v"(cb0), "+v"(cb1)::"memory");
+        } else {
+          asm volatile("s_waitcnt lgkmcnt(0)" : "+v"(xv[j]), "+v"(ca0), "+v"(ca1), "+v"(cb0), "+v"(cb1)::"memory");
+        }
+        u32x4 y;
+#pragma unroll
+        for (int e = 0; e < 4; ++e) {
+          const unsigned v = xv[j][e];
+          const float am0 = e < 2 ? ca0[2 * e] : ca1[2 * e - 4], am1 = e < 2 ? ca0[2 * e + 1] : ca1[2 * e - 3];
+          const float bm0 = e < 2 ? cb0[2 * e] : cb1[2 * e - 4], bm1 = e < 2 ? cb0[2 * e + 1] : cb1[2 * e - 3];
+          float y0 = fmaf(T::to_f(v & 0xffff), am0, bm0), y1 = fmaf(T::to_f(v >> 16), am1, bm1);
+          asm("" : "+v"(y0), "+v"(y1));
+          y[e] = T::pack2(y0, y1);
+        }
+        asm volatile("ds_write_b128 %0, %1" ::"v"(x_addr + (unsigned)(j * IMG)), "v"(y) : "memory");
+      }
+      asm volatile("s_waitcnt lgkmcnt(0)" ::: "memory");
+      __builtin_amdgcn_s_barrier();
+      asm volatile("" ::: "memory");
+    }
+    if constexpr (LNF) {
+      if (wid < 4) {
+        const int srow = wid * 16 + fr;
+        typename T::v8 fs[10];
+#pragma unroll
+        for (int s = 0; s < 10; ++s) fs[s] = *reinterpret_cast<const typename T::v8*>(sa + (s >> 1) * IMG + lds_off(srow, (s & 1) * 4 + fq));
+        float a1 = 0.f, a2 = 0.f;
+#pragma unroll
+        for (int s = 0; s < 10; ++s) { a1 = T::dot_ones(fs[s], a1); a2 = T::dot_self(fs[s], a2); }
+        const float invk = 1.0f / 320.0f;
+        a1 += __shfl_xor(a1, 16, 64); a2 += __shfl_xor(a2, 16, 64);
+        a1 += __shfl_xor(a1, 32, 64); a2 += __shfl_xor(a2, 32, 64);
+        const float mu = a1 * invk;
+        const float var = fmaxf(a2 * invk - mu * mu, 0.f);
+        const float rs = __builtin_amdgcn_rsqf(var + g.ln_eps);
+        const unsigned t_addr = (unsigned)(unsigned long)(lds_ptr_t)(smem + LNT) + (unsigned)srow * 8;
+        if (fq == 0)
+          asm volatile("ds_write_b64 %0, %1" ::"v"(t_addr), "v"((unsigned long long)__float_as_uint(rs) << 32 | __float_as_uint(mu)) : "memory");
+        __builtin_amdgcn_sched_barrier(0);
+      }
+    }
 #pragma unroll
     for (int gi = 0; gi < G; ++gi) {
       const int row_l = wm * (ROWS / 2) + gi * 16 + fr;
@@ -130,7 +199,6 @@
           acc[t][2] += T::to_f(hi & 0xffff); acc[t][3] += T::to_f(hi >> 16);
         }
       }
-      [[maybe_unused]] float s1 = 0.f, s2 = 0.f;
       typename T::v8 fa[2];
       fa[0] = *reinterpret_cast<const typename T::v8*>(sa + lds_off(row_l, fq));
 #pragma unroll
@@ -138,25 +206,21 @@
         if (s + 1 < 10)
           fa[(s + 1) & 1] = *reinterpret_cast<const typename T::v8*>(sa + ((s + 1) >> 1) * IMG + lds_off(row_l, ((s + 1) & 1) * 4 + fq));
         __builtin_amdgcn_sched_barrier(0);
-        if constexpr (LNF) { s1 = T::dot_ones(fa[s & 1], s1); s2 = T::dot_self(fa[s & 1], s2); }
 #pragma unroll
         for (int t = 0; t < 5; ++t) acc[t] = T::mfma16(wf[t][s], fa[s & 1], acc[t]);
         __builtin_amdgcn_sched_barrier(0);
       }
-      [[maybe_unused]] float mu = 0.f, rs = 0.f;
-      if constexpr (LNF) {
-        const float invk = 1.0f / 320.0f;
-        float a1 = s1, a2 = s2;
-        a1 += __shfl_xor(a1, 16, 64); a2 += __shfl_xor(a2, 16, 64);
-        a1 += __shfl_xor(a1, 32, 64); a2 += __shfl_xor(a2, 32, 64);
-        mu = a1 * invk;
-        const float var = fmaxf(a2 * invk - mu * mu, 0.f);
-        rs = __builtin_amdgcn_rsqf(var + g.ln_eps);
-      }
-      if (!RES && gi > 0) {
+      if (!RES && (gi > 0 || LNF)) {
         asm volatile("s_waitcnt lgkmcnt(0)" ::: "memory");
         __builtin_amdgcn_s_barrier();
         asm volatile("" ::: "memory");
+      }
+      [[maybe_unused]] float mu = 0.f, rs = 0.f;
+      if constexpr (LNF) {
+        unsigned long long mr;
+        asm volatile("ds_read_b64 %0, %1" : "=v"(mr) : "v"((unsigned)(unsigned long)(lds_ptr_t)(smem + LNT) + (unsigned)row_l * 8) : "memory");
+        asm volatile("s_waitcnt lgkmcnt(0)" : "+v"(mr)::"memory");
+        mu = __uint_as_float((unsigned)mr); rs = __uint_as_float((unsigned)(mr >> 32));
       }
       const unsigned char* oimg = RES ? sa + 5 * IMG : smem + STG;
       const unsigned o_addr = (unsigned)(unsigned long)(lds_ptr_t)const_cast<unsigned char*>(oimg);
@@ -194,6 +258,7 @@
 int launch_k320(const K320Args& g, int grid, bool ln, bool res, hipStream_t st) {
   if (ln) hipLaunchKernelGGL((k_gemm_k320<T, 1, false>), dim3(grid), dim3(512), 0, st, g);
   else if (res) hipLaunchKernelGGL((k_gemm_k320<T, 0, true>), dim3(grid), dim3(512), 0, st, g);
+  else if (g.gn_tab) hipLaunchKernelGGL((k_gemm_k320<T, 0, false, true>), dim3(grid), dim3(512), 0, st, g);
   else hipLaunchKernelGGL((k_gemm_k320<T, 0, false>), dim3(grid), dim3(512), 0, st, g);
   return sdn_launch_status();
 }
@@ -218,8 +283,8 @@
 }
 extern "C" void sdn_debug_k320_reset_launch(void) { for (int& v : g_k320_last) v = 0; }
 
-extern "C" int sdn_gemm_k320(int32_t dtype, const sdn_gemm_desc* d, const void* a, const void* w, const float* bias, const float* ln_c,
-                             const float* ln_d, float ln_eps, const void* residual, void* out, void* stream) {
+static int k320_run(int32_t dtype, const sdn_gemm_desc* d, const void* a, const void* w, const float* bias, const float* ln_c,
+                    const float* ln_d, float ln_eps, const void* residual, void* out, void* stream, const float* gn_tab, int32_t gn_hw) {
   if (!d || !a || !w || !out || dtype < 0 || dtype > 1) return SDN_E_INVALID;
   if (d->K != 320 || d->N <= 0 || d->N % 320 != 0 || d->M < 0) return SDN_E_INVALID;
   if (d->a_mode != SDN_A_PLAIN || (d->K1 != 0 && d->K1 != d->K) || d->act != SDN_ACT_NONE || d->out_kind != SDN_OUT_BF16 ||
@@ -255,13 +320,25 @@
   g.a = (const unsigned short*)a; g.w = (const unsigned short*)w; g.bias = bias; g.ln_c = ln_c; g.ln_d = ln_d;
   g.res = (const unsigned short*)residual; g.out = (unsigned short*)out;
   g.M = d->M; g.ldc = ldc; g.ncg = ncg; g.ln_eps = ln_eps;
+  g.gn_tab = gn_tab; g.gn_hw = gn_hw; g.gn_batch = gn_tab ? d->M / gn_hw : 0;
   {
     int s0, c0;
     const int S = sdn_k320_map(grid, ncg, 0, &s0, &c0);
     const int rows = residual ? 32 : 64;
-    const int v[8] = {6, dtype, ln ? 1 : 0, residual ? 1 : 0, grid, ncg, S, (d->M + rows - 1) / rows};
+    const int v[8] = {6, dtype, gn_tab ? 2 : (ln ? 1 : 0), residual ? 1 : 0, grid, ncg, S, (d->M + rows - 1) / rows};
     for (int i = 0; i < 8; ++i) g_k320_last[i] = v[i];
   }
   hipStream_t st = (hipStream_t)stream;
   return dtype == 0 ? launch_k320<SdnBF16>(g, grid, ln, residual != nullptr, st) : launch_k320<SdnF16>(g, grid, ln, residual != nullptr, st);
 }
+
+extern "C" int sdn_gemm_k320(int32_t dtype, const sdn_gemm_desc* d, const void* a, const void* w, const float* bias, const float* ln_c,
+                             const float* ln_d, float ln_eps, const void* residual, void* out, void* stream) {
+  return k320_run(dtype, d, a, w, bias, ln_c, ln_d, ln_eps, residual, out, stream, nullptr, 0);
+}
+
+extern "C" int sdn_gemm_k320_gn(int32_t dtype, const sdn_gemm_desc* d, const void* x, int32_t hw, const float* gn_tab, const void* w,
+                                const float* bias, const float* ln_c, const float* ln_d, const void* residual, void* out, void* stream) {
+  if (!d || !gn_tab || hw <= 0 || hw % 64 != 0 || d->N != 320 || d->M % hw != 0 || ln_c || ln_d || residual || !al16(gn_tab)) return SDN_E_INVALID;
+  return k320_run(dtype, d, x, w, bias, nullptr, nullptr, 0.f, nullptr, out, stream, gn_tab, hw);
+}
diff --git a/safe_denoiser_amd/csrc/sdn_norm.hip b/safe_denoiser_amd/csrc/sdn_norm.hip
--- a/safe_denoiser_amd/csrc/sdn_norm.hip
+++ b/safe_denoiser_amd/csrc/sdn_norm.hip
@@ -162,6 +162,18 @@
   }
 }
 
+__global__ void __launch_bounds__(THREADS)
+k_affine_table(const float* __restrict__ stats, const float* __restrict__ gamma, const float* __restrict__ beta, int C, int groups,
+                  float* __restrict__ tab) {
+  const int cpg = C / groups, b = blockIdx.x;
+  for (int c = threadIdx.x; c < C; c += THREADS) {
+    const int gi = c / cpg;
+    const float mean = stats[((long)b * groups + gi) * 2 + 0], rstd = stats[((long)b * groups + gi) * 2 + 1];
+    const float a = rstd * gamma[c];
+    tab[(long)b * 2 * C + c] = a; tab[(long)b * 2 * C + C + c] = beta[c] - mean * a;
+  }
+}
+
 template <typename T, int NQ, int R>
 __global__ void __launch_bounds__(THREADS)
 k_layernorm(const unsigned short* __restrict__ x, long rows, int C, float eps, const float* __restrict__ gamma,
@@ -362,8 +374,8 @@
 template <typename T>
 int groupnorm_impl(const void* x, const void* x2, int32_t batch, int32_t hw, int32_t c1, int32_t c2, int32_t groups,
                    float eps, int32_t silu, const float* gamma, const float* beta, void* out, float* stats_ws,
-                   void* stream, const float* cols1 = nullptr, const float* cols2 = nullptr) {
-  if (!x || !gamma || !beta || !out || !stats_ws || batch < 0 || hw <= 0 || c1 <= 0 || c2 < 0 || groups <= 0 ||
+                   void* stream, const float* cols1 = nullptr, const float* cols2 = nullptr, bool stats_only = false) {
+  if (!x || !gamma || !beta || (!out && !stats_only) || !stats_ws || batch < 0 || hw <= 0 || c1 <= 0 || c2 < 0 || groups <= 0 ||
       groups > 64)
     return SDN_E_INVALID;
   if (c2 > 0 && !x2) return SDN_E_INVALID;
@@ -397,6 +409,7 @@
     hipLaunchKernelGGL(k_gn_finalize, dim3(batch), dim3(512), 0, st, partials, ntiles, groups,
                        (float)hw * (float)(C / groups), eps, stats_ws);
   }
+  if (stats_only) return sdn_launch_status();
   int rows_per_block = (256 * 8 * 16) / C;
   if (rows_per_block < 1) rows_per_block = 1;
   const int nblk = (hw + rows_per_block - 1) / rows_per_block;
@@ -591,6 +604,16 @@
 SDN_NORM_ENTRY(bf16, SdnBF16)
 SDN_NORM_ENTRY(f16, SdnF16)
 
+extern "C" int sdn_groupnorm_table(int32_t dtype, const void* x, int32_t batch, int32_t hw, int32_t c, int32_t groups, float eps,
+                                   const float* gamma, const float* beta, float* stats_ws, const float* cols, float* tab, void* stream) {
+  if (!tab || (reinterpret_cast<uintptr_t>(tab) & 15) || dtype < 0 || dtype > 1) return SDN_E_INVALID;
+  const int rc = dtype == 0 ? sdn_norm_detail::groupnorm_impl<SdnBF16>(x, nullptr, batch, hw, c, 0, groups, eps, 0, gamma, beta, nullptr, stats_ws, stream, cols, nullptr, true)
+                            : sdn_norm_detail::groupnorm_impl<SdnF16>(x, nullptr, batch, hw, c, 0, groups, eps, 0, gamma, beta, nullptr, stats_ws, stream, cols, nullptr, true);
+  if (rc != SDN_OK || batch == 0) return rc;
+  hipLaunchKernelGGL(sdn_norm_detail::k_affine_table, dim3(batch), dim3(sdn_norm_detail::THREADS), 0, (hipStream_t)stream, stats_ws, gamma, beta, c, groups, tab);
+  return sdn_launch_status();
+}
+
 extern "C" int sdn_row_stats_bf16(const void* x, int64_t rows, int32_t c, float eps, float* out, void* stream) {
   return sdn_norm_detail::row_stats_impl<SdnBF16>(x, rows, c, eps, out, stream);
 }
diff --git a/safe_denoiser_amd/csrc/sdn_plan.h b/safe_denoiser_amd/csrc/sdn_plan.h
--- a/safe_denoiser_amd/csrc/sdn_plan.h
+++ b/safe_denoiser_amd/csrc/sdn_plan.h
@@ -169,6 +169,7 @@
   bool x3_pairs = true;
   bool res_pre = true;
   bool gemm_k320 = true;
+  bool k320_gn = false;
   bool x3_expand = true;
   bool split_k = false;
   bool conv_up4 = true;
@@ -206,7 +207,7 @@
 
 namespace sdn_plan {
 
-constexpr bool kK320Plain = true, kK320Ln = true, kK320Rp = true;
+constexpr bool kK320Plain = true, kK320Ln = true, kK320Rp = true, kK320Gn = true;
 
 struct GemmSpec {
   int64_t M; int N, K;
@@ -218,6 +219,7 @@
   Ref cols;
   bool res_pre = false;
   bool k320 = false;
+  Ref gn_tab; int gn_hw = 0;
   bool triple_out = false;
   bool pair_out = false;
   bool force_x3t = false;
@@ -235,6 +237,7 @@
   GemmSpec& with_cols(Ref v) { cols = v; return *this; }
   GemmSpec& with_res_pre(bool v) { res_pre = v; return *this; }
   GemmSpec& with_k320(bool v) { k320 = v; return *this; }
+  GemmSpec& with_gn_table(Ref tab, int hw) { gn_tab = tab; gn_hw = hw; return *this; }
   GemmSpec& with_triple_out(bool v) { triple_out = v; return *this; }
   GemmSpec& with_pair_out(bool v) { pair_out = v; return *this; }
   GemmSpec& with_force_x3t(bool v) { force_x3t = v; return *this; }
@@ -300,6 +303,7 @@
   void push_gemm(Op& o, Ref cols);
   void conv3x3(const ConvSpec& s);
   void groupnorm(const Act& x, const Act* x2, float eps, int silu, Ref gamma, Ref beta, const Act& out);
+  void groupnorm_table(const Act& x, float eps, Ref gamma, Ref beta, const Act& tab);
   void layernorm(const Act& x, Ref gamma, Ref beta, const Act& out);
   void repeat(const Act& in, const Act& out, int rep);
   void attention(Ref q, Ref k, Ref v, Ref out, int nq, int nk, int C, int ldq, int ldk, int ldv, bool kv_pairs = false);
diff --git a/safe_denoiser_amd/csrc/sdn_plan_api.hip b/safe_denoiser_amd/csrc/sdn_plan_api.hip
--- a/safe_denoiser_amd/csrc/sdn_plan_api.hip
+++ b/safe_denoiser_amd/csrc/sdn_plan_api.hip
@@ -361,6 +361,7 @@
 void sdn_debug_set_res_pre(sdn_unet* u, int on) { if (u && u->res_pre != (on != 0)) set_plan_toggle(u, &sdn_unet::res_pre, on != 0); }
 
 void sdn_debug_set_gemm_k320(sdn_unet* u, int on) { if (u && u->gemm_k320 != (on != 0)) set_plan_toggle(u, &sdn_unet::gemm_k320, on != 0); }
+void sdn_debug_set_k320_gn(sdn_unet* u, int on) { if (u && u->k320_gn != (on != 0)) set_plan_toggle(u, &sdn_unet::k320_gn, on != 0); }
 
 void sdn_debug_set_ln_fold(sdn_unet* u, int on) { if (u) set_plan_toggle(u, &sdn_unet::ln_fold, on != 0); }
 
diff --git a/safe_denoiser_amd/csrc/sdn_plan_core.hip b/safe_denoiser_amd/csrc/sdn_plan_core.hip
--- a/safe_denoiser_amd/csrc/sdn_plan_core.hip
+++ b/safe_denoiser_amd/csrc/sdn_plan_core.hip
@@ -136,11 +136,15 @@
   o.bytes = 2.0 * ((double)M * K + (double)N * K + (double)M * (act_ == SDN_ACT_GEGLU ? N / 2 : N)) +
             (residual.space != SP_NONE ? 2.0 * (double)M * N : 0.0);
   snprintf(o.label, sizeof(o.label), "k_gemm<%d>%s", sdn_gemm_pick_tile((int)M, N, K, act_, residual.space != SP_NONE && !rp), rp ? "/rp" : "");
+  const bool gn = s.gn_tab.space != SP_NONE;
   if (s.k320 && !x3t && K == 320 && N % 320 == 0 && act_ == SDN_ACT_NONE && s.out_kind == SDN_OUT_BF16 && s.n_valid == 0 && s.a2.space == SP_NONE &&
       s.rowbias.space == SP_NONE && (residual.space == SP_NONE || rp) && s.cols.space == SP_NONE && !u->split_k &&
-      (rp ? kK320Rp : kK320Plain)) {
-    o.k320 = 1;
-    snprintf(o.label, sizeof(o.label), "k_gemm_k320%s", rp ? "/rp" : "");
+      (rp ? kK320Rp : kK320Plain) && (!gn || (N == 320 && residual.space == SP_NONE && s.gn_hw > 0 && s.gn_hw % 64 == 0 && M % s.gn_hw == 0))) {
+    o.k320 = gn ? 2 : 1;
+    if (gn) { o.aux = s.gn_tab; o.hw = s.gn_hw; }
+    snprintf(o.label, sizeof(o.label), "k_gemm_k320%s", gn ? "/gn" : (rp ? "/rp" : ""));
+  } else if (gn) {
+    plan_bad = true;
   }
   push_gemm(o, s.cols);
 }
@@ -236,6 +240,15 @@
   snprintf(o.label, sizeof(o.label), o.cols1.space != SP_NONE ? "k_gn_apply" : "k_gn_stats+apply");
   emit(o);
 }
+void Builder::groupnorm_table(const Act& x, float eps, Ref gamma, Ref beta, const Act& tab) {
+  Op o; o.kind = OP_GN; o.a = R(x); o.mod = 1;
+  o.batch = B; o.hw = x.hw; o.c1 = x.C; o.c2 = 0; o.groups = u->cfg.norm_groups; o.eps = eps;
+  o.silu = 0; o.w = gamma; o.bias = beta; o.out = R(tab); o.aux = gn_stats;
+  if (x.st_off >= 0) o.cols1 = Ref{SP_WS, x.st_off};
+  o.bytes = (o.cols1.space != SP_NONE ? 0.0 : 2.0 * (double)B * x.hw * x.C) + 8.0 * (double)B * x.C;
+  snprintf(o.label, sizeof(o.label), o.cols1.space != SP_NONE ? "k_gn_table" : "k_gn_stats+table");
+  emit(o);
+}
 void Builder::layernorm(const Act& x, Ref gamma, Ref beta, const Act& out) {
   Op o; o.kind = OP_LN; o.a = R(x); o.rows = (int64_t)B * x.hw; o.c1 = x.C; o.eps = 1e-5f; o.w = gamma; o.bias = beta;
   o.out = R(out);
diff --git a/safe_denoiser_amd/csrc/sdn_plan_run.hip b/safe_denoiser_amd/csrc/sdn_plan_run.hip
--- a/safe_denoiser_amd/csrc/sdn_plan_run.hip
+++ b/safe_denoiser_amd/csrc/sdn_plan_run.hip
@@ -198,6 +198,11 @@
                                (void*)P(o.out), stream);
       break;
     case OP_GEMM:
+      if (o.k320 == 2) {
+        rc = sdn_gemm_k320_gn(f16 ? 1 : 0, &o.gd, P(o.a), o.hw, (const float*)P(o.aux), P(o.w), (const float*)P(o.bias), nullptr, nullptr, nullptr,
+                              (void*)P(o.out), stream);
+        break;
+      }
       if (o.k320) {
         rc = sdn_gemm_k320(f16 ? 1 : 0, &o.gd, P(o.a), P(o.w), o.ln ? nullptr : (const float*)P(o.bias), o.ln ? (const float*)P(o.ln_c) : nullptr,
                            o.ln ? (const float*)P(o.ln_d) : nullptr, o.eps, o.ln ? nullptr : P(o.residual), (void*)P(o.out), stream);
@@ -229,6 +234,11 @@
                          (const float*)P(o.rowgate), P(o.residual), (void*)P(o.out), stream);
       break;
     case OP_GN:
+      if (o.mod == 1) {
+        rc = sdn_groupnorm_table(f16 ? 1 : 0, P(o.a), o.batch, o.hw, o.c1, o.groups, o.eps, (const float*)P(o.w), (const float*)P(o.bias),
+                                 (float*)P(o.aux), o.cols1.space != SP_NONE ? (const float*)P(o.cols1) : nullptr, (float*)P(o.out), stream);
+        break;
+      }
       if (o.cols1.space != SP_NONE) {
         rc = (f16 ? sdn_groupnorm_cols_f16 : sdn_groupnorm_cols_bf16)(P(o.a), P(o.a2), o.batch, o.hw, o.c1, o.c2, o.groups, o.eps,
                                                                       o.silu, (const float*)P(o.w), (const float*)P(o.bias),
diff --git a/safe_denoiser_amd/csrc/sdn_plan_unet.hip b/safe_denoiser_amd/csrc/sdn_plan_unet.hip
--- a/safe_denoiser_amd/csrc/sdn_plan_unet.hip
+++ b/safe_denoiser_amd/csrc/sdn_plan_unet.hip
@@ -104,12 +104,21 @@
   Ref f2w = param(tb + ".ff.net.2.weight", SDN_P_MAT, C, 4 * C), f2b = param(tb + ".ff.net.2.bias", SDN_P_VEC_F32, C, 0);
   Ref pow_ = param(pfx + ".proj_out.weight", SDN_P_MAT, C, C), pob = param(pfx + ".proj_out.bias", SDN_P_VEC_F32, C, 0);
 
-  Act gn = act(rows, C, hw, x.side);
-  groupnorm(x, nullptr, 1e-6f, 0, ng, nb, gn);
-  Act h = act(rows, C, hw, x.side);
   const bool k320 = u->gemm_k320 && C == 320 && es == 2 && !x3t && u->subbatch_bytes == 0;
-  gemm(GemmSpec(rows, C, C, R(gn), piw, pib, R(h)).with_k320(k320));
-  drop(gn);
+  Act h;
+  if (k320 && u->k320_gn && kK320Gn && hw % 64 == 0 && !u->split_k) {
+    Act tab = act(B, 2 * C, 0, 0, 4);
+    groupnorm_table(x, 1e-6f, ng, nb, tab);
+    h = act(rows, C, hw, x.side);
+    gemm(GemmSpec(rows, C, C, R(x), piw, pib, R(h)).with_k320(true).with_gn_table(R(tab), hw));
+    drop(tab);
+  } else {
+    Act gn = act(rows, C, hw, x.side);
+    groupnorm(x, nullptr, 1e-6f, 0, ng, nb, gn);
+    h = act(rows, C, hw, x.side);
+    gemm(GemmSpec(rows, C, C, R(gn), piw, pib, R(h)).with_k320(k320));
+    drop(gn);
+  }
   const bool fold12 = u->ln_fold && C <= 640, fold3 = u->ln_fold && C == 320;
   const int hd = C / u->cfg.n_heads;
   const bool x3p = x3t && u->x3_pairs && (hd == 40 || hd == 80 || hd == 160);
```

Result: no change. 8.447 images/sec, median of 6 (+0.3%).
